# norabelrose/sparse-vae

Measured on AMD Instinct MI355X. Metric: training tokens/sec + ELBO match vs CPU ref, 512-tok seq, 1/2/4/8 MI355X, higher is better.
Workload: dtype bf16; 1 GPU; c2: TransformerVAE 6L d512 heads 8 seq 512, batch 64/GPU, dense attention, dropout 0.1, fwd+bwd+allreduce+clip+RAdam; model=TransformerVAE-6L-d512, global_batch=64, seq_len=512, parallelism=dp1

## Files before the change

include/svae.h:

```cpp
#ifndef SVAE_H
#define SVAE_H
#include <stdint.h>
#ifdef __cplusplus
extern "C" {
#endif

typedef void* svae_stream_t;

enum svae_epi {
  SVAE_EPI_BF16 = 0,
  SVAE_EPI_F32 = 1,
  SVAE_EPI_F32_ACC = 2,
  SVAE_EPI_F32_ATOMIC = 3,
  SVAE_EPI_GELU = 4,
  SVAE_EPI_GELU_BWD = 5,
  SVAE_EPI_DROPOUT_RESID = 6,
  SVAE_EPI_ROTARY_BF16 = 7,
  SVAE_EPI_CE_STATS = 8,
  SVAE_EPI_CE_PROB = 9,
  SVAE_EPI_ROWSCALE_GATHER = 10
};

typedef struct svae_gemm_desc {
  const void* A;
  const void* B;
  int64_t lda, ldb, batch_stride_a, batch_stride_b;
  int32_t M, N, K;
  int32_t batch, splits;
  int32_t a_t, b_t;
  int32_t epi;
  void* C;
  int64_t ldc, batch_stride_c;
  const float* bias;
  const float* resid;
  int64_t ldr;
  void* aux;
  int64_t ldaux;
  float alpha;
  float drop_p;
  uint64_t seed;
  const float* rot_tab;
  int32_t rot_cols, rot_d, rot_seq;
  const int32_t* labels;
  float* label_logit;
  float* a_rowsum;
  const float* k_weight;
  const float* row_a;
  const float* row_b;
  const void* gather;
  int64_t ldg;
  float* delta;
  const float* delta_o32;
  int64_t ld_o32;
  int32_t delta_hd, delta_seq;
} svae_gemm_desc;

int svae_gemm(const svae_gemm_desc* d, svae_stream_t stream);

int svae_gemm_pair(const svae_gemm_desc* d0, const svae_gemm_desc* d1, svae_stream_t stream);

#define SVAE_GROUP_MAX 256
#define SVAE_GROUP_MAX_BLOCKS 1024
int64_t svae_gemm_group_table_bytes(int32_t n);
int svae_gemm_group(const svae_gemm_desc* d, int32_t n, int32_t max_blocks, void* table, void* table_host,
                    int64_t table_bytes, svae_stream_t stream);

int svae_resid_ln_fwd(const float* x, const void* y, int32_t y_dtype, int64_t ldy, float drop_p, uint64_t seed,
                      const float* zrows, int32_t zmod, const float* w, const float* b, float* xo, void* h, float* mean,
                      float* rstd, int32_t rows, int32_t D, svae_stream_t stream);
int svae_layernorm_fwd(const void* x, int32_t x_dtype, const float* w, const float* b, void* y,
                       float* mean, float* rstd, int32_t rows, int32_t D, svae_stream_t stream);
int svae_layernorm_bwd(const void* dy, const void* x, int32_t x_dtype, const float* w, const float* mean,
                       const float* rstd, const float* dres, float* dx, void* dx_bf, float* part,
                       int32_t nblk, int32_t rows, int32_t D, int32_t zero_mod, svae_stream_t stream);
int svae_layernorm_bwd_drop(const void* dy, const void* x, int32_t x_dtype, const float* w, const float* mean,
                            const float* rstd, const float* dres, float* dx, void* dx_bf, float* part, int32_t nblk,
                            int32_t rows, int32_t D, int32_t zero_mod, float bf_drop_p, uint64_t bf_seed,
                            int32_t bf_zero_mod, float* zrow, void* zrow_bf, svae_stream_t stream);
int svae_layernorm_bwd_gelu(const void* dy, const void* x, int32_t x_dtype, const float* w, const float* mean,
                            const float* rstd, const void* gp, void* out_bf, float* part, int32_t nblk, int32_t rows,
                            int32_t D, svae_stream_t stream);
int svae_layernorm_fwd_z(float* x, const float* zrows, int32_t zmod, const float* w, const float* b, void* y,
                         float* mean, float* rstd, int32_t rows, int32_t D, svae_stream_t stream);
int svae_layernorm_nblk(int32_t rows);
#define SVAE_LN_MULTI_MAX 4
int svae_layernorm_fwd_multi(const float* x, const float* const* w, const float* const* b, void* const* y, int32_t n,
                             float* mean, float* rstd, int32_t rows, int32_t D, svae_stream_t stream);
int svae_layernorm_bwd_multi(const void* const* dy, const float* x, const float* const* w, const float* mean,
                             const float* rstd, const float* dres, float* dx, float* const* part, int32_t nblk,
                             int32_t n, int32_t rows, int32_t D, svae_stream_t stream);

int svae_colsum(const void* in, int32_t in_dtype, int32_t rows, int32_t cols, int64_t ld, float* out,
                int32_t accumulate, svae_stream_t stream);

#define SVAE_COLSUM_MAX 8
typedef struct svae_colsum_seg {
  const float* in;
  float* out;
  int64_t ld;
  int32_t rows, cols;
} svae_colsum_seg;
int svae_colsum_multi(const svae_colsum_seg* segs, int32_t n, svae_stream_t stream);

typedef struct svae_attn_desc {
  const void* q; const void* k; const void* v; void* o;
  int64_t sq, sk, sv, so, bq, bk, bv, bo;
  const uint8_t* key_pad;
  float* lse;
  int32_t B, H, Lq, Lk, hd, causal;
  float scale;
  const void* dout; int64_t sdo, bdo;
  float* delta;
  float* dq;
  int64_t bdq;
  void* dk; void* dv;
  int64_t sdk, sdv, bdk, bdv;
  const float* rot_tab;
  int32_t rot_d;
  float* o32;
  int64_t so32, bo32;
  float* dq_part;
  void* dq_bf;
  int64_t ldq_bf;
  int32_t window;
  int32_t delta_ready;
  void* o_lo;
  int64_t so_lo, bo_lo;
  float* fwd_ws;
  int64_t fwd_ws_elems;
} svae_attn_desc;

int svae_attn_fwd(const svae_attn_desc* d, svae_stream_t stream);
int64_t svae_attn_fwd_ws_elems(int32_t B, int32_t H, int32_t Lq, int32_t Lk, int32_t hd, int32_t causal, int32_t window);
int svae_attn_bwd(const svae_attn_desc* d, svae_stream_t stream);
int64_t svae_attn_dq_part_elems(int32_t B, int32_t H, int32_t Lq, int32_t Lk, int32_t hd);
int64_t svae_attn_dq_part_elems_w(int32_t B, int32_t H, int32_t Lq, int32_t Lk, int32_t hd, int32_t window);
int svae_dq_finalize(const float* dq, void* out, int64_t ldo, int32_t rows, int32_t D, const float* rot_tab,
                     int32_t seq, svae_stream_t stream);

int svae_embedding_fwd(const int32_t* ids, const void* table_bf, float* out, void* out_bf, int32_t rows,
                       int32_t D, svae_stream_t stream);
int svae_embedding_fwd_dual(const int32_t* ids, const void* table, float* out, float* out2, int32_t rows, int32_t D,
                            svae_stream_t stream);
int svae_embedding_bwd(const int32_t* ids, const float* dout, float* dtable, int32_t rows, int32_t D,
                       svae_stream_t stream);

int svae_reparam_kl_fwd(const float* stats, const float* eps, uint64_t seed, const int64_t* ntok,
                        float* z, void* z_bf, float* eps_out, float* raw_kl, float* kl_out, int32_t B,
                        int32_t Z, svae_stream_t stream);
int svae_reparam_kl_bwd(const float* stats, const float* eps, const float* dz, const int64_t* ntok,
                        const float* gkl, float* dstats, int32_t B, int32_t Z, svae_stream_t stream);

int svae_ce_finalize(const float* part, int32_t ntile, const float* label_logit, const int32_t* labels,
                     int32_t rows, int32_t seq, int32_t nchunks, int32_t chunk_len, float* lse, float* row_loss,
                     float* chunk_w, float* nll_out, float* red_ws, svae_stream_t stream);
int svae_ce_weighted_nll(const float* row_loss, const int32_t* labels, const float* tok_w, int32_t rows,
                         int32_t seq, int32_t nchunks, int32_t chunk_len, float* out, float* red_ws,
                         svae_stream_t stream);
int32_t svae_ce_red_ws_elems(int32_t nchunks);
int svae_ce_grad(void* logits, int64_t ld, const float* lse, const float* chunk_w, const int32_t* labels,
                 const float* gscale, float* dbias, int32_t rows, int32_t V, int32_t seq, int32_t nchunks,
                 int32_t chunk_len, svae_stream_t stream);

int svae_ce_label_logit(const void* hh, int64_t ldh, const void* W, int64_t ldw, const float* bias,
                        const int32_t* labels, int32_t rows, int32_t D, float* out, svae_stream_t stream);
int svae_ce_prob_finalize(const float* part, int32_t ntile, const float* row_off, const int32_t* labels,
                          int32_t rows, int32_t seq, int32_t nchunks, int32_t chunk_len, float* lse, float* row_loss,
                          float* chunk_w, float* nll_out, float* red_ws, svae_stream_t stream);
int svae_ce_prob_finalize_fix(const float* part, int32_t ntile, float* row_off, const int32_t* labels, int32_t rows,
                              int32_t seq, int32_t nchunks, int32_t chunk_len, float* lse, float* row_loss,
                              float* chunk_w, float* nll_out, float* red_ws, const void* hh, int64_t ldh, const void* W,
                              int64_t ldw, const float* bias, void* P, int64_t ldp, int32_t V, int32_t D,
                              int32_t* sat_ws, svae_stream_t stream);
int svae_ce_prob_bwd_prep(const void* hh, int64_t ldh, const float* lse, const float* row_off, const float* chunk_w,
                          const int32_t* labels, const float* gscale, int32_t rows, int32_t seq, int32_t nchunks,
                          int32_t chunk_len, int32_t D, void* hh_out, float* r_out, float* q_out, float* dbias,
                          svae_stream_t stream);
int svae_embedding_bwd_ce(const int32_t* ids, const float* dout, float* dtable, int32_t rows, int32_t D, int32_t seq,
                          const void* hh, const float* q, svae_stream_t stream);

int svae_dropout_bwd_cast(const float* g, void* out, float p, uint64_t seed, int64_t n, int32_t cols,
                          int64_t ld_in, svae_stream_t stream);
int svae_gelu_bwd(const float* dx, const void* gp, void* out, int64_t n, svae_stream_t stream);
int svae_prep_tokens(const int64_t* ids, const void* pad, int32_t pad_mode, int32_t B, int32_t L, int32_t* ids32,
                     int32_t* labels, void* padm, const int64_t* ntok, int64_t* ntok_out, svae_stream_t stream);
int svae_step_scalars(const float* nll, const float* kl, const float* gloss, float kl_weight, float* loss, float* gs,
                      svae_stream_t stream);
int svae_cast_bf16(const float* in, void* out, int64_t n, svae_stream_t stream);
int svae_transpose_blocks(const void* src, void* dst, const int64_t* table, int32_t nblocks, int32_t total_tiles,
                          svae_stream_t stream);
int svae_extract_rows(float* x, int64_t ld, int32_t rows, int32_t mod, int32_t D, float* out,
                      svae_stream_t stream);
int svae_zproj_bwd(const float* g, const void* z, const void* W, float* dW, float* db, float* dz, int32_t B,
                   int32_t d, int32_t Z, svae_stream_t stream);
#define SVAE_ZPROJ_MAX 32
typedef struct svae_zproj_seg {
  const float* g;
  const void* W;
  float* dW;
  float* db;
} svae_zproj_seg;
int svae_zproj_bwd_multi(const svae_zproj_seg* segs, int32_t n, const void* z, float* dz, int32_t B, int32_t d,
                         int32_t Z, svae_stream_t stream);
typedef struct svae_zproj_fwd_seg {
  const void* W;
  const float* bias;
  float* out;
} svae_zproj_fwd_seg;
int svae_zproj_fwd_multi(const svae_zproj_fwd_seg* segs, int32_t n, const void* z, int32_t B, int32_t d, int32_t Z,
                         svae_stream_t stream);

int svae_sumsq(const float* g, int64_t n, float* part, int32_t nblk, svae_stream_t stream);
int svae_radam(float* p, void* pbf, const float* g, float* m, float* v, int64_t n, const float* part,
               int32_t nblk, const float* scal, float* norm_out, svae_stream_t stream);
int svae_clip_grad(float* g, int64_t n, const float* part, int32_t nblk, float max_norm, float* norm_out,
                   svae_stream_t stream);

int svae_gemm_f32(const float* A, const float* W, float* C, int32_t M, int32_t N, int32_t K, int64_t lda, int64_t ldw,
                  int64_t ldc, const float* bias, const float* resid, int64_t ldr, int32_t epi, const float* rot_tab,
                  int32_t rot_cols, int32_t rot_d, int32_t rot_seq, svae_stream_t stream);
int svae_attn_fwd_f32(const float* q, const float* k, const float* v, float* o, int64_t sq, int64_t sk, int64_t sv,
                      int64_t so, int64_t bq, int64_t bk, int64_t bv, int64_t bo, const uint8_t* key_pad, int32_t B,
                      int32_t H, int32_t Lq, int32_t Lk, int32_t hd, int32_t causal, int32_t window, float scale,
                      svae_stream_t stream);
int svae_layernorm_fwd_f32(const float* x, const float* w, const float* b, float* y, int32_t rows, int32_t D,
                           svae_stream_t stream);

int svae_mutual_info(const float* stats, const float* eps, uint64_t seed, const float* kl, int32_t B, int32_t Z,
                     int32_t S, float* ws, float* out, svae_stream_t stream);

int svae_ce_seq_logprob(const float* part, int32_t ntile, const float* label_logit, const int32_t* labels,
                        int32_t rows, int32_t seq, float* out, svae_stream_t stream);

int svae_dec_linear(const float* X, int64_t ldx, const float* W, int64_t ldw, const float* bias, float* Y, int64_t ldy,
                    const float* resid, int64_t ldr, int32_t M, int32_t N, int32_t K, int32_t epi, const float* rot_tab,
                    int32_t rot_cols, int32_t rot_d, const int32_t* cur, float* part_ws, int64_t part_elems,
                    svae_stream_t stream);
int svae_dec_attn(const float* qkv, int64_t ldq, float* kcache, float* vcache, int32_t B, int32_t H, int32_t hd,
                  int32_t T, const int32_t* cur, int32_t window, float scale, float* O, int64_t ldo,
                  svae_stream_t stream);
int svae_dec_embed(const int64_t* out_ids, int32_t T, const int32_t* cur, const float* table, float* x, int32_t B,
                   int32_t D, svae_stream_t stream);
int svae_dec_penalty(float* logits, int64_t ldl, int32_t rows, const int32_t* row_map, const int64_t* out_ids,
                     int32_t T, const int32_t* cur, const uint8_t* live, float penalty, svae_stream_t stream);
int svae_dec_sample(const float* logits, int64_t ldl, int32_t V, int32_t rows, const int32_t* row_map,
                    int64_t* out_ids, int32_t T, const int32_t* cur, uint8_t* live, int32_t end_token,
                    float temperature, int32_t top_k, float top_p, uint64_t seed, int32_t* live_count,
                    svae_stream_t stream);
int svae_dec_advance(int32_t* cur, svae_stream_t stream);

int svae_slot_linear(const float* X, int64_t ldx, const float* W, int64_t ldw, const float* bias, float* Y, int64_t ldy,
                     const float* resid, int64_t ldr, int32_t S, int32_t N, int32_t K, const float* rot_tab,
                     int32_t rot_cols, int32_t rot_d, const int32_t* pos, float* part_ws, int64_t part_elems,
                     svae_stream_t stream);
int svae_slot_attn(const float* qkv, int64_t ldq, float* kcache, float* vcache, int32_t S, int32_t H, int32_t hd,
                   int32_t T, const int32_t* pos, int32_t window, float scale, float* O, int64_t ldo,
                   svae_stream_t stream);
int svae_slot_embed(const int64_t* ids, int32_t T, const int32_t* pos, const float* table, float* x, int32_t S,
                    int32_t D, svae_stream_t stream);
int svae_slot_splice(float* x, const float* zp, int64_t ldz, const int32_t* pos, int32_t S, int32_t D,
// ... 77 lines not shown
```

sparse-vae_amd/csrc/elementwise.hip:

```cpp
#include "common.h"
#include "../../include/svae.h"

using namespace svae;

namespace {

__global__ __launch_bounds__(256) void emb_fwd_kernel(const int* __restrict__ ids, const float* __restrict__ table,
                                                      float* __restrict__ out, bf16* __restrict__ out_bf, int rows,
                                                      int D, float* __restrict__ out2) {
  const int lane = threadIdx.x & 63;
  const int row = blockIdx.x * 4 + (threadIdx.x >> 6);
  if (row >= rows) return;
  const long long src = (long long)ids[row] * D;
  for (int c = lane * 4; c < D; c += 256) {
    const f32x4 v = *(const f32x4*)(table + src + c);
    *(f32x4*)(out + (long long)row * D + c) = v;
    if (out2) *(f32x4*)(out2 + (long long)row * D + c) = v;
    if (out_bf)
      *(bf16x4*)(out_bf + (long long)row * D + c) = (bf16x4){f2bf(v[0]), f2bf(v[1]), f2bf(v[2]), f2bf(v[3])};
  }
}

__global__ __launch_bounds__(256) void emb_bwd_kernel(const int* __restrict__ ids, const float* __restrict__ dout,
                                                      float* __restrict__ dtable, int rows, int D) {
  const int lane = threadIdx.x & 63;
  const int row = blockIdx.x * 4 + (threadIdx.x >> 6);
  if (row >= rows) return;
  const long long dst = (long long)ids[row] * D;
  for (int c = lane; c < D; c += 64) atomicAdd(dtable + dst + c, dout[(long long)row * D + c]);
}

__global__ __launch_bounds__(256) void emb_bwd_ce_kernel(const int* __restrict__ ids, const float* __restrict__ dout,
                                                         float* __restrict__ dtable, int rows, int D, int seq,
                                                         const bf16* __restrict__ hh, const float* __restrict__ q) {
  const int lane = threadIdx.x & 63;
  const int row = blockIdx.x * 4 + (threadIdx.x >> 6);
  if (row >= rows) return;
  const long long dst = (long long)ids[row] * D;
  const float qp = (row % seq != 0) ? q[row - 1] : 0.f;
  const bf16* hp = hh + (long long)(row - 1) * D;
  for (int c = lane; c < D; c += 64) {
    float g = dout[(long long)row * D + c];
    if (qp != 0.f) g -= qp * (float)hp[c];
    atomicAdd(dtable + dst + c, g);
  }
}

constexpr int REPARAM_WAVES = 16;

__global__ __launch_bounds__(1024) void reparam_fwd_kernel(const float* __restrict__ stats, const float* __restrict__ eps_in,
                                                           unsigned long long seed, const long long* __restrict__ ntok,
                                                           float* __restrict__ z, bf16* __restrict__ z_bf,
                                                           float* __restrict__ eps_out, float* __restrict__ raw_kl,
                                                           float* __restrict__ kl_out, int B, int Z) {
  __shared__ float red[2][REPARAM_WAVES];
  const int lane = threadIdx.x & 63, wave = threadIdx.x >> 6;
  float acc_norm = 0.f, acc_raw = 0.f;
  constexpr int NB = 4;
  for (int b0 = wave; b0 < B; b0 += NB * REPARAM_WAVES) {
    float klsum[NB];
#pragma unroll
    for (int k = 0; k < NB; ++k) klsum[k] = 0.f;
    for (int j = lane; j < Z; j += 64) {
      float mu[NB], lv[NB], e[NB];
#pragma unroll
      for (int k = 0; k < NB; ++k) {
        const int b = b0 + k * REPARAM_WAVES;
        if (b < B) {
          mu[k] = stats[(long long)b * 2 * Z + j];
          lv[k] = stats[(long long)b * 2 * Z + Z + j];
          if (eps_in) {
            e[k] = eps_in[(long long)b * Z + j];
          } else {
            const unsigned long long idx = ((unsigned long long)b * Z + j) * 2ull;
            const float u1 = rand_uniform(seed, idx), u2 = rand_uniform(seed, idx + 1);
            e[k] = sqrtf(-2.f * __logf(u1)) * __cosf(6.283185307179586f * u2);
          }
        }
      }
#pragma unroll
      for (int k = 0; k < NB; ++k) {
        const int b = b0 + k * REPARAM_WAVES;
        if (b < B) {
          const float var = __expf(lv[k]);
          const float zz = mu[k] + e[k] * sqrtf(var);
          if (eps_out) eps_out[(long long)b * Z + j] = e[k];
          z[(long long)b * Z + j] = zz;
          if (z_bf) z_bf[(long long)b * Z + j] = f2bf(zz);
          klsum[k] += 0.5f * (mu[k] * mu[k] + var - lv[k] - 1.0f);
        }
      }
    }
#pragma unroll
    for (int k = 0; k < NB; ++k) {
      const int b = b0 + k * REPARAM_WAVES;
      if (b < B) {
        const float ks = wave_sum(klsum[k]);
        if (lane == 0) raw_kl[b] = ks;
        acc_raw += ks;
        acc_norm += ks / (float)ntok[b];
      }
    }
  }
  if (lane == 0) { red[0][wave] = acc_norm; red[1][wave] = acc_raw; }
  __syncthreads();
  if (threadIdx.x == 0) {
    float n = 0.f, r = 0.f;
#pragma unroll
    for (int w = 0; w < REPARAM_WAVES; ++w) { n += red[0][w]; r += red[1][w]; }
    kl_out[0] = n / B;
    kl_out[1] = r / B;
  }
}

__global__ __launch_bounds__(256) void reparam_bwd_kernel(const float* __restrict__ stats, const float* __restrict__ eps,
                                                          const float* __restrict__ dz, const long long* __restrict__ ntok,
                                                          const float* __restrict__ gkl, float* __restrict__ dstats,
                                                          int B, int Z) {
  const int i = blockIdx.x * 256 + threadIdx.x;
  if (i >= B * Z) return;
  const int b = i / Z, j = i % Z;
  const float mu = stats[(long long)b * 2 * Z + j];
  const float lv = stats[(long long)b * 2 * Z + Z + j];
  const float var = __expf(lv), sd = sqrtf(var);
  const float w = gkl[0] / ((float)B * (float)ntok[b]);
  const float g = dz ? dz[i] : 0.f;
  dstats[(long long)b * 2 * Z + j] = g + w * mu;
  dstats[(long long)b * 2 * Z + Z + j] = g * eps[i] * sd * 0.5f + w * 0.5f * (var - 1.0f);
}

__global__ __launch_bounds__(256) void ce_rows_kernel(const float* __restrict__ part, int ntile,
                                                      const float* __restrict__ label_logit, const int* __restrict__ labels,
                                                      int rows, float* __restrict__ lse, float* __restrict__ row_loss) {
  const int lane = threadIdx.x & 63;
  const int row = blockIdx.x * 4 + (threadIdx.x >> 6);
  if (row >= rows) return;
  const float2* pr = (const float2*)part + (long long)row * ntile;
  float mx = -INFINITY;
  for (int t = lane; t < ntile; t += 64) mx = fmaxf(mx, pr[t].x);
  mx = wave_max(mx);
  float se = 0.f;
  for (int t = lane; t < ntile; t += 64) {
    const float2 v = pr[t];
    se += (v.x == -INFINITY) ? 0.f : v.y * __expf(v.x - mx);
  }
  se = wave_sum(se);
  if (lane == 0) {
    const float l = mx + __logf(se);
    lse[row] = l;
    row_loss[row] = labels[row] != 0 ? l - label_logit[row] : 0.f;
  }
}

__global__ __launch_bounds__(256) void ce_label_logit_kernel(const bf16* __restrict__ hh, long long ldh,
                                                             const bf16* __restrict__ W, long long ldw,
                                                             const float* __restrict__ bias,
                                                             const int* __restrict__ labels, int rows, int D,
                                                             float* __restrict__ out) {
  const int lane = threadIdx.x & 63;
  const int row = blockIdx.x * 4 + (threadIdx.x >> 6);
  if (row >= rows) return;
  const int lab = labels[row];
  if (lab == 0) {
    if (lane == 0) out[row] = 0.f;
    return;
  }
  float acc = 0.f;
  for (int c = lane * 8; c < D; c += 512) {
    const bf16x8 a = *(const bf16x8*)(hh + (long long)row * ldh + c);
    const bf16x8 b = *(const bf16x8*)(W + (long long)lab * ldw + c);
#pragma unroll
    for (int e = 0; e < 8; ++e) acc = fmaf((float)a[e], (float)b[e], acc);
  }
  acc = wave_sum(acc);
  if (lane == 0) out[row] = acc + (bias ? bias[lab] : 0.f);
}

__global__ __launch_bounds__(256) void ce_prob_rows_kernel(const float* __restrict__ part, int ntile,
                                                           const float* __restrict__ off, const int* __restrict__ labels,
                                                           int rows, float* __restrict__ lse, float* __restrict__ row_loss,
                                                           int* __restrict__ sat) {
  __shared__ float red[8][33];
  const int r = threadIdx.x & 31, sl = threadIdx.x >> 5;
  const int row = blockIdx.x * 32 + r;
  float acc = 0.f;
  if (row < rows) {
    int t = sl;
    for (; t + 56 < ntile; t += 64) {
      float v[8];
#pragma unroll
      for (int u = 0; u < 8; ++u) v[u] = part[(long long)(t + 8 * u) * rows + row];
      acc += ((v[0] + v[1]) + (v[2] + v[3])) + ((v[4] + v[5]) + (v[6] + v[7]));
    }
    for (; t < ntile; t += 8) acc += part[(long long)t * rows + row];
  }
  red[sl][r] = acc;
  __syncthreads();
  if (sl != 0 || row >= rows) return;
  float se = red[0][r];
#pragma unroll
  for (int k = 1; k < 8; ++k) se += red[k][r];
  const bool live = labels[row] != 0;
  const float l = live ? __logf(se) : 0.f;
  lse[row] = live ? off[row] + l : 0.f;
  row_loss[row] = l;
  if (sat && live && !(se < 0x1p100f)) sat[1 + atomicAdd(sat, 1)] = row;
}

__global__ __launch_bounds__(256) void ce_prob_fixup_kernel(const int* __restrict__ sat, const bf16* __restrict__ hh,
                                                            long long ldh, const bf16* __restrict__ W, long long ldw,
                                                            const float* __restrict__ bias, bf16* __restrict__ P,
                                                            long long ldp, int V, int D, float* __restrict__ off,
                                                            float* __restrict__ lse, float* __restrict__ row_loss) {
  __shared__ float h[1024];
  __shared__ float red[4];
  const int n = sat[0];
  const int lane = threadIdx.x & 63, w = threadIdx.x >> 6;
  for (int i = blockIdx.x; i < n; i += gridDim.x) {
    const int row = sat[1 + i];
    __syncthreads();
    for (int c = threadIdx.x; c < D; c += 256) h[c] = (float)hh[(long long)row * ldh + c];
    __syncthreads();
    float mx = -INFINITY;
    for (int col = threadIdx.x; col < V; col += 256) {
      const bf16* wr = W + (long long)col * ldw;
      float acc = 0.f;
      for (int c = 0; c < D; c += 8) {
        const bf16x8 b = *(const bf16x8*)(wr + c);
#pragma unroll
        for (int e = 0; e < 8; ++e) acc = fmaf(h[c + e], (float)b[e], acc);
      }
      mx = fmaxf(mx, acc + (bias ? bias[col] : 0.f));
    }
    mx = wave_max(mx);
    if (lane == 0) red[w] = mx;
    __syncthreads();
    mx = fmaxf(fmaxf(red[0], red[1]), fmaxf(red[2], red[3]));
    __syncthreads();
    float se = 0.f;
    for (int col = threadIdx.x; col < V; col += 256) {
      const bf16* wr = W + (long long)col * ldw;
      float acc = 0.f;
      for (int c = 0; c < D; c += 8) {
        const bf16x8 b = *(const bf16x8*)(wr + c);
#pragma unroll
        for (int e = 0; e < 8; ++e) acc = fmaf(h[c + e], (float)b[e], acc);
      }
      const float p = __expf(acc + (bias ? bias[col] : 0.f) - mx);
      P[(long long)row * ldp + col] = f2bf(p);
      se += p;
    }
    se = wave_sum(se);
    if (lane == 0) red[w] = se;
    __syncthreads();
    if (threadIdx.x == 0) {
      const float l = mx + __logf(red[0] + red[1] + red[2] + red[3]);
      row_loss[row] = l - off[row];
      lse[row] = l;
      off[row] = mx;
    }
  }
}

__global__ __launch_bounds__(256) void ce_prob_bwd_prep_kernel(const bf16* __restrict__ hh, long long ldh,
                                                               const float* __restrict__ lse,
                                                               const float* __restrict__ off,
                                                               const float* __restrict__ chunk_w,
                                                               const int* __restrict__ labels,
                                                               const float* __restrict__ gscale, int rows, int seq,
                                                               int nchunks, int chunk_len, int D,
                                                               bf16* __restrict__ hh_out, float* __restrict__ r_out,
                                                               float* __restrict__ q_out, float* __restrict__ dbias) {
  const int lane = threadIdx.x & 63;
  const int row = blockIdx.x * 4 + (threadIdx.x >> 6);
  if (row >= rows) return;
  const int lab = labels[row];
  float q = 0.f, r = 0.f;
  if (lab != 0) {
    const int ch = min((row % seq) / chunk_len, nchunks - 1);
    q = gscale[0] * chunk_w[ch];
    r = q * __expf(off[row] - lse[row]);
  }
  for (int c = lane * 8; c < D; c += 512) {
    const bf16x8 a = *(const bf16x8*)(hh + (long long)row * ldh + c);
    bf16x8 o;
#pragma unroll
    for (int e = 0; e < 8; ++e) o[e] = f2bf(r * (float)a[e]);
    *(bf16x8*)(hh_out + (long long)row * D + c) = o;
  }
  if (lane == 0) {
    r_out[row] = r;
    q_out[row] = q;
    if (lab != 0 && dbias) atomicAdd(dbias + lab, -q);
  }
}

__global__ __launch_bounds__(256) void ce_seq_logprob_kernel(const float* __restrict__ part, int ntile,
                                                             const float* __restrict__ label_logit,
                                                             const int* __restrict__ labels, int seq,
                                                             float* __restrict__ out) {
  __shared__ float ws[4];
  const int lane = threadIdx.x & 63, w = threadIdx.x >> 6;
  const long long r0 = (long long)blockIdx.x * seq;
  float acc = 0.f;
  for (int i = w; i < seq; i += 4) {
    const long long row = r0 + i;
    if (labels[row] == 0) continue;
    const float2* pr = (const float2*)part + row * ntile;
    float mx = -INFINITY;
    for (int t = lane; t < ntile; t += 64) mx = fmaxf(mx, pr[t].x);
    mx = wave_max(mx);
    float se = 0.f;
    for (int t = lane; t < ntile; t += 64) {
      const float2 v = pr[t];
      se += (v.x == -INFINITY) ? 0.f : v.y * __expf(v.x - mx);
    }
    se = wave_sum(se);
    acc += label_logit[row] - (mx + __logf(se));
  }
  if (lane == 0) ws[w] = acc;
  __syncthreads();
  if (threadIdx.x == 0) out[blockIdx.x] = ws[0] + ws[1] + ws[2] + ws[3];
}

__global__ __launch_bounds__(256) void mi_marginal_kernel(const float* __restrict__ stats, const float* __restrict__ eps,
                                                          unsigned long long seed, int B, int Z,
                                                          float* __restrict__ ws) {
  extern __shared__ float xs[];
  __shared__ float red[8];
  const int si = blockIdx.x, i = si % B, tid = threadIdx.x;
  const int lane = tid & 63, w = tid >> 6;
  float sq = 0.f;
  for (int z = tid; z < Z; z += 256) {
    const float mu = stats[(long long)i * 2 * Z + z];
    const float sd = sqrtf(__expf(stats[(long long)i * 2 * Z + Z + z]));
    float e;
    if (eps) {
      e = eps[(long long)si * Z + z];
    } else {
      const unsigned long long idx = ((unsigned long long)si * Z + z) * 2ull;
      const float u1 = rand_uniform(seed, idx), u2 = rand_uniform(seed, idx + 1);
      e = sqrtf(-2.f * __logf(u1)) * __cosf(6.283185307179586f * u2);
    }
    const float x = mu + e * sd;
    xs[z] = x;
    sq += x * x;
  }
  __syncthreads();
  const float lsq2pi = 0.91893853320467274f;
  float m = -INFINITY, e = 0.f;
  for (int j = tid; j < B; j += 256) {
    const float* st = stats + (long long)j * 2 * Z;
    float acc = 0.f;
    for (int z = 0; z < Z; ++z) {
      const float lv = st[Z + z];
      const float d = xs[z] - st[z];
      acc += -(d * d) * (0.5f * __expf(-lv)) - 0.5f * lv - lsq2pi;
    }
    const float nm = fmaxf(m, acc);
    e = e * __expf(m - nm) + __expf(acc - nm);
    m = nm;
  }
  float mx = wave_max(m);
  if (lane == 0) red[w] = mx;
  __syncthreads();
  mx = fmaxf(fmaxf(red[0], red[1]), fmaxf(red[2], red[3]));
  __syncthreads();
  float se = wave_sum(m == -INFINITY ? 0.f : e * __expf(m - mx));
  sq = wave_sum(sq);
  if (lane == 0) { red[w] = se; red[4 + w] = sq; }
  __syncthreads();
  if (tid == 0) {
    ws[si] = mx + __logf(red[0] + red[1] + red[2] + red[3]) - __logf((float)B);
    ws[gridDim.x + si] = red[4] + red[5] + red[6] + red[7];
  }
}

__global__ __launch_bounds__(256) void mi_final_kernel(const float* __restrict__ ws, int n, int Z,
                                                       const float* __restrict__ kl, float* __restrict__ out) {
  __shared__ float red[8];
  const int tid = threadIdx.x, lane = tid & 63, w = tid >> 6;
  float m = 0.f, q = 0.f;
  for (int k = tid; k < n; k += 256) { m += ws[k]; q += ws[n + k]; }
  m = wave_sum(m);
  q = wave_sum(q);
  if (lane == 0) { red[w] = m; red[4 + w] = q; }
  __syncthreads();
  if (tid == 0) {
    const float mm = (red[0] + red[1] + red[2] + red[3]) / n;
    const float qq = (red[4] + red[5] + red[6] + red[7]) / n;
    const float sample_prob = -0.5f * (qq + Z * 1.8378770664093453f);
    out[0] = kl[0] - (sample_prob - mm);
  }
}

constexpr int CE_RED_BLOCKS = 64;
constexpr int CE_MAX_CHUNKS = 1024;

__global__ __launch_bounds__(256) void ce_reduce_part_kernel(const float* __restrict__ row_loss,
                                                             const int* __restrict__ labels,
                                                             const float* __restrict__ tok_w, int rows, int seq,
                                                             int nchunks, int chunk_len, float* __restrict__ part) {
  __shared__ float red[8];
  const int ch = blockIdx.y;
  const int p0 = ch * chunk_len;
  const int clen = ch == nchunks - 1 ? seq - p0 : chunk_len;
  const int n = (rows / seq) * clen;
  float s = 0.f, c = 0.f;
  for (int i = blockIdx.x * 256 + threadIdx.x; i < n; i += CE_RED_BLOCKS * 256) {
    const int r = (i / clen) * seq + p0 + i % clen;
    const int lab = labels[r];
    if (lab != 0) {
      const float w = tok_w ? tok_w[lab] : 1.f;
      s += w * row_loss[r];
      c += w;
    }
  }
  s = wave_sum(s);
  c = wave_sum(c);
  if ((threadIdx.x & 63) == 0) { red[threadIdx.x >> 6] = s; red[4 + (threadIdx.x >> 6)] = c; }
  __syncthreads();
  if (threadIdx.x == 0) {
    float* o = part + ((long long)ch * CE_RED_BLOCKS + blockIdx.x) * 2;
    o[0] = (red[0] + red[1]) + (red[2] + red[3]);
    o[1] = (red[4] + red[5]) + (red[6] + red[7]);
  }
}

__global__ __launch_bounds__(256) void ce_reduce_final_kernel(const float* __restrict__ part, int nchunks,
                                                              float* __restrict__ chunk_w, float* __restrict__ nll_out) {
  __shared__ float mean[CE_MAX_CHUNKS];
  for (int k = threadIdx.x; k < nchunks; k += 256) {
    float ts = 0.f, tc = 0.f;
    for (int b = 0; b < CE_RED_BLOCKS; ++b) {
      ts += part[((long long)k * CE_RED_BLOCKS + b) * 2];
      tc += part[((long long)k * CE_RED_BLOCKS + b) * 2 + 1];
    }
    mean[k] = ts / tc;
    if (chunk_w) chunk_w[k] = 1.0f / (tc * (float)nchunks);
  }
  __syncthreads();
  if (threadIdx.x == 0) {
    float nll = 0.f;
    for (int j = 0; j < nchunks; ++j) nll += mean[j];
    nll_out[0] = nll / nchunks;
  }
}

#define CE_U 2
#define CE_LOAD(p) __builtin_nontemporal_load(p)
#define CE_STORE(v, p) __builtin_nontemporal_store(v, p)
__global__ __launch_bounds__(256) void ce_grad_kernel(bf16* __restrict__ logits, long long ld, const float* __restrict__ lse,
                                                      const float* __restrict__ chunk_w, const int* __restrict__ labels,
                                                      const float* __restrict__ gscale, float* __restrict__ dbias, int rows,
                                                      int V, int seq, int nchunks, int chunk_len, int rows_per_block) {
  const int c0 = (blockIdx.x * 256 + threadIdx.x) * 8;
  const int r0 = blockIdx.y * rows_per_block;
  const int r1 = min(rows, r0 + rows_per_block);
  const float g = gscale[0];
  float db[8] = {0.f, 0.f, 0.f, 0.f, 0.f, 0.f, 0.f, 0.f};
  if (c0 < V) {
    for (int row = r0; row < r1; row += CE_U) {
      bf16x8 v[CE_U];
#pragma unroll
      for (int u = 0; u < CE_U; ++u)
        if (row + u < r1) v[u] = CE_LOAD((const bf16x8*)(logits + (long long)(row + u) * ld + c0));
#pragma unroll
      for (int u = 0; u < CE_U; ++u) {
        const int rr = row + u;
        if (rr >= r1) break;
        bf16x8* ptr = (bf16x8*)(logits + (long long)rr * ld + c0);
        const int lab = labels[rr];
        bf16x8 o;
        if (lab == 0) {
          o = (bf16x8){0, 0, 0, 0, 0, 0, 0, 0};
        } else {
          const int ch = min((rr % seq) / chunk_len, nchunks - 1);
          const float w = g * chunk_w[ch];
          const float l = lse[rr];
#pragma unroll
          for (int e = 0; e < 8; ++e) {
            float pr = __expf((float)v[u][e] - l);
            if (c0 + e == lab) pr -= 1.0f;
            const float d = w * pr;
            db[e] += d;
            o[e] = f2bf(d);
          }
        }
        CE_STORE(o, ptr);
      }
    }
    if (dbias) {
#pragma unroll
      for (int e = 0; e < 8; ++e) atomicAdd(dbias + c0 + e, db[e]);
    }
  }
}

__global__ __launch_bounds__(256) void dropout_bwd_cast_kernel(const float* __restrict__ g, bf16* __restrict__ out, float p,
                                                               unsigned long long seed, long long n, int cols, long long ld_in) {
  const float scale = p > 0.f ? 1.0f / (1.0f - p) : 1.0f;
  for (long long i = ((long long)blockIdx.x * 256 + threadIdx.x) * 4; i < n; i += (long long)gridDim.x * 1024) {
    const long long r = i / cols;
    const int c = (int)(i % cols);
    const f32x4 v = *(const f32x4*)(g + r * ld_in + c);
    bf16x4 o;
    float u[4] = {1.f, 1.f, 1.f, 1.f};
    if (p > 0.f) rand_uniform4(seed, (unsigned long long)i >> 2, u);
#pragma unroll
    for (int e = 0; e < 4; ++e) {
      float x = v[e];
      if (p > 0.f) x = (u[e] >= p) ? x * scale : 0.f;
      o[e] = f2bf(x);
    }
    *(bf16x4*)(out + i) = o;
  }
}

__global__ __launch_bounds__(256) void prep_tokens_kernel(const int64_t* __restrict__ ids, const unsigned char* __restrict__ pad,
                                                          int pad_mode, int rows, int L, int32_t* __restrict__ ids32,
                                                          int32_t* __restrict__ labels, unsigned char* __restrict__ padm,
                                                          const int64_t* __restrict__ ntok, int64_t* __restrict__ ntok_out,
                                                          int B) {
  const int t = blockIdx.x * 256 + threadIdx.x;
  if (t < B && ntok) ntok_out[t] = ntok[t];
  if (t >= rows) return;
  const int64_t v = ids[t];
  ids32[t] = (int32_t)v;
  labels[t] = (t % L == L - 1) ? 0 : (int32_t)ids[t + 1];
// ... 224 lines not shown
  if (g < 1) g = 1;
  if (g > cap) g = cap;
  return (int)g;
}

}

SVAE_EXPORT int svae_embedding_fwd(const int32_t* ids, const void* table, float* out, void* out_bf, int32_t rows,
                                   int32_t D, svae_stream_t stream) {
  if (!ids || !table || !out || rows <= 0 || D % 4) return SVAE_EINVAL;
  hipLaunchKernelGGL(emb_fwd_kernel, dim3((rows + 3) / 4), dim3(256), 0, (hipStream_t)stream, ids, (const float*)table,
                     out, (bf16*)out_bf, rows, D, (float*)nullptr);
  SVAE_LAUNCH_CHECK();
  return SVAE_OK;
}

SVAE_EXPORT int svae_embedding_fwd_dual(const int32_t* ids, const void* table, float* out, float* out2, int32_t rows,
                                        int32_t D, svae_stream_t stream) {
  if (!ids || !table || !out || !out2 || rows <= 0 || D % 4) return SVAE_EINVAL;
  hipLaunchKernelGGL(emb_fwd_kernel, dim3((rows + 3) / 4), dim3(256), 0, (hipStream_t)stream, ids, (const float*)table,
                     out, (bf16*)nullptr, rows, D, out2);
  SVAE_LAUNCH_CHECK();
  return SVAE_OK;
}

SVAE_EXPORT int svae_embedding_bwd(const int32_t* ids, const float* dout, float* dtable, int32_t rows, int32_t D,
                                   svae_stream_t stream) {
  if (!ids || !dout || !dtable || rows <= 0 || D <= 0) return SVAE_EINVAL;
  hipLaunchKernelGGL(emb_bwd_kernel, dim3((rows + 3) / 4), dim3(256), 0, (hipStream_t)stream, ids, dout, dtable, rows, D);
  SVAE_LAUNCH_CHECK();
  return SVAE_OK;
}

SVAE_EXPORT int svae_embedding_bwd_ce(const int32_t* ids, const float* dout, float* dtable, int32_t rows, int32_t D,
                                      int32_t seq, const void* hh, const float* q, svae_stream_t stream) {
  if (!ids || !dout || !dtable || !hh || !q || rows <= 0 || D <= 0 || seq <= 0 || rows % seq) return SVAE_EINVAL;
  hipLaunchKernelGGL(emb_bwd_ce_kernel, dim3((rows + 3) / 4), dim3(256), 0, (hipStream_t)stream, ids, dout, dtable, rows,
                     D, seq, (const bf16*)hh, q);
  SVAE_LAUNCH_CHECK();
  return SVAE_OK;
}

SVAE_EXPORT int svae_ce_label_logit(const void* hh, int64_t ldh, const void* W, int64_t ldw, const float* bias,
                                    const int32_t* labels, int32_t rows, int32_t D, float* out, svae_stream_t stream) {
  if (!hh || !W || !labels || !out || rows <= 0 || D <= 0 || D % 8 || ldh % 8 || ldw % 8) return SVAE_EINVAL;
  if (((uintptr_t)hh | (uintptr_t)W) & 15) return SVAE_EINVAL;
  hipLaunchKernelGGL(ce_label_logit_kernel, dim3((rows + 3) / 4), dim3(256), 0, (hipStream_t)stream, (const bf16*)hh,
                     (long long)ldh, (const bf16*)W, (long long)ldw, bias, labels, rows, D, out);
  SVAE_LAUNCH_CHECK();
  return SVAE_OK;
}

SVAE_EXPORT int svae_ce_prob_finalize(const float* part, int32_t ntile, const float* row_off, const int32_t* labels,
                                      int32_t rows, int32_t seq, int32_t nchunks, int32_t chunk_len, float* lse,
                                      float* row_loss, float* chunk_w, float* nll_out, float* red_ws,
                                      svae_stream_t stream) {
  return svae_ce_prob_finalize_fix(part, ntile, (float*)row_off, labels, rows, seq, nchunks, chunk_len, lse, row_loss,
                                   chunk_w, nll_out, red_ws, nullptr, 0, nullptr, 0, nullptr, nullptr, 0, 0, 0, nullptr,
                                   stream);
}

SVAE_EXPORT int svae_ce_prob_finalize_fix(const float* part, int32_t ntile, float* row_off, const int32_t* labels,
                                          int32_t rows, int32_t seq, int32_t nchunks, int32_t chunk_len, float* lse,
                                          float* row_loss, float* chunk_w, float* nll_out, float* red_ws,
                                          const void* hh, int64_t ldh, const void* W, int64_t ldw, const float* bias,
                                          void* P, int64_t ldp, int32_t V, int32_t D, int32_t* sat_ws,
                                          svae_stream_t stream) {
  if (!part || !row_off || !labels || !lse || !row_loss || !chunk_w || !nll_out || !red_ws) return SVAE_EINVAL;
  if (rows <= 0 || ntile <= 0 || seq <= 0 || rows % seq || nchunks <= 0 || nchunks > CE_MAX_CHUNKS ||
      chunk_len <= 0 || (long long)(nchunks - 1) * chunk_len >= seq)
    return SVAE_EINVAL;
  const bool fix = sat_ws != nullptr;
  if (fix && (!hh || !W || !P || V <= 0 || D <= 0 || D > 1024 || D % 8 || ldh % 8 || ldw % 8 ||
              (((uintptr_t)hh | (uintptr_t)W) & 15)))
    return SVAE_EINVAL;
  hipStream_t s = (hipStream_t)stream;
  if (fix && hipMemsetAsync(sat_ws, 0, sizeof(int32_t), s) != hipSuccess) return SVAE_ELAUNCH;
  hipLaunchKernelGGL(ce_prob_rows_kernel, dim3((rows + 31) / 32), dim3(256), 0, s, part, ntile, row_off, labels, rows,
                     lse, row_loss, (int*)sat_ws);
  if (fix)
    hipLaunchKernelGGL(ce_prob_fixup_kernel, dim3(64), dim3(256), 0, s, (const int*)sat_ws, (const bf16*)hh,
                       (long long)ldh, (const bf16*)W, (long long)ldw, bias, (bf16*)P, (long long)ldp, V, D, row_off,
                       lse, row_loss);
  hipLaunchKernelGGL(ce_reduce_part_kernel, dim3(CE_RED_BLOCKS, nchunks), dim3(256), 0, s, row_loss, labels,
                     (const float*)nullptr, rows, seq, nchunks, chunk_len, red_ws);
  hipLaunchKernelGGL(ce_reduce_final_kernel, dim3(1), dim3(256), 0, s, red_ws, nchunks, chunk_w, nll_out);
  SVAE_LAUNCH_CHECK();
  return SVAE_OK;
}

SVAE_EXPORT int svae_ce_prob_bwd_prep(const void* hh, int64_t ldh, const float* lse, const float* row_off,
                                      const float* chunk_w, const int32_t* labels, const float* gscale, int32_t rows,
                                      int32_t seq, int32_t nchunks, int32_t chunk_len, int32_t D, void* hh_out,
                                      float* r_out, float* q_out, float* dbias, svae_stream_t stream) {
  if (!hh || !lse || !row_off || !chunk_w || !labels || !gscale || !hh_out || !r_out || !q_out) return SVAE_EINVAL;
  if (rows <= 0 || seq <= 0 || nchunks <= 0 || chunk_len <= 0 || D <= 0 || D % 8 || ldh % 8) return SVAE_EINVAL;
  if (((uintptr_t)hh | (uintptr_t)hh_out) & 15) return SVAE_EINVAL;
  hipLaunchKernelGGL(ce_prob_bwd_prep_kernel, dim3((rows + 3) / 4), dim3(256), 0, (hipStream_t)stream, (const bf16*)hh,
                     (long long)ldh, lse, row_off, chunk_w, labels, gscale, rows, seq, nchunks, chunk_len, D,
                     (bf16*)hh_out, r_out, q_out, dbias);
  SVAE_LAUNCH_CHECK();
  return SVAE_OK;
}

SVAE_EXPORT int svae_reparam_kl_fwd(const float* stats, const float* eps, uint64_t seed, const int64_t* ntok, float* z,
                                    void* z_bf, float* eps_out, float* raw_kl, float* kl_out, int32_t B, int32_t Z,
                                    svae_stream_t stream) {
  if (!stats || !ntok || !z || !raw_kl || !kl_out || B <= 0 || Z <= 0) return SVAE_EINVAL;
  hipLaunchKernelGGL(reparam_fwd_kernel, dim3(1), dim3(64 * REPARAM_WAVES), 0, (hipStream_t)stream, stats, eps, seed,
                     (const long long*)ntok, z, (bf16*)z_bf, eps_out, raw_kl, kl_out, B, Z);
  SVAE_LAUNCH_CHECK();
  return SVAE_OK;
}

SVAE_EXPORT int svae_reparam_kl_bwd(const float* stats, const float* eps, const float* dz, const int64_t* ntok,
                                    const float* gkl, float* dstats, int32_t B, int32_t Z, svae_stream_t stream) {
  if (!stats || !eps || !ntok || !gkl || !dstats || B <= 0 || Z <= 0) return SVAE_EINVAL;
  hipLaunchKernelGGL(reparam_bwd_kernel, dim3((B * Z + 255) / 256), dim3(256), 0, (hipStream_t)stream, stats, eps, dz,
                     (const long long*)ntok, gkl, dstats, B, Z);
  SVAE_LAUNCH_CHECK();
  return SVAE_OK;
}

SVAE_EXPORT int svae_ce_finalize(const float* part, int32_t ntile, const float* label_logit, const int32_t* labels,
                                 int32_t rows, int32_t seq, int32_t nchunks, int32_t chunk_len, float* lse,
                                 float* row_loss, float* chunk_w, float* nll_out, float* red_ws, svae_stream_t stream) {
  if (!part || !label_logit || !labels || !lse || !row_loss || !chunk_w || !nll_out || !red_ws) return SVAE_EINVAL;
  if (rows <= 0 || ntile <= 0 || seq <= 0 || rows % seq || nchunks <= 0 || nchunks > CE_MAX_CHUNKS ||
      chunk_len <= 0 || (long long)(nchunks - 1) * chunk_len >= seq)
    return SVAE_EINVAL;
  hipStream_t s = (hipStream_t)stream;
  hipLaunchKernelGGL(ce_rows_kernel, dim3((rows + 3) / 4), dim3(256), 0, s, part, ntile, label_logit, labels, rows, lse,
                     row_loss);
  hipLaunchKernelGGL(ce_reduce_part_kernel, dim3(CE_RED_BLOCKS, nchunks), dim3(256), 0, s, row_loss, labels,
                     (const float*)nullptr, rows, seq, nchunks, chunk_len, red_ws);
  hipLaunchKernelGGL(ce_reduce_final_kernel, dim3(1), dim3(256), 0, s, red_ws, nchunks, chunk_w, nll_out);
  SVAE_LAUNCH_CHECK();
  return SVAE_OK;
}

SVAE_EXPORT int svae_ce_weighted_nll(const float* row_loss, const int32_t* labels, const float* tok_w, int32_t rows,
                                     int32_t seq, int32_t nchunks, int32_t chunk_len, float* out, float* red_ws,
                                     svae_stream_t stream) {
  if (!row_loss || !labels || !tok_w || !out || !red_ws) return SVAE_EINVAL;
  if (rows <= 0 || seq <= 0 || rows % seq || nchunks <= 0 || nchunks > CE_MAX_CHUNKS || chunk_len <= 0 ||
      (long long)(nchunks - 1) * chunk_len >= seq)
    return SVAE_EINVAL;
  hipStream_t s = (hipStream_t)stream;
  hipLaunchKernelGGL(ce_reduce_part_kernel, dim3(CE_RED_BLOCKS, nchunks), dim3(256), 0, s, row_loss, labels, tok_w, rows,
                     seq, nchunks, chunk_len, red_ws);
  hipLaunchKernelGGL(ce_reduce_final_kernel, dim3(1), dim3(256), 0, s, red_ws, nchunks, (float*)nullptr, out);
  SVAE_LAUNCH_CHECK();
  return SVAE_OK;
}

SVAE_EXPORT int32_t svae_ce_red_ws_elems(int32_t nchunks) { return nchunks * CE_RED_BLOCKS * 2; }

SVAE_EXPORT int svae_mutual_info(const float* stats, const float* eps, uint64_t seed, const float* kl, int32_t B,
                                 int32_t Z, int32_t S, float* ws, float* out, svae_stream_t stream) {
  if (!stats || !kl || !ws || !out || B <= 0 || Z <= 0 || S <= 0 || Z > 4096) return SVAE_EINVAL;
  hipStream_t s = (hipStream_t)stream;
  hipLaunchKernelGGL(mi_marginal_kernel, dim3(S * B), dim3(256), (size_t)Z * sizeof(float), s, stats, eps,
                     (unsigned long long)seed, B, Z, ws);
  hipLaunchKernelGGL(mi_final_kernel, dim3(1), dim3(256), 0, s, ws, S * B, Z, kl, out);
  SVAE_LAUNCH_CHECK();
  return SVAE_OK;
}

SVAE_EXPORT int svae_ce_seq_logprob(const float* part, int32_t ntile, const float* label_logit, const int32_t* labels,
                                    int32_t rows, int32_t seq, float* out, svae_stream_t stream) {
  if (!part || !label_logit || !labels || !out || rows <= 0 || ntile <= 0 || seq <= 0 || rows % seq) return SVAE_EINVAL;
  hipLaunchKernelGGL(ce_seq_logprob_kernel, dim3(rows / seq), dim3(256), 0, (hipStream_t)stream, part, ntile,
                     label_logit, labels, seq, out);
  SVAE_LAUNCH_CHECK();
  return SVAE_OK;
}

SVAE_EXPORT int svae_ce_grad(void* logits, int64_t ld, const float* lse, const float* chunk_w, const int32_t* labels,
                             const float* gscale, float* dbias, int32_t rows, int32_t V, int32_t seq, int32_t nchunks,
                             int32_t chunk_len, svae_stream_t stream) {
  if (!logits || !lse || !chunk_w || !labels || !gscale || rows <= 0 || V % 8 || ld % 8) return SVAE_EINVAL;
  const int strips = (V + 2047) / 2048;
  int rpb = 256;
  while (rpb > 16 && (long long)strips * ((rows + rpb - 1) / rpb) < 1024) rpb /= 2;
  dim3 grid(strips, (rows + rpb - 1) / rpb);
  hipLaunchKernelGGL(ce_grad_kernel, grid, dim3(256), 0, (hipStream_t)stream, (bf16*)logits, ld, lse, chunk_w, labels,
                     gscale, dbias, rows, V, seq, nchunks, chunk_len, rpb);
  SVAE_LAUNCH_CHECK();
  return SVAE_OK;
}

SVAE_EXPORT int svae_dropout_bwd_cast(const float* g, void* out, float p, uint64_t seed, int64_t n, int32_t cols,
                                      int64_t ld_in, svae_stream_t stream) {
  if (!g || !out || n <= 0 || cols <= 0 || cols % 4 || n % cols || ld_in % 4) return SVAE_EINVAL;
  hipLaunchKernelGGL(dropout_bwd_cast_kernel, dim3(grid_for(n, 1024)), dim3(256), 0, (hipStream_t)stream, g, (bf16*)out,
                     p, seed, n, cols, ld_in);
  SVAE_LAUNCH_CHECK();
  return SVAE_OK;
}

SVAE_EXPORT int svae_gelu_bwd(const float* dx, const void* gp, void* out, int64_t n, svae_stream_t stream) {
  if (!dx || !gp || !out || n <= 0) return SVAE_EINVAL;
  hipLaunchKernelGGL(gelu_bwd_kernel, dim3(grid_for(n, 256)), dim3(256), 0, (hipStream_t)stream, dx, (const bf16*)gp,
                     (bf16*)out, n);
  SVAE_LAUNCH_CHECK();
  return SVAE_OK;
}

SVAE_EXPORT int svae_prep_tokens(const int64_t* ids, const void* pad, int32_t pad_mode, int32_t B, int32_t L,
                                 int32_t* ids32, int32_t* labels, void* padm, const int64_t* ntok, int64_t* ntok_out,
                                 svae_stream_t stream) {
  if (!ids || !ids32 || !labels || B <= 0 || L <= 0 || pad_mode < 0 || pad_mode > 2) return SVAE_EINVAL;
  if ((pad_mode && !padm) || (pad_mode == 2 && !pad) || (!ntok != !ntok_out)) return SVAE_EINVAL;
  const long long rows = (long long)B * L;
  if (rows > 0x7FFFFFFFLL - 256) return SVAE_EINVAL;
  const long long work = rows > B ? rows : B;
  hipLaunchKernelGGL(prep_tokens_kernel, dim3((unsigned)((work + 255) / 256)), dim3(256), 0, (hipStream_t)stream, ids,
                     (const unsigned char*)pad, pad_mode, (int)rows, L, ids32, labels, (unsigned char*)padm, ntok,
                     ntok_out, B);
  SVAE_LAUNCH_CHECK();
  return SVAE_OK;
}

SVAE_EXPORT int svae_step_scalars(const float* nll, const float* kl, const float* gloss, float kl_weight, float* loss,
                                  float* gs, svae_stream_t stream) {
  if ((!loss && !gs) || (loss && (!nll || !kl)) || (gs && !gloss)) return SVAE_EINVAL;
  hipLaunchKernelGGL(step_scalars_kernel, dim3(1), dim3(64), 0, (hipStream_t)stream, nll, kl, gloss, kl_weight, loss, gs);
  SVAE_LAUNCH_CHECK();
  return SVAE_OK;
}

SVAE_EXPORT int svae_cast_bf16(const float* in, void* out, int64_t n, svae_stream_t stream) {
// ... 263 lines not shown
```

sparse-vae_amd/csrc/layernorm.hip:

```cpp
#include <algorithm>

#include "common.h"
#include "../../include/svae.h"

using namespace svae;

namespace {


template <typename T>
__device__ __forceinline__ f32x4 load4(const T* p);
template <>
__device__ __forceinline__ f32x4 load4<float>(const float* p) { return *(const f32x4*)p; }
template <>
__device__ __forceinline__ f32x4 load4<bf16>(const bf16* p) {
  bf16x4 v = *(const bf16x4*)p;
  return (f32x4){(float)v[0], (float)v[1], (float)v[2], (float)v[3]};
}
__device__ __forceinline__ void store4_bf(bf16* p, f32x4 v) {
  *(bf16x4*)p = (bf16x4){f2bf(v[0]), f2bf(v[1]), f2bf(v[2]), f2bf(v[3])};
}

template <int MAXV>
__device__ __forceinline__ int ln_col(int lane, int k) {
// ... 407 lines not shown
      if (c < D) {
#pragma unroll
        for (int e = 0; e < 4; ++e) xh[j][e] = (cur.xv[j][e] - mean) * rstd;
#pragma unroll
        for (int i = 0; i < NM; ++i) {
          if (i >= m.n) break;
          const f32x4 ww = *(const f32x4*)(m.w[i] + c);
#pragma unroll
          for (int e = 0; e < 4; ++e) {
            const float dv = (float)cur.dv[i][j][e];
            g[j][e] += dv * ww[e];
            adw[i][j][e] += dv * xh[j][e];
            adb[i][j][e] += dv;
          }
        }
#pragma unroll
        for (int e = 0; e < 4; ++e) { s1 += g[j][e]; s2 += g[j][e] * xh[j][e]; }
      }
    }
    const float m1 = wave_sum(s1) / D, m2 = wave_sum(s2) / D;
#pragma unroll
    for (int j = 0; j < MAXV; ++j) {
      const int c = (lane + 64 * j) * 4;
      if (c < D) {
        f32x4 o;
#pragma unroll
        for (int e = 0; e < 4; ++e) o[e] = rstd * (g[j][e] - m1 - xh[j][e] * m2) + cur.rr[j][e];
        *(f32x4*)(dx + base + c) = o;
      }
    }
    cur = nxt;
  }
#pragma unroll
  for (int i = 0; i < NM; ++i) {
    if (i >= m.n) break;
    if (i > 0) __syncthreads();
#pragma unroll
    for (int j = 0; j < MAXV; ++j) {
      const int c = (lane + 64 * j) * 4;
      if (c < D) {
        *(f32x4*)&red[wave][0][c] = adw[i][j];
        *(f32x4*)&red[wave][1][c] = adb[i][j];
      }
    }
    __syncthreads();
    for (int c = threadIdx.x; c < 2 * D; c += 256) {
      const int which = c / D, col = c % D;
      const float s = red[0][which][col] + red[1][which][col] + red[2][which][col] + red[3][which][col];
      m.part[i][((long long)blockIdx.x * 2 + which) * D + col] = s;
    }
  }
}

template <typename T>
__global__ __launch_bounds__(256) void colsum_kernel(const T* __restrict__ in, int rows, int cols, long long ld,
                                                     float* __restrict__ out, int rows_per_split) {
  __shared__ f32x4 red[16][17];
  const int ct = threadIdx.x & 15, rt = threadIdx.x >> 4;
  const int c = (blockIdx.x * 16 + ct) * 4;
  const int r0 = blockIdx.y * rows_per_split;
  const int r1 = min(rows, r0 + rows_per_split);
  f32x4 acc = {0.f, 0.f, 0.f, 0.f};
  if (c < cols) {
    int r = r0 + rt;
    for (; r + 112 < r1; r += 128) {
      f32x4 v[8];
#pragma unroll
      for (int i = 0; i < 8; ++i) v[i] = load4<T>(in + (long long)(r + 16 * i) * ld + c);
      acc += ((v[0] + v[1]) + (v[2] + v[3])) + ((v[4] + v[5]) + (v[6] + v[7]));
    }
    for (; r < r1; r += 16) acc += load4<T>(in + (long long)r * ld + c);
  }
  red[rt][ct] = acc;
  __syncthreads();
  if (threadIdx.x < 16 && c < cols) {
    f32x4 s = red[0][ct];
#pragma unroll
    for (int i = 1; i < 16; ++i) s += red[i][ct];
#pragma unroll
    for (int e = 0; e < 4; ++e) atomicAdd(out + c + e, s[e]);
  }
}

struct ColsumSegs {
  const float* in[SVAE_COLSUM_MAX];
  float* out[SVAE_COLSUM_MAX];
  long long ld[SVAE_COLSUM_MAX];
  int rows[SVAE_COLSUM_MAX], cols[SVAE_COLSUM_MAX], rps[SVAE_COLSUM_MAX], colblocks[SVAE_COLSUM_MAX];
  int first[SVAE_COLSUM_MAX + 1];
  int n;
};
__global__ __launch_bounds__(256) void colsum_multi_kernel(ColsumSegs sg) {
  __shared__ f32x4 red[16][17];
  int sgi = 0;
  while (sgi + 1 < sg.n && (int)blockIdx.x >= sg.first[sgi + 1]) ++sgi;
  const int local = blockIdx.x - sg.first[sgi];
  const int cb = local % sg.colblocks[sgi], split = local / sg.colblocks[sgi];
  const float* in = sg.in[sgi];
  const int rows = sg.rows[sgi], cols = sg.cols[sgi];
  const long long ld = sg.ld[sgi];
  const int ct = threadIdx.x & 15, rt = threadIdx.x >> 4;
  const int c = (cb * 16 + ct) * 4;
  const int r0 = split * sg.rps[sgi];
  const int r1 = min(rows, r0 + sg.rps[sgi]);
  f32x4 acc = {0.f, 0.f, 0.f, 0.f};
  if (c < cols) {
    int r = r0 + rt;
    for (; r + 112 < r1; r += 128) {
      f32x4 v[8];
#pragma unroll
      for (int i = 0; i < 8; ++i) v[i] = *(const f32x4*)(in + (long long)(r + 16 * i) * ld + c);
      acc += ((v[0] + v[1]) + (v[2] + v[3])) + ((v[4] + v[5]) + (v[6] + v[7]));
    }
    for (; r < r1; r += 16) acc += *(const f32x4*)(in + (long long)r * ld + c);
  }
  red[rt][ct] = acc;
  __syncthreads();
  if (threadIdx.x < 16 && c < cols) {
    f32x4 s = red[0][ct];
#pragma unroll
    for (int i = 1; i < 16; ++i) s += red[i][ct];
#pragma unroll
    for (int e = 0; e < 4; ++e) atomicAdd(sg.out[sgi] + c + e, s[e]);
  }
}

static void colsum_grid(int rows, int cols, int& colblocks, int& splits, int& rps) {
  colblocks = (cols + 63) / 64;
  splits = (256 + colblocks - 1) / colblocks;
  const int max_splits = (rows + 127) / 128;
  if (splits > max_splits) splits = max_splits;
  if (splits < 1) splits = 1;
  rps = (rows + splits - 1) / splits;
  splits = (rows + rps - 1) / rps;
}

}

SVAE_EXPORT int svae_colsum_multi(const svae_colsum_seg* segs, int32_t n, svae_stream_t stream) {
  if (!segs || n <= 0 || n > SVAE_COLSUM_MAX) return SVAE_EINVAL;
  ColsumSegs sg;
  sg.n = n;
  int total = 0;
  for (int i = 0; i < n; ++i) {
    const svae_colsum_seg& q = segs[i];
    if (!q.in || !q.out || q.rows <= 0 || q.cols <= 0 || q.cols % 4 || q.ld % 4) return SVAE_EINVAL;
    if (((uintptr_t)q.in | (uintptr_t)q.out) & 15) return SVAE_EINVAL;
    int cb, sp, rps;
    colsum_grid(q.rows, q.cols, cb, sp, rps);
    sg.in[i] = q.in; sg.out[i] = q.out; sg.ld[i] = q.ld;
    sg.rows[i] = q.rows; sg.cols[i] = q.cols; sg.rps[i] = rps; sg.colblocks[i] = cb;
    sg.first[i] = total;
    total += cb * sp;
  }
  sg.first[n] = total;
  hipLaunchKernelGGL(colsum_multi_kernel, dim3((unsigned)total), dim3(256), 0, (hipStream_t)stream, sg);
  SVAE_LAUNCH_CHECK();
  return SVAE_OK;
}

struct LnFwdPlan {
  unsigned grid;
  int mv;
};
static LnFwdPlan ln_fwd_plan(int rows, int D) {
  const int mv = (D % 8 == 0 && D <= 512) ? 2 : D <= 768 ? 3 : D % 8 == 0 ? 4 : 5;
  return {(unsigned)std::min((rows + 3) / 4, D <= 768 ? 2048 : 1024), mv};
}

SVAE_EXPORT int svae_layernorm_fwd(const void* x, int32_t x_dtype, const float* w, const float* b, void* y,
                                   float* mean, float* rstd, int32_t rows, int32_t D, svae_stream_t stream) {
  if (!x || !w || !b || !y || !mean || !rstd || rows <= 0 || D <= 0 || D % 4 || D > 1024) return SVAE_EINVAL;
  const LnFwdPlan plan = ln_fwd_plan(rows, D);
  const dim3 grid(plan.grid);
  hipStream_t s = (hipStream_t)stream;
#define SVAE_LN_FWD(MV)                                                                                            \
  do {                                                                                                             \
    if (x_dtype == 0)                                                                                              \
      hipLaunchKernelGGL((ln_fwd_kernel<float, MV>), grid, dim3(256), 0, s, (const float*)x, w, b, (bf16*)y, mean, \
                         rstd, rows, D);                                                                           \
    else                                                                                                           \
      hipLaunchKernelGGL((ln_fwd_kernel<bf16, MV>), grid, dim3(256), 0, s, (const bf16*)x, w, b, (bf16*)y, mean,   \
                         rstd, rows, D);                                                                           \
  } while (0)
  if (plan.mv == 2) SVAE_LN_FWD(2);
  else if (plan.mv == 3) SVAE_LN_FWD(3);
  else if (plan.mv == 4) SVAE_LN_FWD(4);
  else SVAE_LN_FWD(5);
#undef SVAE_LN_FWD
  SVAE_LAUNCH_CHECK();
  return SVAE_OK;
}

SVAE_EXPORT int svae_layernorm_fwd_z(float* x, const float* zrows, int32_t zmod, const float* w, const float* b, void* y,
                                     float* mean, float* rstd, int32_t rows, int32_t D, svae_stream_t stream) {
  if (!x || !zrows || zmod <= 0 || !w || !b || !y || !mean || !rstd || rows <= 0 || D <= 0 || D % 8 || D > 1024)
    return SVAE_EINVAL;
  if (((uintptr_t)x | (uintptr_t)zrows) & 15) return SVAE_EINVAL;
  const LnFwdPlan plan = ln_fwd_plan(rows, D);
  const dim3 grid(plan.grid);
  hipStream_t s = (hipStream_t)stream;
  if (plan.mv == 2)
    hipLaunchKernelGGL((ln_fwd_kernel<float, 2, true>), grid, dim3(256), 0, s, (const float*)x, w, b, (bf16*)y, mean,
                       rstd, rows, D, zrows, zmod, x);
  else if (plan.mv == 3)
    hipLaunchKernelGGL((ln_fwd_kernel<float, 3, true>), grid, dim3(256), 0, s, (const float*)x, w, b, (bf16*)y, mean,
                       rstd, rows, D, zrows, zmod, x);
  else
    hipLaunchKernelGGL((ln_fwd_kernel<float, 4, true>), grid, dim3(256), 0, s, (const float*)x, w, b, (bf16*)y, mean,
                       rstd, rows, D, zrows, zmod, x);
  SVAE_LAUNCH_CHECK();
  return SVAE_OK;
}

SVAE_EXPORT int svae_resid_ln_fwd(const float* x, const void* y, int32_t y_dtype, int64_t ldy, float drop_p,
                                  uint64_t seed, const float* zrows, int32_t zmod, const float* w, const float* b,
                                  float* xo, void* h, float* mean, float* rstd, int32_t rows, int32_t D,
                                  svae_stream_t stream) {
  if (!h || rows <= 0 || D <= 0 || D % 8 || D > 1024 || (!x && !y && !zrows) || (y_dtype != 0 && y_dtype != 1))
    return SVAE_EINVAL;
  if ((w == nullptr) != (b == nullptr) || (w && (!mean || !rstd)) || (zrows && zmod <= 0)) return SVAE_EINVAL;
  if (drop_p < 0.f || drop_p >= 1.f || (y && ldy % 8) || (((uintptr_t)y | (uintptr_t)h) & 15)) return SVAE_EINVAL;
  if (((uintptr_t)x | (uintptr_t)xo | (uintptr_t)zrows | (uintptr_t)w | (uintptr_t)b) & 15) return SVAE_EINVAL;
  dim3 grid((rows + 3) / 4);
  hipStream_t s = (hipStream_t)stream;
#define SVAE_RLN(NR, CPL, TY)                                                                                     \
  hipLaunchKernelGGL((resid_ln_fwd_kernel<NR, CPL, TY>), grid, dim3(256), 0, s, x, (const TY*)y, (long long)ldy,     \
                     drop_p, (unsigned long long)seed, zrows, zmod, w, b, xo, (bf16*)h, mean, rstd, rows, D)
  if (D <= 512) {
    if (y_dtype == 0) SVAE_RLN(1, 8, float); else SVAE_RLN(1, 8, bf16);
  } else if (D <= 768) {
    if (y_dtype == 0) SVAE_RLN(3, 4, float); else SVAE_RLN(3, 4, bf16);
  } else {
    if (y_dtype == 0) SVAE_RLN(2, 8, float); else SVAE_RLN(2, 8, bf16);
  }
#undef SVAE_RLN
  SVAE_LAUNCH_CHECK();
  return SVAE_OK;
}

SVAE_EXPORT int svae_layernorm_fwd_multi(const float* x, const float* const* w, const float* const* b, void* const* y,
// ... 131 lines not shown
```

sparse-vae_amd/sparse_vae/_native.py:

```python
import ctypes
import os

import torch

_HERE = os.path.dirname(os.path.abspath(__file__))
LIB_PATH = os.environ.get('SVAE_LIB') or os.path.join(_HERE, 'libsvae.so')

c_void_p, c_int32, c_int64, c_float, c_uint64 = (ctypes.c_void_p, ctypes.c_int32, ctypes.c_int64,
                                                  ctypes.c_float, ctypes.c_uint64)
c_fptr = ctypes.c_void_p

EPI_BF16, EPI_F32, EPI_F32_ACC, EPI_F32_ATOMIC, EPI_GELU, EPI_GELU_BWD, EPI_DROPOUT_RESID, \
    EPI_ROTARY_BF16, EPI_CE_STATS, EPI_CE_PROB, EPI_ROWSCALE_GATHER = range(11)

LATENT_L2, LATENT_COSINE, LATENT_KL = range(3)
LATENT_METRICS = {'l2': LATENT_L2, 'cosine': LATENT_COSINE, 'kl': LATENT_KL}
LATENT_MAX_BLOCKS = 1024
TSNE_ROWS_PER_BLOCK, TSNE_TILE_COLS = 512, 256
PAIR_RBF, PAIR_IMQ = range(2)
PAIR_KINDS = {'rbf': PAIR_RBF, 'imq': PAIR_IMQ}
PAIRSUM_TILE_COLS, PAIRSUM_MAX_P, MMD_REDUCE_BLOCKS = 32, 8, 256
KMEANS_MAX_K, KMEANS_TILE_CENTROIDS, KMEANS_SORT_BLOCKS, KMEANS_SEED_BLOCK_ROWS = 1024, 32, 256, 256


class GemmDesc(ctypes.Structure):
    _fields_ = [
        ('A', c_void_p), ('B', c_void_p),
        ('lda', c_int64), ('ldb', c_int64), ('batch_stride_a', c_int64), ('batch_stride_b', c_int64),
        ('M', c_int32), ('N', c_int32), ('K', c_int32),
        ('batch', c_int32), ('splits', c_int32),
        ('a_t', c_int32), ('b_t', c_int32),
        ('epi', c_int32),
        ('C', c_void_p),
        ('ldc', c_int64), ('batch_stride_c', c_int64),
        ('bias', c_void_p), ('resid', c_void_p), ('ldr', c_int64),
        ('aux', c_void_p), ('ldaux', c_int64),
        ('alpha', c_float), ('drop_p', c_float), ('seed', c_uint64),
        ('rot_tab', c_void_p), ('rot_cols', c_int32), ('rot_d', c_int32), ('rot_seq', c_int32),
        ('labels', c_void_p), ('label_logit', c_void_p),
        ('a_rowsum', c_void_p),
        ('k_weight', c_void_p), ('row_a', c_void_p), ('row_b', c_void_p), ('gather', c_void_p), ('ldg', c_int64),
        ('delta', c_void_p), ('delta_o32', c_void_p), ('ld_o32', c_int64), ('delta_hd', c_int32), ('delta_seq', c_int32),
    ]


class AttnDesc(ctypes.Structure):
    _fields_ = [
        ('q', c_void_p), ('k', c_void_p), ('v', c_void_p), ('o', c_void_p),
        ('sq', c_int64), ('sk', c_int64), ('sv', c_int64), ('so', c_int64),
        ('bq', c_int64), ('bk', c_int64), ('bv', c_int64), ('bo', c_int64),
        ('key_pad', c_void_p), ('lse', c_void_p),
        ('B', c_int32), ('H', c_int32), ('Lq', c_int32), ('Lk', c_int32), ('hd', c_int32), ('causal', c_int32),
        ('scale', c_float),
        ('dout', c_void_p), ('sdo', c_int64), ('bdo', c_int64),
        ('delta', c_void_p), ('dq', c_void_p), ('bdq', c_int64),
        ('dk', c_void_p), ('dv', c_void_p),
        ('sdk', c_int64), ('sdv', c_int64), ('bdk', c_int64), ('bdv', c_int64),
        ('rot_tab', c_void_p), ('rot_d', c_int32),
        ('o32', c_void_p), ('so32', c_int64), ('bo32', c_int64),
        ('dq_part', c_void_p), ('dq_bf', c_void_p), ('ldq_bf', c_int64),
        ('window', c_int32),
        ('delta_ready', c_int32),
        ('o_lo', c_void_p), ('so_lo', c_int64), ('bo_lo', c_int64),
        ('fwd_ws', c_void_p), ('fwd_ws_elems', c_int64),
    ]


GROUP_MAX = 256
COLSUM_MAX = 8
LN_MULTI_MAX = 4


ZPROJ_MAX = 32


class ZprojSeg(ctypes.Structure):
    _fields_ = [('g', c_void_p), ('W', c_void_p), ('dW', c_void_p), ('db', c_void_p)]


class ZprojFwdSeg(ctypes.Structure):
    _fields_ = [('W', c_void_p), ('bias', c_void_p), ('out', c_void_p)]


class ColsumSeg(ctypes.Structure):
    _fields_ = [('inp', c_void_p), ('out', c_void_p), ('ld', c_int64), ('rows', c_int32), ('cols', c_int32)]


_SIGS = {
    'svae_gemm': [ctypes.POINTER(GemmDesc), c_void_p],
    'svae_gemm_pair': [ctypes.POINTER(GemmDesc), ctypes.POINTER(GemmDesc), c_void_p],
    'svae_gemm_group_table_bytes': [c_int32],
    'svae_gemm_group': [ctypes.POINTER(GemmDesc), c_int32, c_int32, c_void_p, c_void_p, c_int64, c_void_p],
    'svae_resid_ln_fwd': [c_void_p, c_void_p, c_int32, c_int64, c_float, c_uint64, c_void_p, c_int32, c_void_p,
                          c_void_p, c_void_p, c_void_p, c_void_p, c_void_p, c_int32, c_int32, c_void_p],
    'svae_layernorm_fwd': [c_void_p, c_int32, c_void_p, c_void_p, c_void_p, c_void_p, c_void_p, c_int32, c_int32,
                           c_void_p],
    'svae_layernorm_bwd': [c_void_p, c_void_p, c_int32, c_void_p, c_void_p, c_void_p, c_void_p, c_void_p, c_void_p,
                           c_void_p, c_int32, c_int32, c_int32, c_int32, c_void_p],
    'svae_layernorm_bwd_drop': [c_void_p, c_void_p, c_int32, c_void_p, c_void_p, c_void_p, c_void_p, c_void_p,
                                c_void_p, c_void_p, c_int32, c_int32, c_int32, c_int32, c_float, c_uint64, c_int32,
                                c_void_p, c_void_p, c_void_p],
    'svae_layernorm_bwd_gelu': [c_void_p, c_void_p, c_int32, c_void_p, c_void_p, c_void_p, c_void_p, c_void_p,
                                c_void_p, c_int32, c_int32, c_int32, c_void_p],
    'svae_layernorm_nblk': [c_int32],
    'svae_colsum': [c_void_p, c_int32, c_int32, c_int32, c_int64, c_void_p, c_int32, c_void_p],
    'svae_colsum_multi': [c_void_p, c_int32, c_void_p],
    'svae_attn_fwd': [ctypes.POINTER(AttnDesc), c_void_p],
    'svae_attn_bwd': [ctypes.POINTER(AttnDesc), c_void_p],
    'svae_attn_dq_part_elems': [c_int32, c_int32, c_int32, c_int32, c_int32],
    'svae_attn_dq_part_elems_w': [c_int32, c_int32, c_int32, c_int32, c_int32, c_int32],
    'svae_attn_fwd_ws_elems': [c_int32, c_int32, c_int32, c_int32, c_int32, c_int32, c_int32],
    'svae_transpose_blocks': [c_void_p, c_void_p, c_void_p, c_int32, c_int32, c_void_p],
    'svae_dq_finalize': [c_void_p, c_void_p, c_int64, c_int32, c_int32, c_void_p, c_int32, c_void_p],
    'svae_embedding_fwd': [c_void_p, c_void_p, c_void_p, c_void_p, c_int32, c_int32, c_void_p],
    'svae_embedding_fwd_dual': [c_void_p, c_void_p, c_void_p, c_void_p, c_int32, c_int32, c_void_p],
    'svae_embedding_bwd': [c_void_p, c_void_p, c_void_p, c_int32, c_int32, c_void_p],
    'svae_reparam_kl_fwd': [c_void_p, c_void_p, c_uint64, c_void_p, c_void_p, c_void_p, c_void_p, c_void_p,
                            c_void_p, c_int32, c_int32, c_void_p],
    'svae_reparam_kl_bwd': [c_void_p, c_void_p, c_void_p, c_void_p, c_void_p, c_void_p, c_int32, c_int32, c_void_p],
    'svae_ce_finalize': [c_void_p, c_int32, c_void_p, c_void_p, c_int32, c_int32, c_int32, c_int32, c_void_p,
                         c_void_p, c_void_p, c_void_p, c_void_p, c_void_p],
    'svae_ce_weighted_nll': [c_void_p, c_void_p, c_void_p, c_int32, c_int32, c_int32, c_int32, c_void_p, c_void_p,
                             c_void_p],
    'svae_ce_red_ws_elems': [c_int32],
    'svae_clip_grad': [c_void_p, c_int64, c_void_p, c_int32, c_float, c_void_p, c_void_p],
    'svae_ce_label_logit': [c_void_p, c_int64, c_void_p, c_int64, c_void_p, c_void_p, c_int32, c_int32, c_void_p,
                            c_void_p],
    'svae_ce_prob_finalize': [c_void_p, c_int32, c_void_p, c_void_p, c_int32, c_int32, c_int32, c_int32, c_void_p,
                              c_void_p, c_void_p, c_void_p, c_void_p, c_void_p],
    'svae_ce_prob_finalize_fix': [c_void_p, c_int32, c_void_p, c_void_p, c_int32, c_int32, c_int32, c_int32, c_void_p,
                                  c_void_p, c_void_p, c_void_p, c_void_p, c_void_p, c_int64, c_void_p, c_int64, c_void_p,
                                  c_void_p, c_int64, c_int32, c_int32, c_void_p, c_void_p],
    'svae_ce_prob_bwd_prep': [c_void_p, c_int64, c_void_p, c_void_p, c_void_p, c_void_p, c_void_p, c_int32, c_int32,
                              c_int32, c_int32, c_int32, c_void_p, c_void_p, c_void_p, c_void_p, c_void_p],
    'svae_embedding_bwd_ce': [c_void_p, c_void_p, c_void_p, c_int32, c_int32, c_int32, c_void_p, c_void_p, c_void_p],
    'svae_ce_grad': [c_void_p, c_int64, c_void_p, c_void_p, c_void_p, c_void_p, c_void_p, c_int32, c_int32, c_int32,
                     c_int32, c_int32, c_void_p],
    'svae_dropout_bwd_cast': [c_void_p, c_void_p, c_float, c_uint64, c_int64, c_int32, c_int64, c_void_p],
    'svae_gelu_bwd': [c_void_p, c_void_p, c_void_p, c_int64, c_void_p],
    'svae_prep_tokens': [c_void_p, c_void_p, c_int32, c_int32, c_int32, c_void_p, c_void_p, c_void_p, c_void_p,
                         c_void_p, c_void_p],
    'svae_step_scalars': [c_void_p, c_void_p, c_void_p, c_float, c_void_p, c_void_p, c_void_p],
    'svae_zproj_bwd_multi': [c_void_p, c_int32, c_void_p, c_void_p, c_int32, c_int32, c_int32, c_void_p],
    'svae_zproj_fwd_multi': [c_void_p, c_int32, c_void_p, c_int32, c_int32, c_int32, c_void_p],
    'svae_layernorm_fwd_multi': [c_void_p, c_void_p, c_void_p, c_void_p, c_int32, c_void_p, c_void_p, c_int32, c_int32,
                                 c_void_p],
    'svae_layernorm_bwd_multi': [c_void_p, c_void_p, c_void_p, c_void_p, c_void_p, c_void_p, c_void_p, c_void_p,
                                 c_int32, c_int32, c_int32, c_int32, c_void_p],
    'svae_layernorm_fwd_z': [c_void_p, c_void_p, c_int32, c_void_p, c_void_p, c_void_p, c_void_p, c_void_p, c_int32,
                             c_int32, c_void_p],
    'svae_cast_bf16': [c_void_p, c_void_p, c_int64, c_void_p],
    'svae_extract_rows': [c_void_p, c_int64, c_int32, c_int32, c_int32, c_void_p, c_void_p],
    'svae_zproj_bwd': [c_void_p, c_void_p, c_void_p, c_void_p, c_void_p, c_void_p, c_int32, c_int32, c_int32, c_void_p],
    'svae_sumsq': [c_void_p, c_int64, c_void_p, c_int32, c_void_p],
    'svae_radam': [c_void_p, c_void_p, c_void_p, c_void_p, c_void_p, c_int64, c_void_p, c_int32, c_void_p,
                   c_void_p, c_void_p],
    'svae_gemm_f32': [c_void_p, c_void_p, c_void_p, c_int32, c_int32, c_int32, c_int64, c_int64, c_int64, c_void_p,
                      c_void_p, c_int64, c_int32, c_void_p, c_int32, c_int32, c_int32, c_void_p],
    'svae_attn_fwd_f32': [c_void_p, c_void_p, c_void_p, c_void_p, c_int64, c_int64, c_int64, c_int64, c_int64, c_int64,
                          c_int64, c_int64, c_void_p, c_int32, c_int32, c_int32, c_int32, c_int32, c_int32, c_int32,
                          c_float, c_void_p],
    'svae_layernorm_fwd_f32': [c_void_p, c_void_p, c_void_p, c_void_p, c_int32, c_int32, c_void_p],
    'svae_ce_seq_logprob': [c_void_p, c_int32, c_void_p, c_void_p, c_int32, c_int32, c_void_p, c_void_p],
    'svae_dec_linear': [c_void_p, c_int64, c_void_p, c_int64, c_void_p, c_void_p, c_int64, c_void_p, c_int64, c_int32,
                        c_int32, c_int32, c_int32, c_void_p, c_int32, c_int32, c_void_p, c_void_p, c_int64, c_void_p],
    'svae_dec_attn': [c_void_p, c_int64, c_void_p, c_void_p, c_int32, c_int32, c_int32, c_int32, c_void_p, c_int32,
                      c_float, c_void_p, c_int64, c_void_p],
    'svae_dec_embed': [c_void_p, c_int32, c_void_p, c_void_p, c_void_p, c_int32, c_int32, c_void_p],
    'svae_dec_penalty': [c_void_p, c_int64, c_int32, c_void_p, c_void_p, c_int32, c_void_p, c_void_p, c_float,
                         c_void_p],
    'svae_dec_sample': [c_void_p, c_int64, c_int32, c_int32, c_void_p, c_void_p, c_int32, c_void_p, c_void_p, c_int32,
                        c_float, c_int32, c_float, c_uint64, c_void_p, c_void_p],
    'svae_dec_advance': [c_void_p, c_void_p],
    'svae_slot_linear': [c_void_p, c_int64, c_void_p, c_int64, c_void_p, c_void_p, c_int64, c_void_p, c_int64, c_int32,
                         c_int32, c_int32, c_void_p, c_int32, c_int32, c_void_p, c_void_p, c_int64, c_void_p],
    'svae_slot_attn': [c_void_p, c_int64, c_void_p, c_void_p, c_int32, c_int32, c_int32, c_int32, c_void_p, c_int32,
                       c_float, c_void_p, c_int64, c_void_p],
    'svae_slot_embed': [c_void_p, c_int32, c_void_p, c_void_p, c_void_p, c_int32, c_int32, c_void_p],
    'svae_slot_splice': [c_void_p, c_void_p, c_int64, c_void_p, c_int32, c_int32, c_void_p],
    'svae_slot_penalty': [c_void_p, c_int64, c_int32, c_void_p, c_int32, c_void_p, c_float, c_void_p],
    'svae_slot_sample': [c_void_p, c_int64, c_int32, c_int32, c_void_p, c_int32, c_void_p, c_void_p, c_void_p, c_int32,
                         c_int32, c_float, c_int32, c_float, c_uint64, c_void_p],
    'svae_slot_refill': [c_void_p, c_void_p, c_void_p, c_int32, c_int32, c_int32, c_void_p, c_void_p, c_int32, c_int32,
                         c_void_p, c_void_p, c_void_p],
    'svae_mutual_info': [c_void_p, c_void_p, c_uint64, c_void_p, c_int32, c_int32, c_int32, c_void_p, c_void_p,
                         c_void_p],
    'svae_latent_prepare': [c_void_p, c_void_p, c_void_p, c_void_p, c_void_p, c_int32, c_int32, c_void_p],
    'svae_latent_scores': [c_int32, c_void_p, c_void_p, c_void_p, c_void_p, c_int32, c_void_p, c_void_p, c_void_p,
                           c_void_p, c_int32, c_int32, c_void_p, c_void_p],
    'svae_latent_topk_ws_bytes': [c_int32, c_int32],
    'svae_latent_topk': [c_int32, c_void_p, c_void_p, c_void_p, c_void_p, c_int32, c_void_p, c_void_p, c_void_p,
                         c_void_p, c_int32, c_int32, c_int32, c_void_p, c_int64, c_void_p, c_void_p, c_void_p],
    'svae_tsne_affinities': [c_void_p, c_int32, c_int32, c_float, c_void_p, c_void_p, c_void_p],
    'svae_tsne_repulse_slice_cols': [c_int32],
    'svae_tsne_repulse_ws_bytes': [c_int32],
    'svae_tsne_repulse': [c_void_p, c_int32, c_void_p, c_int64, c_void_p, c_void_p, c_void_p, c_void_p],
    'svae_tsne_attract': [c_void_p, c_void_p, c_void_p, c_void_p, c_void_p, c_int32, c_int32, c_void_p, c_void_p],
    'svae_tsne_update': [c_void_p, c_void_p, c_void_p, c_void_p, c_void_p, c_void_p, c_int32, c_float, c_float,
                         c_float, c_void_p],
    'svae_pairsum_geometry': [c_int32, c_int32, c_int32, c_int32, c_void_p],
    'svae_pairsum_ws_bytes': [c_int32, c_int32, c_int32, c_int32],
    'svae_pairsum': [c_void_p, c_int32, c_void_p, c_int32, c_int32, c_int32, c_int32, c_void_p, c_int32, c_void_p,
                     c_void_p, c_int64, c_void_p, c_void_p],
    'svae_mmd_rowterm_ws_bytes': [c_int32],
    'svae_mmd_rowterm': [c_void_p, c_void_p, c_void_p, c_int32, c_int32, c_void_p, c_int64, c_void_p, c_void_p],
    'svae_latent_colstats_ws_bytes': [c_int32, c_int32],
    'svae_latent_colstats': [c_void_p, c_void_p, c_int32, c_int32, c_void_p, c_int64, c_void_p, c_void_p, c_void_p,
                             c_void_p],
    'svae_latent_draw': [c_void_p, c_void_p, c_void_p, c_uint64, c_int32, c_int32, c_void_p, c_void_p],
    'svae_kmeans_geometry': [c_int32, c_int32, c_int32, c_void_p],
    'svae_kmeans_assign_ws_bytes': [c_int32, c_int32, c_int32],
    'svae_kmeans_assign': [c_void_p, c_int32, c_void_p, c_int32, c_int32, c_void_p, c_void_p, c_void_p, c_void_p,
                           c_void_p, c_int64, c_void_p],
    'svae_kmeans_update_ws_bytes': [c_int32, c_int32, c_int32],
    'svae_kmeans_update': [c_void_p, c_int32, c_void_p, c_int32, c_int32, c_void_p, c_void_p, c_void_p, c_int64,
                           c_void_p],
    'svae_kmeans_seed_ws_bytes': [c_int32, c_int32, c_int32],
# ... 42 lines not shown
```

sparse-vae_amd/sparse_vae/engine.py:

```python
import math
import os
from collections import OrderedDict

import torch

from . import kernels as K
from ._native import COLSUM_MAX, GROUP_MAX, LN_MULTI_MAX, ZPROJ_MAX
from ._native import EPI_BF16, EPI_F32, EPI_F32_ACC, EPI_GELU, EPI_GELU_BWD, EPI_DROPOUT_RESID, \
    EPI_ROTARY_BF16, EPI_CE_STATS, EPI_F32_ATOMIC, EPI_CE_PROB, EPI_ROWSCALE_GATHER

bf16, f32 = torch.bfloat16, torch.float32
ALIGN = 64
CE_CHUNK_NUMEL = 2 ** 30


def _attn_entries(pre, d, learned):
    out = []
    if learned:
        out.append((pre + 'learned_queries', (1, learned, d)))
        names = ['k_linear', 'v_linear']
    else:
        names = ['q_linear', 'k_linear', 'v_linear']
    out += [(pre + n + '.weight', (d, d)) for n in names]
    out += [(pre + n + '.bias', (d,)) for n in names]
    out += [(pre + 'output_linear.weight', (d, d)), (pre + 'output_linear.bias', (d,))]
    return out


def _ctx_ln_entries(pre, d):
    return [(pre + 'context_layer_norm.weight', (d,)), (pre + 'context_layer_norm.bias', (d,))]


def _layer_entries(pre, d, learned=None, cross=False, ctx_ln=True):
    out = _attn_entries(pre + 'attention.', d, learned)
    out += [(pre + 'attn_layer_norm.weight', (d,)), (pre + 'attn_layer_norm.bias', (d,))]
    if cross:
        out += _attn_entries(pre + 'cross_attention.', d, None)
        out += [(pre + 'cross_attn_layer_norm.weight', (d,)), (pre + 'cross_attn_layer_norm.bias', (d,))]
        if ctx_ln:
            out += _ctx_ln_entries(pre, d)
    out += [(pre + 'ffn.0.weight', (4 * d, d)), (pre + 'ffn.0.bias', (4 * d,)), (pre + 'ffn.2.weight', (d, 4 * d)),
            (pre + 'ffn_layer_norm.weight', (d,)), (pre + 'ffn_layer_norm.bias', (d,))]
    return out


def _pos_linear_entries(pre, d):
    return [(pre + 'pos_linear.weight', (d, d)), (pre + 'pos_linear.bias', (d,))]


def ctx_ln_batched(hp):
    return hp.enc_layers - 2 >= 2 and os.environ.get('SVAE_CTX_LN_BATCH', '1') != '0'


def layout_entries(hp):
    d, V, Z, N = hp.d_model, hp.vocab_size, hp.latent_depth, hp.num_latents
    live = [('output_layer.0.weight', (d, d)), ('output_layer.0.bias', (d,)),
            ('output_layer.2.weight', (d,)), ('output_layer.2.bias', (d,)), ('output_layer.3.bias', (V,))]
    dead = []
    for i in reversed(range(hp.num_layers)):
        live += _layer_entries(f'decoder_layers.{i}.', d)
        live += [(f'z_projections.{i}.weight', (d, Z)), (f'z_projections.{i}.bias', (d,))]
        dead += _pos_linear_entries(f'decoder_layers.{i}.attention.', d)
    live += [('q_of_z_given_x.linear.weight', (2 * Z, d)), ('q_of_z_given_x.linear.bias', (2 * Z,))]
    live += _layer_entries('encoder.bottleneck.', d, learned=1)
    dead += _pos_linear_entries('encoder.bottleneck.attention.', d)
    nmid = hp.enc_layers - 2
    batched = ctx_ln_batched(hp)
    for j in reversed(range(nmid)):
        live += _layer_entries(f'encoder.middle_layers.{j}.', d, cross=True, ctx_ln=not batched)
        dead += _pos_linear_entries(f'encoder.middle_layers.{j}.attention.', d)
        dead += _pos_linear_entries(f'encoder.middle_layers.{j}.cross_attention.', d)
    if batched:
        for j in reversed(range(nmid)):
            live += _ctx_ln_entries(f'encoder.middle_layers.{j}.', d)
    live += _layer_entries('encoder.first_layer.', d, learned=N)
    dead += _pos_linear_entries('encoder.first_layer.attention.', d)
    live += [('input_layer.0.weight', (V, d))]
    return live, dead


class FlatParams:

    def __init__(self, hp, device):
        live, dead = layout_entries(hp)
        self.ctx_batched = ctx_ln_batched(hp)
        self.offsets = OrderedDict()
        off = 0
        for name, shape in live + dead:
            n = math.prod(shape)
            self.offsets[name] = (off, shape)
# ... 38 lines not shown
                assert off + rows * cols <= o or o + r * c <= off, f'overlapping transposed blocks at {name}'
            self.t_blocks[key] = (off, rows, cols)
            self._t_table = None
            self.refresh_transposed([key])
        return self.shadow_t[off:off + rows * cols].view(cols, rows)

    def refresh_transposed(self, keys=None):
        if not self.t_blocks:
            return
        if keys is None and self._t_table is not None:
            table, nb, tiles = self._t_table
        else:
            rows_tab, tiles = [], 0
            for k in (keys if keys is not None else self.t_blocks):
                o, r, c = self.t_blocks[k]
                rows_tab.append([o, r, c, tiles])
                tiles += -(-r // 64) * -(-c // 64)
            table = torch.tensor(rows_tab, dtype=torch.int64).to(self.device)
            nb = len(rows_tab)
            if keys is None:
                self._t_table = (table, nb, tiles)
        K.transpose_blocks(self.shadow, self.shadow_t, table, nb, tiles)

    def sync_shadow(self, force=False):
        if force or self.master._version != self.shadow_version:
            K.cast_bf16(self.master, self.shadow)
            self.refresh_transposed()
            self.shadow_version = self.master._version


class Workspace:

    def __init__(self, device):
        self.device = device
        self.bufs = {}

    def get(self, name, shape, dtype=bf16, zero=False):
        t = self.bufs.get(name)
        if t is None or t.shape != torch.Size(shape) or t.dtype != dtype:
            t = torch.empty(shape, dtype=dtype, device=self.device)
            self.bufs[name] = t
        if zero:
            t.zero_()
        return t


def rotary_table(positions, d, max_pos=10000):
    half = d // 2
    freqs = torch.arange(half, dtype=f32)
    pos = torch.arange(0, positions, dtype=f32)
    theta = max_pos ** (-freqs / half)
    ang = pos[:, None] * theta
    return torch.stack([ang.cos(), ang.sin()], dim=-1).contiguous()


def _mix_seed(a, b):
    x = (a * 0x9E3779B97F4A7C15 + b * 0xBF58476D1CE4E5B9 + 0x94D049BB133111EB) & 0xFFFFFFFFFFFFFFFF
    x ^= x >> 31
    return x


class VAEEngine:
    def __init__(self, hp, flat: FlatParams):
        self.hp = hp
        self.P = flat
        self.ws = Workspace(flat.device)
        self.d = hp.d_model
        self.H = hp.num_heads
        self.He = hp.d_model // 64
        assert self.d % self.H == 0 and self.d % 64 == 0
        self.hd = self.d // self.H
        self._rot = {}
        self.window = getattr(hp, 'attn_window', 0)
        self.saved = None
        self.probe = None
        self.head_mode = os.environ.get('SVAE_HEAD', 'prob')
        assert self.head_mode in ('prob', 'logits'), self.head_mode
        self.dw_group = os.environ.get('SVAE_DW_GROUP', '1') != '0'
        self._dw_jobs = []
        self._dwq = None
        self._dw_names = False
        self._dwg_states, self._dwg_sched = [], {}
        self._zp_pending, self._zp_ctx = [], None
        self._cs_pending = []
        self.ncu = (torch.cuda.get_device_properties(flat.device).multi_processor_count
                    if flat.device.type == 'cuda' else 256)

    def rot(self, L, window=0):
        need = max(L, self.hp.num_latents)
        base = 2 * window * 32 if window else 10000
        t = self._rot.get(base)
        if t is None or t.shape[0] < need:
            t = rotary_table(max(need, 512), self.d, base).to(self.P.device)
            self._rot[base] = t
        return t

    def _ln_fwd(self, name, x, rows, tag, zsplice=None):
        D = self.d
        y = self.ws.get(tag + '.y', (rows, D))
        mean = self.ws.get(tag + '.mean', (rows,), f32)
        rstd = self.ws.get(tag + '.rstd', (rows,), f32)
        if zsplice is not None:
            K.layernorm_fwd_z(x, zsplice[0], zsplice[1], self.P.f(name + '.weight'), self.P.f(name + '.bias'), y, mean,
                              rstd, rows, D)
        else:
            K.layernorm_fwd(x, self.P.f(name + '.weight'), self.P.f(name + '.bias'), y, mean, rstd, rows, D)
        return y, (x, mean, rstd)

    def _ln_bwd(self, name, dy, st, rows, dres, dx, dx_bf=None, bf_drop=None, zsplice=None, gelu=None):
        x, mean, rstd = st
        D = self.d
        wg = self.P.grad[self.P.offsets[name + '.weight'][0]:][:2 * D]
        if len(self._cs_pending) == COLSUM_MAX:
            self.flush_colsum()
        k, n1 = len(self._cs_pending), 1024 * 2 * D
        part = self.ws.get('ln.parts', (COLSUM_MAX * n1,), f32)[k * n1:(k + 1) * n1]
        if gelu is not None:
            K.layernorm_bwd_gelu(dy, x, self.P.f(name + '.weight'), mean, rstd, gelu, dx_bf, wg, rows, D, part,
                                 defer=self._cs_pending)
            return
        K.layernorm_bwd(dy, x, self.P.f(name + '.weight'), mean, rstd, dres, dx, dx_bf, wg, rows, D, part,
                        bf_drop=bf_drop, zsplice=zsplice, defer=self._cs_pending)

    def flush_zproj(self):
        if self._zp_pending:
            z_bf, dz, B, d, Z = self._zp_ctx
            K.zproj_bwd_multi(self._zp_pending, z_bf, dz, B, d, Z)
            self._zp_pending = []

    def flush_colsum(self):
        if self._cs_pending:
            K.colsum_multi(self._cs_pending)
            self._cs_pending = []

    def _job(self, dY, X, wname, rows, n_out, n_in, ldy=None, ldx=None, bias=None):
        bg = None
        if bias is not None:
            off = self.P.offsets[bias][0]
            bg = self.P.grad[off:off + n_out]
        return K.DwJob(dY, X, self.P.g(wname), rows, n_out, n_in, ldy, ldx, bg)

    def _dw(self, job):
        if self._dwq is not None and job.rows >= K.GROUP_MIN_ROWS:
            self._dwq.append(job)
        else:
            K.linear_dw(*job)

    def _head_dw_splits(self, V, d):
        env = int(os.environ.get('SVAE_HEAD_DW_SPLITS', '0') or 0)
        if env > 0:
            return env
        tiles = -(-V // 256) * -(-d // 256)
        ncu = self.ncu
        eff = lambda s: tiles * s / (ncu * -(-(tiles * s) // ncu))
        return 2 if tiles >= ncu and eff(2) > eff(1) + 0.1 else 1

    def _dw_pair(self, j0, j1):
        if self._dwq is not None:
            self._dw(j0)
            self._dw(j1)
        else:
            K.linear_dw_pair(j0, j1)

    def _bname(self, name, st):
        return f'{name}.{st["tag"]}' if self._dw_names else name

    def flush_dw(self):
        q, self._dw_jobs = self._dw_jobs, []
        k = 0
        for c in range(0, len(q), GROUP_MAX):
            jobs = q[c:c + GROUP_MAX]
            key = tuple((j.n_out, j.n_in, j.rows) for j in jobs)
            if key not in self._dwg_sched:
                self._dwg_sched[key] = K.group_schedule(key, self.ncu)
            for idx, splits, slab in self._dwg_sched[key]:
                if len(self._dwg_states) <= k:
                    self._dwg_states.append(K.DwGroupState(self.P.device))
                K.linear_dw_group([jobs[i] for i in idx], splits, self._dwg_states[k], slab=slab)
                k += 1

    def _db(self, dY, bname, rows, cols, ld=None):
        off = self.P.offsets[bname][0]
        K.colsum(dY, rows, cols, ld or cols, self.P.grad[off:off + cols])

    def layer_fwd(self, pre, x, B, Sx, L, pad, *, learned=0, cross=False, causal=False, ctx=None, heads, hd,
                  drop_p=0.0, seed=0, tag, out=None, window=0, out_bf=None, zsplice=None, ctx_ln=None):
        d, ws, P = self.d, self.ws, self.P
        rows_x = B * Sx
        rot = self.rot(max(Sx, L), window)
        st = {'pre': pre, 'B': B, 'Sx': Sx, 'L': L, 'learned': learned, 'cross': cross, 'causal': causal,
              'heads': heads, 'hd': hd, 'drop_p': drop_p, 'seed': seed, 'x': x, 'tag': tag, 'window': window}
        a = pre + 'attention.'
        h, st['ln_a'] = self._ln_fwd(pre + 'attn_layer_norm', x, rows_x, tag + '.ln_a', zsplice=zsplice)
        st['h'] = h
        pad_k = pad if Sx == L else None
        if learned:
            Lq = learned
            kv = ws.get(tag + '.kv', (rows_x, 2 * d))
            K.gemm(h, P.w(a + 'k_linear.weight'), kv, rows_x, 2 * d, d, epi=EPI_ROTARY_BF16,
                   bias=P.f(a + 'k_linear.bias'), rot=rot, rot_cols=d, rot_d=d, rot_seq=Sx)
            q = P.w(a + 'learned_queries').view(Lq, d)
            qargs = dict(sq=d, bq=0)
            kt, vt, sk = kv, kv[:, d:], 2 * d
            st['kv'] = kv
        else:
            Lq = Sx
            qkv = ws.get(tag + '.qkv', (rows_x, 3 * d))
            K.gemm(h, P.w(a + 'q_linear.weight'), qkv, rows_x, 3 * d, d, epi=EPI_ROTARY_BF16,
                   bias=P.f(a + 'q_linear.bias'), rot=rot, rot_cols=2 * d, rot_d=d, rot_seq=Sx)
            q = qkv
            qargs = dict(sq=3 * d, bq=Sx * 3 * d)
            kt, vt, sk = qkv[:, d:], qkv[:, 2 * d:], 3 * d
            st['qkv'] = qkv
        rows_q = B * Lq
        O = ws.get(tag + '.O', (rows_q, d))
        Ox = self._o_extra(tag + '.O', rows_q, d, Lq)
        lse = ws.get(tag + '.lse', (B, heads, Lq), f32)
        K.attention(q, kt, vt, O, lse, B=B, H=heads, Lq=Lq, Lk=Sx, hd=hd, so=d, bo=Lq * d, sk=sk, sv=sk,
                    bk=Sx * sk, bv=Sx * sk, key_pad=pad_k, causal=causal, window=window, **Ox, **qargs)
        st.update(O=O, Ox=Ox, lse=lse, Lq=Lq, pad_k=pad_k)
        resid = Lq == Sx
        x1 = ws.get(tag + '.x1', (rows_q, d), f32)
        K.gemm(O, P.w(a + 'output_linear.weight'), x1, rows_q, d, d, epi=EPI_F32,
               bias=P.f(a + 'output_linear.bias'), resid=x if resid else None, ldr=d)
        st['resid'] = resid
        st['x1'] = x1
        xc = x1
        if cross:
            c = pre + 'cross_attention.'
            rows_c = B * L
            if ctx_ln is not None:
                cx, st['ln_ctx'] = ctx_ln
                st['ctx_deferred'] = True
            else:
                cx, st['ln_ctx'] = self._ln_fwd(pre + 'context_layer_norm', ctx, rows_c, tag + '.ln_ctx')
            hq, st['ln_cross'] = self._ln_fwd(pre + 'cross_attn_layer_norm', x1, rows_q, tag + '.ln_cross')
            qc = ws.get(tag + '.qc', (rows_q, d))
            K.gemm(hq, P.w(c + 'q_linear.weight'), qc, rows_q, d, d, epi=EPI_ROTARY_BF16, bias=P.f(c + 'q_linear.bias'),
                   rot=rot, rot_cols=d, rot_d=d, rot_seq=Lq)
            kvc = ws.get(tag + '.kvc', (rows_c, 2 * d))
            K.gemm(cx, P.w(c + 'k_linear.weight'), kvc, rows_c, 2 * d, d, epi=EPI_ROTARY_BF16,
                   bias=P.f(c + 'k_linear.bias'), rot=rot, rot_cols=d, rot_d=d, rot_seq=L)
            Oc = ws.get(tag + '.Oc', (rows_q, d))
            Ocx = self._o_extra(tag + '.Oc', rows_q, d, Lq)
            lsec = ws.get(tag + '.lsec', (B, heads, Lq), f32)
            K.attention(qc, kvc, kvc[:, d:], Oc, lsec, B=B, H=heads, Lq=Lq, Lk=L, hd=hd, sq=d, bq=Lq * d, sk=2 * d,
                        sv=2 * d, bk=L * 2 * d, bv=L * 2 * d, so=d, bo=Lq * d, key_pad=pad, causal=False, **Ocx)
            st['Ocx'] = Ocx
            x2 = ws.get(tag + '.x2', (rows_q, d), f32)
            K.gemm(Oc, P.w(c + 'output_linear.weight'), x2, rows_q, d, d, epi=EPI_F32,
                   bias=P.f(c + 'output_linear.bias'), resid=x1, ldr=d)
            st.update(cx=cx, hq=hq, qc=qc, kvc=kvc, Oc=Oc, lsec=lsec, x2=x2, pad_ctx=pad)
            xc = x2
        h2, st['ln_f'] = self._ln_fwd(pre + 'ffn_layer_norm', xc, rows_q, tag + '.ln_f')
        gprime = ws.get(tag + '.gprime', (rows_q, 4 * d))
        f = ws.get(tag + '.f', (rows_q, 4 * d))
        K.gemm(h2, P.w(pre + 'ffn.0.weight'), f, rows_q, 4 * d, d, epi=EPI_GELU, bias=P.f(pre + 'ffn.0.bias'),
               aux=gprime, ldaux=4 * d)
        out = ws.get(tag + '.out', (rows_q, d), f32) if out is None else out
        K.gemm(f, P.w(pre + 'ffn.2.weight'), out, rows_q, d, 4 * d, epi=EPI_DROPOUT_RESID, resid=xc, ldr=d,
               drop_p=drop_p, seed=seed, aux=out_bf, ldaux=d if out_bf is not None else 0)
        st.update(h2=h2, gprime=gprime, f=f, xc=xc, rows_q=rows_q)
        return out, st

    def _o_extra(self, tag, rows_q, d, Lq):
        return dict(o_lo=self.ws.get(tag + 'lo', (rows_q, d)), so_lo=d, bo_lo=Lq * d)

    def _dq_part(self, B, H, Lq, Lk, hd, window=0):
        n = K.attn_dq_part_elems(B, H, Lq, Lk, hd, window)
        t = self.ws.bufs.get('b.dqpart')
        return t if t is not None and t.numel() >= n else self.ws.get('b.dqpart', (n,), f32)

    def layer_bwd(self, st, dout, dx_out, *, dx_accumulate=False, dctx=None, g2_ready=False, next_drop=None,
                  zsplice=None, next_st=None):
        d, ws, P = self.d, self.ws, self.P
        pre, B, Sx, L, Lq = st['pre'], st['B'], st['Sx'], st['L'], st['Lq']
        heads, hd = st['heads'], st['hd']
        rows_x, rows_q = B * Sx, st['rows_q']
        rot = self.rot(max(Sx, L), st['window'])
        a = pre + 'attention.'
        bn = lambda name: self._bname(name, st)
        self._dwq = self._dw_jobs if self._dw_names else None
        g2 = ws.get(bn('b.g2'), (rows_q, d))
        if not g2_ready:
            K.dropout_bwd_cast(dout, g2, st['drop_p'], st['seed'], rows_q, d)
        dpre = ws.get(bn('b.dpre'), (rows_q, 4 * d))
        K.gemm(g2, P.wT(pre + 'ffn.2.weight', d, 4 * d), dpre, rows_q, 4 * d, d, epi=EPI_GELU_BWD, aux=st['gprime'],
               ldaux=4 * d)
        self._dw_pair(self._job(g2, st['f'], pre + 'ffn.2.weight', rows_q, d, 4 * d),
                      self._job(dpre, st['h2'], pre + 'ffn.0.weight', rows_q, 4 * d, d, bias=pre + 'ffn.0.bias'))
        dh2 = ws.get('b.dh2', (rows_q, d))
        K.gemm(dpre, P.wT(pre + 'ffn.0.weight', 4 * d, d), dh2, rows_q, d, 4 * d, epi=EPI_BF16)
        dxc = ws.get('b.dxc', (rows_q, d), f32)
        gxc = ws.get(bn('b.gxc'), (rows_q, d))
        self._ln_bwd(pre + 'ffn_layer_norm', dh2, st['ln_f'], rows_q, dout, dxc, gxc)
        dx1, gx1 = dxc, gxc
        if st['cross']:
            c = pre + 'cross_attention.'
            rows_c = B * L
            dOc = ws.get('b.dO', (rows_q, d))
            delta = ws.get('b.delta', (B, heads, Lq), f32)
            K.gemm(gxc, P.wT(c + 'output_linear.weight', d, d), dOc, rows_q, d, d, epi=EPI_BF16)
            dqc = ws.get(bn('b.dqc'), (rows_q, d))
            dkvc = ws.get(bn('b.dkvc'), (rows_c, 2 * d))
            K.attention(st['qc'], st['kvc'], st['kvc'][:, d:], st['Oc'], st['lsec'], B=B, H=heads, Lq=Lq, Lk=L,
                        hd=hd, sq=d, bq=Lq * d, sk=2 * d, sv=2 * d, bk=L * 2 * d, bv=L * 2 * d, so=d, bo=Lq * d,
                        key_pad=st['pad_ctx'], causal=False, backward=True, dout=dOc, sdo=d, bdo=Lq * d, delta=delta,
                        dq_bf=dqc, ldq_bf=d, dk=dkvc, dv=dkvc[:, d:], sdk=2 * d, sdv=2 * d, bdk=L * 2 * d,
                        bdv=L * 2 * d, rot=rot, rot_d=d, **st['Ocx'], dq_part=self._dq_part(B, heads, Lq, L, hd))
            self._dw_pair(self._job(gxc, st['Oc'], c + 'output_linear.weight', rows_q, d, d,
                                    bias=c + 'output_linear.bias'),
                          self._job(dqc, st['hq'], c + 'q_linear.weight', rows_q, d, d, bias=c + 'q_linear.bias'))
            dhq = ws.get('b.dhq', (rows_q, d))
            K.gemm(dqc, P.wT(c + 'q_linear.weight', d, d), dhq, rows_q, d, d, epi=EPI_BF16)
            self._dw(self._job(dkvc, st['cx'], c + 'k_linear.weight', rows_c, 2 * d, d, bias=c + 'k_linear.bias'))
            dcx = ws.get('b.dcx.' + st['tag'] if st.get('ctx_deferred') else 'b.dcx', (rows_c, d))
            K.gemm(dkvc, P.wT(c + 'k_linear.weight', 2 * d, d), dcx, rows_c, d, 2 * d, epi=EPI_BF16)
            dx1 = ws.get('b.dx1', (rows_q, d), f32)
            gx1 = ws.get(bn('b.gx1'), (rows_q, d))
            self._ln_bwd(pre + 'cross_attn_layer_norm', dhq, st['ln_cross'], rows_q, dxc, dx1, gx1)
            if st.get('ctx_deferred'):
                st['dcx'] = dcx
            else:
                self._ln_bwd(pre + 'context_layer_norm', dcx, st['ln_ctx'], rows_c, dctx, dctx)
        wo_dw = self._job(gx1, st['O'], a + 'output_linear.weight', rows_q, d, d, bias=a + 'output_linear.bias')
        dO = ws.get('b.dO', (rows_q, d))
        delta = ws.get('b.delta', (B, heads, Lq), f32)
        K.gemm(gx1, P.wT(a + 'output_linear.weight', d, d), dO, rows_q, d, d, epi=EPI_BF16)
        if st['learned']:
            kv = st['kv']
            dq32 = ws.get('b.dq32', (B * Lq, d), f32)
            dkv = ws.get(bn('b.dkv'), (rows_x, 2 * d))
            K.attention(P.w(a + 'learned_queries').view(Lq, d), kv, kv[:, d:], st['O'], st['lse'], B=B, H=heads,
                        Lq=Lq, Lk=Sx, hd=hd, sq=d, bq=0, sk=2 * d, sv=2 * d, bk=Sx * 2 * d, bv=Sx * 2 * d, so=d,
                        bo=Lq * d, key_pad=st['pad_k'], causal=False, backward=True, dout=dO, sdo=d, bdo=Lq * d,
                        delta=delta, dq=dq32, bdq=Lq * d, dk=dkv, dv=dkv[:, d:], sdk=2 * d, sdv=2 * d,
                        bdk=Sx * 2 * d, bdv=Sx * 2 * d, rot=rot, rot_d=d, **st['Ox'],
                        dq_part=self._dq_part(B, heads, Lq, Sx, hd))
            K.colsum(dq32, B, Lq * d, Lq * d, P.g(a + 'learned_queries').view(-1))
            self._dw_pair(wo_dw, self._job(dkv, st['h'], a + 'k_linear.weight', rows_x, 2 * d, d,
                                           bias=a + 'k_linear.bias'))
            dh = ws.get('b.dh', (rows_x, d))
            K.gemm(dkv, P.wT(a + 'k_linear.weight', 2 * d, d), dh, rows_x, d, 2 * d, epi=EPI_BF16)
        else:
            qkv = st['qkv']
            dqkv = ws.get(bn('b.dqkv'), (rows_x, 3 * d))
            K.attention(qkv, qkv[:, d:], qkv[:, 2 * d:], st['O'], st['lse'], B=B, H=heads, Lq=Lq, Lk=Sx, hd=hd,
                        sq=3 * d, bq=Sx * 3 * d, sk=3 * d, sv=3 * d, bk=Sx * 3 * d, bv=Sx * 3 * d, so=d, bo=Lq * d,
                        key_pad=st['pad_k'], causal=st['causal'], window=st['window'], backward=True, dout=dO,
                        sdo=d, bdo=Lq * d, delta=delta, dq_bf=dqkv, ldq_bf=3 * d, dk=dqkv[:, d:], dv=dqkv[:, 2 * d:],
                        sdk=3 * d, sdv=3 * d, bdk=Sx * 3 * d, bdv=Sx * 3 * d, rot=rot, rot_d=d, **st['Ox'],
                        dq_part=self._dq_part(B, heads, Lq, Sx, hd, st['window']))
            self._dw_pair(wo_dw, self._job(dqkv, st['h'], a + 'q_linear.weight', rows_x, 3 * d, d,
                                           bias=a + 'q_linear.bias'))
            dh = ws.get('b.dh', (rows_x, d))
            K.gemm(dqkv, P.wT(a + 'q_linear.weight', 3 * d, d), dh, rows_x, d, 3 * d, epi=EPI_BF16)
        if st['resid']:
            self._ln_bwd(pre + 'attn_layer_norm', dh, st['ln_a'], rows_x, dx1, dx_out,
                         dx_bf=(ws.get(self._bname('b.g2', next_st or st), (rows_x, d)) if next_drop is not None
                                else None), bf_drop=next_drop,
                         zsplice=zsplice)
            if dx_accumulate:
                raise NotImplementedError('residual + accumulate is handled by the caller')
        else:
            self._ln_bwd(pre + 'attn_layer_norm', dh, st['ln_a'], rows_x, dx_out if dx_accumulate else None, dx_out)
        self._dwq = None

    def forward(self, ids, ntok, *, pad=True, eps=None, seed=0, kl_weight=1.0, dropout=0.1, need_logits=False):
        hp, d, ws, P = self.hp, self.d, self.ws, self.P
        if not ids.is_cuda:
            raise RuntimeError('VAEEngine needs device tensors (no CPU fallback)')
        P.sync_shadow()
        B, L = ids.shape
        T, V, Z, N = B * L, hp.vocab_size, hp.latent_depth, hp.num_latents
        ids32 = ws.get('ids', (B, L), torch.int32)
        padm = None
        if pad is not None and pad is not False:
            padm = ws.get('pad', (B, L), torch.uint8)
        labels = ws.get('labels', (B, L), torch.int32)
        ntok64 = ws.get('ntok', (B,), torch.int64)
        if (ids.dtype == torch.int64 and ids.is_contiguous() and isinstance(ntok, torch.Tensor) and ntok.is_cuda
                and ntok.dtype == torch.int64 and ntok.is_contiguous() and ntok.numel() == B
                and (padm is None or pad is True or (pad.dtype == torch.bool and pad.is_contiguous()))):
            K.prep_tokens(ids, pad if padm is not None else None, B, L, ids32, labels, padm, ntok, ntok64)
        else:
            ids32, padm = self._inputs(ids, pad)
            labels[:, :-1].copy_(ids32[:, 1:])
            labels[:, -1] = 0
            ntok64.copy_(ntok)
        sv = {'B': B, 'L': L, 'dropout': dropout, 'seed': seed}

        x_emb = ws.get('x_emb', (T, d), f32)
        K.embedding_fwd(ids32, P.f('input_layer.0.weight'), x_emb, T, d, out2=ws.get('x_dec0', (T, d), f32))

        enc_bf, stats, sv['enc_layers'] = self._encode(x_emb, B, L, padm, dropout, seed)

        zf = ws.get('z', (B, Z), f32)
        zb = ws.get('z_bf', (B, Z))
        eps_buf = ws.get('eps', (B, Z), f32)
        raw_kl = ws.get('raw_kl', (B,), f32)
        kl = ws.get('kl', (2,), f32)
        if eps is not None:
            eps_buf.copy_(eps.reshape(B, Z))
        K.reparam_fwd(stats, eps_buf if eps is not None else None, _mix_seed(seed, 7), ntok64, zf, zb, eps_buf,
                      raw_kl, kl, B, Z)
        sv.update(enc_bf=enc_bf, stats=stats, z_bf=zb, eps=eps_buf)

        xf, sv['dec_layers'] = self._decode(x_emb, zb, padm, B, L, dropout, seed, x_ready=True)

        hh, gp0, h0, ln_h = self._head_hidden(xf, T)
        nchunks, chunk_len = K.ce_chunking(B, L, V, CE_CHUNK_NUMEL)
        lse = ws.get('ce.lse', (T,), f32)
        row_loss = ws.get('ce.row_loss', (T,), f32)
        chunk_w = ws.get('ce.chunk_w', (max(8, nchunks),), f32)
        nll = ws.get('nll', (1,), f32)
        ntile = -(-V // 128)
        head = 'logits' if need_logits else self.head_mode
        W, bias = P.w('input_layer.0.weight'), P.f('output_layer.3.bias')
        logits = ws.get('logits', (T, V))
        probe = self.probe
        if probe is not None:
            e0 = torch.cuda.Event(enable_timing=True)
            e0.record()
        if head == 'prob':
            coff = ws.get('ce.off', (T,), f32)
            K.ce_label_logit(hh, W, bias, labels, T, d, coff)
            part = ws.get('ce.psum', (ntile, T), f32)
            K.gemm(hh, W, logits, T, V, d, epi=EPI_CE_PROB, bias=bias, aux=part, labels=labels, row_a=coff)
        else:
            coff = None
            part = ws.get('ce.part', (T, ntile, 2), f32)
            lab_logit = ws.get('ce.label_logit', (T,), f32)
            K.gemm(hh, W, logits, T, V, d, epi=EPI_CE_STATS, bias=bias, aux=part, labels=labels, label_logit=lab_logit)
        if probe is not None:
            e1 = torch.cuda.Event(enable_timing=True)
            e1.record()
            probe.append((e0, e1))
        if head == 'prob':
            sat = ws.get('ce.sat', (T + 1,), torch.int32)
            K.ce_prob_finalize(part, ntile, coff, labels, T, L, nchunks, chunk_len, lse, row_loss, chunk_w, nll,
                               fix=(hh, W, bias, logits, sat))
        else:
            K.ce_finalize(part, ntile, lab_logit, labels, T, L, nchunks, chunk_len, lse, row_loss, chunk_w, nll)
        sv.update(xf=xf, gp0=gp0, h0=h0, hh=hh, ln_h=ln_h, logits=logits, lse=lse, chunk_w=chunk_w,
                  nchunks=nchunks, chunk_len=chunk_len, labels=labels, ids32=ids32, ntok=ntok64, x_emb=x_emb,
                  row_loss=row_loss, head=head, coff=coff)
        loss = ws.get('loss', (1,), f32)
        K.step_scalars(kl_weight, nll=nll, kl=kl, loss=loss)
        self.saved = sv
        return {'loss': loss[0], 'nll': nll[0], 'kl': kl[0], 'train_kl': kl[1], 'raw_kl': raw_kl,
                'mu': stats[:, :Z], 'logvar': stats[:, Z:], 'stats': stats, 'kl_buf': kl, 'z': zf, 'eps': eps_buf,
                'logits': logits if need_logits else None,
                'ce_saturated': sat[0] if head == 'prob' else None}

    def weighted_nll(self, tok_w):
        sv = self.saved
        out = torch.empty(1, dtype=f32, device=self.P.device)
        B, L = sv['B'], sv['L']
        K.ce_weighted_nll(sv['row_loss'], sv['labels'], tok_w, B * L, L, sv['nchunks'], sv['chunk_len'], out)
        return out[0]

    def _encode(self, x_emb, B, L, padm, dropout, seed):
        hp, d, ws, P = self.hp, self.d, self.ws, self.P
        N, Z = hp.num_latents, hp.latent_depth
        lay = []
        z, st = self.layer_fwd('encoder.first_layer.', x_emb, B, L, L, padm, learned=N, heads=self.He, hd=64,
                               drop_p=dropout, seed=_mix_seed(seed, 1000), tag='e0')
        lay.append(st)
        nmid = hp.enc_layers - 2
        cxs = self._ctx_ln_fwd(x_emb, B * L, nmid) if P.ctx_batched else [None] * nmid
        for j in range(nmid):
            z, st = self.layer_fwd(f'encoder.middle_layers.{j}.', z, B, N, L, padm, cross=True, ctx=x_emb,
                                   heads=self.He, hd=64, drop_p=dropout, seed=_mix_seed(seed, 1001 + j), tag=f'e{j + 1}',
                                   ctx_ln=cxs[j])
            lay.append(st)
        enc, st = self.layer_fwd('encoder.bottleneck.', z, B, N, L, padm, learned=1, heads=self.He, hd=64,
                                 drop_p=dropout, seed=_mix_seed(seed, 1999), tag='eb')
        lay.append(st)
        enc_bf = ws.get('enc_bf', (B, d))
        K.cast_bf16(enc, enc_bf)
        stats = ws.get('stats', (B, 2 * Z), f32)
        K.gemm(enc_bf, P.w('q_of_z_given_x.linear.weight'), stats, B, 2 * Z, d, epi=EPI_F32,
               bias=P.f('q_of_z_given_x.linear.bias'))
        return enc_bf, stats, lay

    def _ctx_ln_fwd(self, x, rows, nmid):
        D, ws, P = self.d, self.ws, self.P
        mean = ws.get('ctx.ln.mean', (rows,), f32)
        rstd = ws.get('ctx.ln.rstd', (rows,), f32)
        out = []
        for j0 in range(0, nmid, LN_MULTI_MAX):
            js = range(j0, min(nmid, j0 + LN_MULTI_MAX))
            names = [f'encoder.middle_layers.{j}.context_layer_norm' for j in js]
            ys = [ws.get(f'e{j + 1}.ln_ctx.y', (rows, D)) for j in js]
            K.layernorm_fwd_multi(x, [P.f(n + '.weight') for n in names], [P.f(n + '.bias') for n in names], ys, mean,
                                  rstd, rows, D)
            out += [(y, (x, mean, rstd)) for y in ys]
        return out

    def _ctx_ln_bwd(self, sts, dctx):
        D, P = self.d, self.P
        for j0 in range(0, len(sts), LN_MULTI_MAX):
            grp = sts[j0:j0 + LN_MULTI_MAX]
            x, mean, rstd = grp[0]['ln_ctx']
            rows = x.shape[0]
            names = [g['pre'] + 'context_layer_norm' for g in grp]
            wgs = [P.grad[P.offsets[n + '.weight'][0]:][:2 * D] for n in names]
            n1 = 1024 * 2 * D
            if len(self._cs_pending) + len(grp) > COLSUM_MAX:
                self.flush_colsum()
            k = len(self._cs_pending)
            part = self.ws.get('ln.parts', (COLSUM_MAX * n1,), f32)[k * n1:(k + len(grp)) * n1]
            K.layernorm_bwd_multi([g['dcx'] for g in grp], x, [P.f(n + '.weight') for n in names], mean, rstd, dctx,
                                  dctx, wgs, rows, D, part, defer=self._cs_pending)

    def _inputs(self, ids, pad):
        B, L = ids.shape
        ids32 = self.ws.get('ids', (B, L), torch.int32)
        ids32.copy_(ids)
        padm = None
        if pad is not None and pad is not False:
            padm = self.ws.get('pad', (B, L), torch.uint8)
            padm.copy_(ids.eq(0) if pad is True else pad)
        return ids32, padm

    def mutual_info(self, out, eps=None, num_samples=10):
        stats = out['stats']
        B, Z = stats.shape[0], stats.shape[1] // 2
        if eps is not None:
            eps = eps.to(stats.device, f32).reshape(num_samples, B, Z).contiguous()
        ws = self.ws.get('mi_ws', (2 * num_samples * B,), f32)
        res = torch.empty((), dtype=f32, device=stats.device)
        seed = int(torch.randint(0, 2 ** 62, (1,)).item())
        K.mutual_info(stats, out['kl_buf'], B, Z, seed, res, ws, eps=eps, S=num_samples)
        return res

    def posterior(self, ids, pad=True):
        if not ids.is_cuda:
            raise RuntimeError('VAEEngine needs device tensors (no CPU fallback)')
        self.P.sync_shadow()
        B, L = ids.shape
        ids32, padm = self._inputs(ids, pad)
        x_emb = self.ws.get('x_emb', (B * L, self.d), f32)
        K.embedding_fwd(ids32, self.P.f('input_layer.0.weight'), x_emb, B * L, self.d)
        _, stats, _ = self._encode(x_emb, B, L, padm, 0.0, 0)
        return stats

    def seq_log_prob(self, x_emb, labels, z, pad=None, max_tokens=32768):
        hp, d, ws, P = self.hp, self.d, self.ws, self.P
        if not x_emb.is_cuda:
            raise RuntimeError('VAEEngine needs device tensors (no CPU fallback)')
        P.sync_shadow()
        G, Bt, L = x_emb.shape[0], x_emb.shape[1], x_emb.shape[2]
        V, Z = hp.vocab_size, hp.latent_depth
        out = torch.empty(G, Bt, dtype=f32, device=P.device)
        ntile = -(-V // 128)
        if Bt * L <= max_tokens:
            gstep, bstep = max(1, max_tokens // (Bt * L)), Bt
        else:
            gstep, bstep = 1, max(1, max_tokens // L)
        for g0 in range(0, G, gstep):
            g1 = min(G, g0 + gstep)
            for b0 in range(0, Bt, bstep):
                b1 = min(Bt, b0 + bstep)
                ng, nb = g1 - g0, b1 - b0
                B = ng * nb
                T = B * L
                padm = None
                if pad is not None:
                    padm = ws.get('pad', (B, L), torch.uint8)
                    padm.view(ng, nb, L).copy_(pad[g0:g1, b0:b1])
                lab = ws.get('labels', (B, L), torch.int32)
                lab.view(ng, nb, L)[:, :, :-1].copy_(labels[g0:g1, b0:b1])
                lab[:, -1] = 0
                xe = ws.get('x_emb', (T, d), f32)
                xe.view(ng, nb, L, d).copy_(x_emb[g0:g1, b0:b1])
                zf = ws.get('z_f32', (B, Z), f32)
                zf.view(ng, nb, Z).copy_(z[g0:g1, b0:b1])
                zb = ws.get('z_bf', (B, Z))
                K.cast_bf16(zf, zb)
                xf, _ = self._decode(xe, zb, padm, B, L, 0.0, 0)
                hh = self._head_hidden(xf, T)[0]
                part = ws.get('ce.part', (T, ntile, 2), f32)
                lab_logit = ws.get('ce.label_logit', (T,), f32)
                K.gemm(hh, P.w('input_layer.0.weight'), None, T, V, d, epi=EPI_CE_STATS,
                       bias=P.f('output_layer.3.bias'), aux=part, labels=lab, label_logit=lab_logit)
                res = ws.get('seq_lp', (B,), f32)
                K.ce_seq_logprob(part, ntile, lab_logit, lab, T, L, res)
                out[g0:g1, b0:b1].copy_(res.view(ng, nb))
        return out

    def _head_hidden(self, xf, T):
        d, ws, P = self.d, self.ws, self.P
        gp0 = ws.get('h0_gprime', (T, d))
        h0 = ws.get('h0', (T, d))
# ... 19 lines not shown
            segs = [(P.w(f'z_projections.{i}.weight'), P.f(f'z_projections.{i}.bias'), zall[i])
                    for i in range(hp.num_layers)]
            for c0 in range(0, len(segs), ZPROJ_MAX):
                K.zproj_fwd_multi(segs[c0:c0 + ZPROJ_MAX], zb, B, d, Z)
        for i in range(hp.num_layers):
            last = i + 1 == hp.num_layers
            if not zf_batch:
                K.gemm(zb, P.w(f'z_projections.{i}.weight'), xs, B, d, Z, ldc=L * d, epi=EPI_F32,
                       bias=P.f(f'z_projections.{i}.bias'))
            xs, st = self.layer_fwd(f'decoder_layers.{i}.', xs, B, L, L, padm, causal=True, heads=self.H,
                                    hd=self.hd, drop_p=dropout, seed=_mix_seed(seed, i), tag=f'd{i}',
                                    out=ws.get(f'x_dec{i + 1}', (T, d), f32), window=self.window,
                                    out_bf=xf if last else None, zsplice=(zall[i], L) if zf_batch else None)
            dec.append(st)
        return xf, dec

    def reconstruct_f32(self, x_emb, z, pad=None):
        hp, d, P = self.hp, self.d, self.P
        dev = P.device
        B, L = x_emb.shape[0], x_emb.shape[1]
        T, V, Z, H, hd = B * L, hp.vocab_size, hp.latent_depth, self.H, self.hd
        rot = self.rot(L, self.window)
        padm = None
        if pad is not None:
            padm = torch.empty(B, L, dtype=torch.uint8, device=dev)
            padm.copy_(pad)
        x = x_emb.reshape(T, d).clone()
        h = torch.empty(T, d, device=dev)
        qkv = torch.empty(T, 3 * d, device=dev)
        o = torch.empty(T, d, device=dev)
        x1 = torch.empty(T, d, device=dev)
        f = torch.empty(T, 4 * d, device=dev)
        for i in range(hp.num_layers):
            pre = f'decoder_layers.{i}.'
            a = pre + 'attention.'
            K.gemm_f32(z, P.f(f'z_projections.{i}.weight'), x, B, d, Z, ldc=L * d, bias=P.f(f'z_projections.{i}.bias'))
            K.layernorm_fwd_f32(x, P.f(pre + 'attn_layer_norm.weight'), P.f(pre + 'attn_layer_norm.bias'), h, T, d)
            K.gemm_f32(h, P.f(a + 'q_linear.weight'), qkv, T, 3 * d, d, epi=EPI_ROTARY_BF16, bias=P.f(a + 'q_linear.bias'),
                       rot=rot, rot_cols=2 * d, rot_d=d, rot_seq=L)
            K.attention_f32(qkv, qkv[:, d:], qkv[:, 2 * d:], o, B=B, H=H, Lq=L, Lk=L, hd=hd, sq=3 * d, sk=3 * d,
                            sv=3 * d, so=d, bq=L * 3 * d, bk=L * 3 * d, bv=L * 3 * d, bo=L * d, key_pad=padm, causal=True,
                            window=self.window)
            K.gemm_f32(o, P.f(a + 'output_linear.weight'), x1, T, d, d, bias=P.f(a + 'output_linear.bias'), resid=x, ldr=d)
            K.layernorm_fwd_f32(x1, P.f(pre + 'ffn_layer_norm.weight'), P.f(pre + 'ffn_layer_norm.bias'), h, T, d)
            K.gemm_f32(h, P.f(pre + 'ffn.0.weight'), f, T, 4 * d, d, epi=EPI_GELU, bias=P.f(pre + 'ffn.0.bias'))
            K.gemm_f32(f, P.f(pre + 'ffn.2.weight'), x, T, d, 4 * d, resid=x1, ldr=d)
        h0 = torch.empty(T, d, device=dev)
        K.gemm_f32(x, P.f('output_layer.0.weight'), h0, T, d, d, epi=EPI_GELU, bias=P.f('output_layer.0.bias'))
        K.layernorm_fwd_f32(h0, P.f('output_layer.2.weight'), P.f('output_layer.2.bias'), h, T, d)
        logits = torch.empty(B, L, V, device=dev)
        K.gemm_f32(h, P.f('input_layer.0.weight'), logits, T, V, d, bias=P.f('output_layer.3.bias'))
        return logits

    def reconstruct(self, x_emb, z, pad=None):
        hp, d, ws, P = self.hp, self.d, self.ws, self.P
        P.sync_shadow()
        B, L = x_emb.shape[0], x_emb.shape[1]
        T, V, Z = B * L, hp.vocab_size, hp.latent_depth
        padm = None
        if pad is not None:
            padm = ws.get('pad', (B, L), torch.uint8)
            padm.copy_(pad)
        zb = ws.get('z_bf', (B, Z))
        K.cast_bf16(z, zb)
        xf, _ = self._decode(x_emb.reshape(T, d), zb, padm, B, L, 0.0, 0)
        hh = self._head_hidden(xf, T)[0]
        logits = torch.empty(B, L, V, dtype=bf16, device=P.device)
        K.gemm(hh, P.w('input_layer.0.weight'), logits, T, V, d, epi=EPI_BF16, bias=P.f('output_layer.3.bias'))
        return logits

    def backward(self, gloss, kl_weight, ready=None):
        sv, hp, d, ws, P = self.saved, self.hp, self.d, self.ws, self.P
        user_ready = ready

        def ready(end):
            if user_ready is not None:
                self.flush_colsum()
                self.flush_zproj()
                user_ready(end)
        if sv is None:
            raise RuntimeError('backward() without a saved forward')
        self._dwq, self._dw_jobs = None, []
        self._dw_names = self.dw_group and user_ready is None
        B, L = sv['B'], sv['L']
        T, V, Z, N = B * L, hp.vocab_size, hp.latent_depth, hp.num_latents
        gs = ws.get('gscale', (2,), f32)
        gl = gloss.reshape(1)
        if gl.is_cuda and gl.dtype == f32:
            K.step_scalars(kl_weight, gloss=gl, gs=gs)
        else:
            gs[0:1].copy_(gl)
            gs[1:2].copy_(gl * kl_weight)

        logits = sv['logits']
        dhh = ws.get('b.dhh', (T, d))
        nch, clen = sv['nchunks'], sv['chunk_len']
        if sv['head'] == 'prob':
            hh = sv['hh']
            hh_r = ws.get('b.hh_r', (T, d))
            r_t = ws.get('b.ce_r', (T,), f32)
            q_t = ws.get('b.ce_q', (T,), f32)
            dbias = P.g('output_layer.3.bias')
            K.ce_prob_bwd_prep(hh, sv['lse'], sv['coff'], sv['chunk_w'], sv['labels'], gs[0:1], T, L, nch, clen, d, hh_r,
                               r_t, q_t, dbias)
            s = self._head_dw_splits(V, d)
            if s == 1:
                K.gemm(logits, hh_r, P.g('input_layer.0.weight'), V, d, T, a_t=True, b_t=True, lda=V, ldb=d, ldc=d,
                       epi=EPI_F32_ACC, a_rowsum=dbias, k_weight=r_t)
            else:
                slab = ws.get('b.head_dw_slab', (s * V * d,), f32)
                K.gemm(logits, hh_r, P.g('input_layer.0.weight'), V, d, T, a_t=True, b_t=True, lda=V, ldb=d, ldc=d,
                       epi=EPI_F32_ATOMIC, splits=s, aux=slab, a_rowsum=dbias, k_weight=r_t)
            W = P.w('input_layer.0.weight')
            K.gemm(logits, P.wT('input_layer.0.weight', V, d), dhh, T, d, V, epi=EPI_ROWSCALE_GATHER,
                   labels=sv['labels'], row_a=r_t, row_b=q_t, gather=W, ldg=d)
            sv['ce_q'] = q_t
        else:
            K.ce_grad(logits, V, sv['lse'], sv['chunk_w'], sv['labels'], gs[0:1], T, V, L, nch, clen)
            self._dw(self._job(logits, sv['hh'], 'input_layer.0.weight', T, V, d, bias='output_layer.3.bias'))
            K.gemm(logits, P.wT('input_layer.0.weight', V, d), dhh, T, d, V, epi=EPI_BF16)
        dpre0 = ws.get('b.dpre0', (T, d))
        self._ln_bwd('output_layer.2', dhh, sv['ln_h'], T, None, None, dx_bf=dpre0, gelu=sv['gp0'])
        self._dw(self._job(dpre0, sv['xf'], 'output_layer.0.weight', T, d, d, bias='output_layer.0.bias'))
        dx = ws.get('b.dx_dec', (T, d), f32)
        top = sv['dec_layers'][-1]
        g2_pre = top['rows_q'] == T
        K.gemm(dpre0, P.wT('output_layer.0.weight', d, d), dx, T, d, d, epi=EPI_F32,
               aux=ws.get(self._bname('b.g2', top), (T, d)) if g2_pre else None, ldaux=d if g2_pre else 0,
               drop_p=top['drop_p'] if g2_pre else 0.0, seed=top['seed'] if g2_pre else 0)
        ready(P.end('output_layer.3.bias'))

        dz = ws.get('b.dz', (B, Z), f32, zero=True)
        dzh = ws.get('b.dzh', (B, d), f32)
        dzh_bf = ws.get('b.dzh_bf', (B, d))
        dx_prev = ws.get('b.dx_prev', (T, d), f32)
        g2_ready = g2_pre
        for i in reversed(range(hp.num_layers)):
            st = sv['dec_layers'][i]
            nd = None
            if i > 0 and st['resid'] and sv['dec_layers'][i - 1]['rows_q'] == T:
                nst = sv['dec_layers'][i - 1]
                nd = (nst['drop_p'], nst['seed'], L)
            dzh_i = ws.get('b.dzh_all', (hp.num_layers, B, d), f32)[i]
            zs = (L, dzh_i, None) if st['resid'] and st['rows_q'] == T else None
            self.layer_bwd(st, dx, dx_prev, g2_ready=g2_ready, next_drop=nd, zsplice=zs,
                           next_st=sv['dec_layers'][i - 1] if nd is not None else None)
            g2_ready = nd is not None
            wz, bz = f'z_projections.{i}.weight', f'z_projections.{i}.bias'
            if zs is not None:
                if len(self._zp_pending) == ZPROJ_MAX:
                    self.flush_zproj()
                self._zp_ctx = (sv['z_bf'], dz, B, d, Z)
                self._zp_pending.append((dzh_i, P.w(wz), P.g(wz), P.g(bz)))
            else:
                self.flush_zproj()
                K.extract_rows(dx_prev, d, T, L, d, dzh)
                K.cast_bf16(dzh, dzh_bf)
                self._dw(self._job(dzh_bf, sv['z_bf'], wz, B, d, Z, bias=bz))
                K.gemm(dzh_bf, P.w(wz), dz, B, Z, d, b_t=True, epi=EPI_F32_ATOMIC, splits=max(1, min(8, d // 64)))
            ready(P.end(f'z_projections.{i}.bias'))
            dx, dx_prev = dx_prev, dx
        self.flush_zproj()
        dx_emb = dx

        dstats = ws.get('b.dstats', (B, 2 * Z), f32)
        K.reparam_bwd(sv['stats'], sv['eps'], dz, sv['ntok'], gs[1:2], dstats, B, Z)
        dstats_bf = ws.get('b.dstats_bf', (B, 2 * Z))
        K.cast_bf16(dstats, dstats_bf)
        self._dw(self._job(dstats_bf, sv['enc_bf'], 'q_of_z_given_x.linear.weight', B, 2 * Z, d))
        self._db(dstats, 'q_of_z_given_x.linear.bias', B, 2 * Z)
        denc = ws.get('b.denc', (B, d), f32)
        K.gemm(dstats_bf, P.w('q_of_z_given_x.linear.weight'), denc, B, d, 2 * Z, b_t=True, epi=EPI_F32)
        ready(P.end('q_of_z_given_x.linear.bias'))

        enc = sv['enc_layers']
        dcur = denc
        for k in reversed(range(1, len(enc))):
            st = enc[k]
            nxt = ws.get(f'b.denc{k}', (B * N, d), f32)
            self.layer_bwd(st, dcur, nxt, dctx=dx_emb)
            ready(P.end(st['pre'] + 'ffn_layer_norm.bias'))
            dcur = nxt
        deferred = [st for st in enc if st.get('ctx_deferred')]
        if deferred:
            self._ctx_ln_bwd(deferred[::-1], dx_emb)
            ready(P.end(deferred[0]['pre'] + 'context_layer_norm.bias'))
        st0 = enc[0]
        if st0['resid']:
            tmp = ws.get('b.dfirst', (T, d), f32)
            self.layer_bwd(st0, dcur, tmp)
            self.flush_dw()
            K.embedding_bwd(sv['ids32'], tmp, P.g('input_layer.0.weight'), T, d)
        else:
            self.layer_bwd(st0, dcur, dx_emb, dx_accumulate=True)
            self.flush_dw()

        ready(P.end('encoder.first_layer.ffn_layer_norm.bias'))
        self._embedding_bwd(sv, dx_emb, T, d)
        ready(P.n_live)
        self.flush_colsum()

    def _embedding_bwd(self, sv, dx, T, d):
        if sv['head'] == 'prob':
            K.embedding_bwd_ce(sv['ids32'], dx, self.P.g('input_layer.0.weight'), T, d, sv['L'], sv['hh'], sv['ce_q'])
        else:
            K.embedding_bwd(sv['ids32'], dx, self.P.g('input_layer.0.weight'), T, d)
```

sparse-vae_amd/sparse_vae/kernels.py:

```python
import ctypes
import os
from typing import NamedTuple

import torch

from . import _native as N
from ._native import lib, check, ptr, stream

bf16, f32 = torch.bfloat16, torch.float32

_gemm_desc = N.GemmDesc()


def _dev(*ts):
    for t in ts:
        if t is not None and not t.is_cuda:
            raise RuntimeError('libsvae kernels need device tensors (no CPU fallback)')


def gemm(A, B, C, M, N_, K, *, a_t=False, b_t=False, lda=None, ldb=None, ldc=None, epi=N.EPI_BF16, bias=None,
         resid=None, ldr=0, aux=None, ldaux=0, alpha=1.0, splits=1, drop_p=0.0, seed=0, rot=None, rot_cols=0,
         rot_d=0, rot_seq=0, labels=None, label_logit=None, batch=1, sA=0, sB=0, sC=0, a_rowsum=None, k_weight=None,
         row_a=None, row_b=None, gather=None, ldg=0, delta=None, delta_o32=None, ld_o32=0, delta_hd=0, delta_seq=0):
    d = _fill_desc(_gemm_desc, A, B, C, M, N_, K, a_t=a_t, b_t=b_t, lda=lda, ldb=ldb, ldc=ldc, epi=epi, bias=bias,
# ... 237 lines not shown
                                D, stream()), 'svae_resid_ln_fwd')


def layernorm_fwd(x, w, b, y, mean, rstd, rows, D):
    _dev(x, w, b, y, mean, rstd)
    check(lib.svae_layernorm_fwd(x.data_ptr(), 0 if x.dtype == f32 else 1, w.data_ptr(), b.data_ptr(), y.data_ptr(),
                                 mean.data_ptr(), rstd.data_ptr(), rows, D, stream()), 'svae_layernorm_fwd')


def layernorm_bwd(dy, x, w, mean, rstd, dres, dx, dx_bf, wgrad2, rows, D, part_ws, bf_drop=None, zsplice=None,
                  defer=None):
    nblk = lib.svae_layernorm_nblk(rows)
    part = part_ws[: nblk * 2 * D]
    if bf_drop is None and zsplice is None:
        check(lib.svae_layernorm_bwd(dy.data_ptr(), x.data_ptr(), 0 if x.dtype == f32 else 1, w.data_ptr(),
                                     mean.data_ptr(), rstd.data_ptr(), ptr(dres), dx.data_ptr(), ptr(dx_bf),
                                     part.data_ptr(), nblk, rows, D, 0, stream()), 'svae_layernorm_bwd')
    else:
        p, seed, zmod = bf_drop if bf_drop is not None else (0.0, 0, 0)
        zm, zrow, zrow_bf = zsplice if zsplice is not None else (0, None, None)
        check(lib.svae_layernorm_bwd_drop(dy.data_ptr(), x.data_ptr(), 0 if x.dtype == f32 else 1, w.data_ptr(),
                                          mean.data_ptr(), rstd.data_ptr(), ptr(dres), dx.data_ptr(), ptr(dx_bf),
                                          part.data_ptr(), nblk, rows, D, int(zm), float(p),
                                          int(seed) & 0xFFFFFFFFFFFFFFFF, int(zmod), ptr(zrow), ptr(zrow_bf),
                                          stream()), 'svae_layernorm_bwd_drop')
    if defer is not None:
        defer.append((part, nblk, 2 * D, 2 * D, wgrad2))
    else:
        colsum(part, nblk, 2 * D, 2 * D, wgrad2, accumulate=True)


def layernorm_bwd_gelu(dy, x, w, mean, rstd, gp, out_bf, wgrad2, rows, D, part_ws, defer=None):
    nblk = lib.svae_layernorm_nblk(rows)
    part = part_ws[: nblk * 2 * D]
    check(lib.svae_layernorm_bwd_gelu(dy.data_ptr(), x.data_ptr(), 0 if x.dtype == f32 else 1, w.data_ptr(),
                                      mean.data_ptr(), rstd.data_ptr(), gp.data_ptr(), out_bf.data_ptr(),
                                      part.data_ptr(), nblk, rows, D, stream()), 'svae_layernorm_bwd_gelu')
    if defer is not None:
        defer.append((part, nblk, 2 * D, 2 * D, wgrad2))
    else:
        colsum(part, nblk, 2 * D, 2 * D, wgrad2, accumulate=True)


def _ptrs(ts):
    return (ctypes.c_void_p * N.LN_MULTI_MAX)(*[t.data_ptr() for t in ts])


def layernorm_fwd_multi(x, ws, bs, ys, mean, rstd, rows, D):
    n = len(ys)
    assert 0 < n <= N.LN_MULTI_MAX and len(ws) == n and len(bs) == n and x.dtype == f32
    _dev(x, mean, rstd, *ws, *bs, *ys)
    check(lib.svae_layernorm_fwd_multi(x.data_ptr(), _ptrs(ws), _ptrs(bs), _ptrs(ys), n, mean.data_ptr(),
                                       rstd.data_ptr(), rows, D, stream()), 'svae_layernorm_fwd_multi')


def layernorm_bwd_multi(dys, x, ws, mean, rstd, dres, dx, wgrads, rows, D, part_ws, defer=None):
    n = len(dys)
    assert 0 < n <= N.LN_MULTI_MAX and len(ws) == n and len(wgrads) == n and x.dtype == f32
    _dev(x, mean, rstd, dx, *dys, *ws)
    nblk = lib.svae_layernorm_nblk(rows)
    parts = [part_ws[j * nblk * 2 * D:(j + 1) * nblk * 2 * D] for j in range(n)]
    assert parts[-1].numel() == nblk * 2 * D
    check(lib.svae_layernorm_bwd_multi(_ptrs(dys), x.data_ptr(), _ptrs(ws), mean.data_ptr(), rstd.data_ptr(),
                                       ptr(dres), dx.data_ptr(), _ptrs(parts), nblk, n, rows, D, stream()),
          'svae_layernorm_bwd_multi')
    for part, wg in zip(parts, wgrads):
        if defer is not None:
            defer.append((part, nblk, 2 * D, 2 * D, wg))
        else:
            colsum(part, nblk, 2 * D, 2 * D, wg, accumulate=True)


_colsum_segs = (N.ColsumSeg * N.COLSUM_MAX)()


def colsum_multi(segs):
    assert 0 < len(segs) <= N.COLSUM_MAX
    for i, (inp, rows, cols, ld, out) in enumerate(segs):
        _dev(inp, out)
        assert inp.dtype == f32 and out.dtype == f32
        _colsum_segs[i].inp, _colsum_segs[i].out = inp.data_ptr(), out.data_ptr()
        _colsum_segs[i].ld, _colsum_segs[i].rows, _colsum_segs[i].cols = ld, rows, cols
    check(lib.svae_colsum_multi(ctypes.addressof(_colsum_segs), len(segs), stream()), 'svae_colsum_multi')


def colsum(inp, rows, cols, ld, out, accumulate=True):
    check(lib.svae_colsum(inp.data_ptr(), 0 if inp.dtype == f32 else 1, rows, cols, ld, out.data_ptr(),
                          int(accumulate), stream()), 'svae_colsum')


_attn_desc = N.AttnDesc()


def attention(q, k, v, o, lse, *, B, H, Lq, Lk, hd, sq, sk, sv, so, bq, bk, bv, bo, key_pad=None, causal=False,
              window=0, scale=None, backward=False, dout=None, sdo=0, bdo=0, delta=None, dq=None, bdq=0, dk=None, dv=None,
              sdk=0, sdv=0, bdk=0, bdv=0, rot=None, rot_d=0, o32=None, so32=0, bo32=0, dq_part=None, dq_bf=None,
              ldq_bf=0, delta_ready=False, o_lo=None, so_lo=0, bo_lo=0):
    d = _attn_desc
    d.q, d.k, d.v, d.o = q.data_ptr(), k.data_ptr(), v.data_ptr(), o.data_ptr()
    d.sq, d.sk, d.sv, d.so, d.bq, d.bk, d.bv, d.bo = sq, sk, sv, so, bq, bk, bv, bo
    d.key_pad = ptr(key_pad)
    d.lse = lse.data_ptr()
    d.B, d.H, d.Lq, d.Lk, d.hd, d.causal = B, H, Lq, Lk, hd, int(causal)
    d.window = int(window)
    d.delta_ready = int(bool(delta_ready))
    d.scale = hd ** -0.5 if scale is None else scale
    d.o32, d.so32, d.bo32 = ptr(o32), so32, bo32
    d.o_lo, d.so_lo, d.bo_lo = ptr(o_lo), so_lo, bo_lo
    if backward:
        d.fwd_ws, d.fwd_ws_elems = None, 0
        d.dout, d.sdo, d.bdo = dout.data_ptr(), sdo, bdo
        d.delta, d.bdq = delta.data_ptr(), bdq
        d.dk, d.dv, d.sdk, d.sdv, d.bdk, d.bdv = dk.data_ptr(), dv.data_ptr(), sdk, sdv, bdk, bdv
        d.rot_tab, d.rot_d = ptr(rot), rot_d
        if dq_part is None:
            dq_part = torch.empty(attn_dq_part_elems(B, H, Lq, Lk, hd, window), device=q.device, dtype=torch.float32)
        assert dq_part.numel() >= attn_dq_part_elems(B, H, Lq, Lk, hd, window) and dq_part.dtype == torch.float32
        d.dq_part, d.dq_bf, d.ldq_bf = dq_part.data_ptr(), ptr(dq_bf), ldq_bf
        d.dq = ptr(dq)
        check(lib.svae_attn_bwd(ctypes.byref(d), stream()), 'svae_attn_bwd')
    else:
        d.dout = None
        n = lib.svae_attn_fwd_ws_elems(B, H, Lq, Lk, hd, int(causal), int(window))
        if n > 0:
            ws = _fwd_workspace(n, q.device)
            d.fwd_ws, d.fwd_ws_elems = ws.data_ptr(), ws.numel()
        else:
            d.fwd_ws, d.fwd_ws_elems = None, 0
        check(lib.svae_attn_fwd(ctypes.byref(d), stream()), 'svae_attn_fwd')


_fwd_ws = {}


def _fwd_workspace(n, device):
    t = _fwd_ws.get(device)
    if t is None or t.numel() < n:
        t = torch.empty(n, dtype=torch.float32, device=device)
        _fwd_ws[device] = t
    return t


def attn_dq_part_elems(B, H, Lq, Lk, hd, window=0):
    return lib.svae_attn_dq_part_elems_w(B, H, Lq, Lk, hd, int(window))


def dq_finalize(dq, out, ldo, rows, D, rot=None, seq=0):
    check(lib.svae_dq_finalize(dq.data_ptr(), out.data_ptr(), ldo, rows, D, ptr(rot), seq, stream()),
          'svae_dq_finalize')


def embedding_fwd(ids, table, out, rows, D, out2=None):
    if out2 is not None:
        _dev(ids, table, out, out2)
        check(lib.svae_embedding_fwd_dual(ids.data_ptr(), table.data_ptr(), out.data_ptr(), out2.data_ptr(), rows, D,
                                          stream()), 'svae_embedding_fwd_dual')
        return
    check(lib.svae_embedding_fwd(ids.data_ptr(), table.data_ptr(), out.data_ptr(), None, rows, D, stream()),
          'svae_embedding_fwd')


def embedding_bwd(ids, dout, dtable, rows, D):
    check(lib.svae_embedding_bwd(ids.data_ptr(), dout.data_ptr(), dtable.data_ptr(), rows, D, stream()),
          'svae_embedding_bwd')


def reparam_fwd(stats, eps, seed, ntok, z, z_bf, eps_out, raw_kl, kl_out, B, Z):
    check(lib.svae_reparam_kl_fwd(stats.data_ptr(), ptr(eps), seed & 0xFFFFFFFFFFFFFFFF, ntok.data_ptr(),
                                  z.data_ptr(), ptr(z_bf), ptr(eps_out), raw_kl.data_ptr(), kl_out.data_ptr(), B, Z,
                                  stream()), 'svae_reparam_kl_fwd')


def reparam_bwd(stats, eps, dz, ntok, gkl, dstats, B, Z):
    check(lib.svae_reparam_kl_bwd(stats.data_ptr(), eps.data_ptr(), ptr(dz), ntok.data_ptr(), gkl.data_ptr(),
                                  dstats.data_ptr(), B, Z, stream()), 'svae_reparam_kl_bwd')


def ce_red_ws(device, nchunks):
    n = max(1024, lib.svae_ce_red_ws_elems(nchunks))
    t = _ce_red.get(device)
    if t is None or t.numel() < n:
        t = _ce_red[device] = torch.empty(n, dtype=f32, device=device)
    return t


_ce_red = {}


def ce_finalize(part, ntile, label_logit, labels, rows, seq, nchunks, chunk_len, lse, row_loss, chunk_w, nll):
    assert chunk_w.numel() >= nchunks and chunk_w.dtype == f32
    red = ce_red_ws(part.device, nchunks)
    check(lib.svae_ce_finalize(part.data_ptr(), ntile, label_logit.data_ptr(), labels.data_ptr(), rows, seq,
                               nchunks, chunk_len, lse.data_ptr(), row_loss.data_ptr(), chunk_w.data_ptr(),
                               nll.data_ptr(), red.data_ptr(), stream()), 'svae_ce_finalize')


def ce_weighted_nll(row_loss, labels, tok_w, rows, seq, nchunks, chunk_len, out):
    _dev(row_loss, labels, tok_w, out)
    assert tok_w.dtype == f32 and tok_w.is_contiguous()
    red = ce_red_ws(row_loss.device, nchunks)
    check(lib.svae_ce_weighted_nll(row_loss.data_ptr(), labels.data_ptr(), tok_w.data_ptr(), rows, seq, nchunks,
                                   chunk_len, out.data_ptr(), red.data_ptr(), stream()), 'svae_ce_weighted_nll')


def ce_chunking(B, L, V, chunk_numel=2 ** 30):
    chunks = -(-(B * (L - 1) * V) // chunk_numel)
    chunk_len = -(-(L - 1) // chunks)
    return -(-(L - 1) // chunk_len), chunk_len


def ce_label_logit(hh, W, bias, labels, rows, D, out):
    _dev(hh, W, labels, out)
    check(lib.svae_ce_label_logit(hh.data_ptr(), hh.stride(0), W.data_ptr(), W.stride(0), ptr(bias), labels.data_ptr(),
                                  rows, D, out.data_ptr(), stream()), 'svae_ce_label_logit')


def ce_prob_finalize(part, ntile, row_off, labels, rows, seq, nchunks, chunk_len, lse, row_loss, chunk_w, nll,
                     fix=None):
    assert chunk_w.numel() >= nchunks and chunk_w.dtype == f32
    red = ce_red_ws(part.device, nchunks)
    if fix is None:
        check(lib.svae_ce_prob_finalize(part.data_ptr(), ntile, row_off.data_ptr(), labels.data_ptr(), rows, seq,
                                        nchunks, chunk_len, lse.data_ptr(), row_loss.data_ptr(), chunk_w.data_ptr(),
                                        nll.data_ptr(), red.data_ptr(), stream()), 'svae_ce_prob_finalize')
        return
    hh, W, bias, P, sat = fix
    _dev(hh, W, P, sat)
    assert sat.dtype == torch.int32 and sat.numel() >= rows + 1 and P.shape[0] >= rows
    check(lib.svae_ce_prob_finalize_fix(part.data_ptr(), ntile, row_off.data_ptr(), labels.data_ptr(), rows, seq,
                                        nchunks, chunk_len, lse.data_ptr(), row_loss.data_ptr(), chunk_w.data_ptr(),
                                        nll.data_ptr(), red.data_ptr(), hh.data_ptr(), hh.stride(0), W.data_ptr(),
                                        W.stride(0), ptr(bias), P.data_ptr(), P.stride(0), W.shape[0], hh.shape[1],
                                        sat.data_ptr(), stream()), 'svae_ce_prob_finalize_fix')


def ce_prob_bwd_prep(hh, lse, row_off, chunk_w, labels, gscale, rows, seq, nchunks, chunk_len, D, hh_out, r_out,
                     q_out, dbias=None):
    _dev(hh, lse, row_off, chunk_w, labels, gscale, hh_out, r_out, q_out)
    check(lib.svae_ce_prob_bwd_prep(hh.data_ptr(), hh.stride(0), lse.data_ptr(), row_off.data_ptr(),
                                    chunk_w.data_ptr(), labels.data_ptr(), gscale.data_ptr(), rows, seq, nchunks,
                                    chunk_len, D, hh_out.data_ptr(), r_out.data_ptr(), q_out.data_ptr(), ptr(dbias),
                                    stream()), 'svae_ce_prob_bwd_prep')


def embedding_bwd_ce(ids, dout, dtable, rows, D, seq, hh, q):
    check(lib.svae_embedding_bwd_ce(ids.data_ptr(), dout.data_ptr(), dtable.data_ptr(), rows, D, seq, hh.data_ptr(),
                                    q.data_ptr(), stream()), 'svae_embedding_bwd_ce')


def mutual_info(stats, kl, B, Z, seed, out, ws, eps=None, S=10):
    _dev(stats, kl, out, ws)
    assert ws.numel() >= 2 * S * B
    check(lib.svae_mutual_info(stats.data_ptr(), ptr(eps), seed & 0xFFFFFFFFFFFFFFFF, kl.data_ptr(), B, Z, S,
                               ws.data_ptr(), out.data_ptr(), stream()), 'svae_mutual_info')


def ce_seq_logprob(part, ntile, label_logit, labels, rows, seq, out):
    _dev(part, label_logit, labels, out)
    assert out.dtype == f32 and out.numel() == rows // seq and out.is_contiguous()
    check(lib.svae_ce_seq_logprob(part.data_ptr(), ntile, label_logit.data_ptr(), labels.data_ptr(), rows, seq,
                                  out.data_ptr(), stream()), 'svae_ce_seq_logprob')


def ce_grad(logits, ld, lse, chunk_w, labels, gscale, rows, V, seq, nchunks, chunk_len, dbias=None):
    check(lib.svae_ce_grad(logits.data_ptr(), ld, lse.data_ptr(), chunk_w.data_ptr(), labels.data_ptr(),
                           gscale.data_ptr(), ptr(dbias), rows, V, seq, nchunks, chunk_len, stream()), 'svae_ce_grad')


def prep_tokens(ids, pad, B, L, ids32, labels, padm=None, ntok=None, ntok_out=None):
    assert ids.dtype == torch.int64 and ids.is_contiguous() and ids.numel() == B * L
    mode = 0 if pad is None or pad is False else (1 if pad is True else 2)
    if mode == 2:
        assert pad.dtype == torch.bool and pad.is_contiguous() and pad.numel() == B * L
    if ntok is not None:
        assert ntok.dtype == torch.int64 and ntok.is_contiguous() and ntok.numel() == B
    _dev(ids, ids32, labels)
    check(lib.svae_prep_tokens(ids.data_ptr(), pad.data_ptr() if mode == 2 else None, mode, B, L, ids32.data_ptr(),
                               labels.data_ptr(), ptr(padm), ptr(ntok), ptr(ntok_out), stream()), 'svae_prep_tokens')


def step_scalars(kl_weight, nll=None, kl=None, loss=None, gloss=None, gs=None):
    for t in (nll, kl, loss, gloss, gs):
        assert t is None or (t.is_cuda and t.dtype == f32)
    check(lib.svae_step_scalars(ptr(nll), ptr(kl), ptr(gloss), float(kl_weight), ptr(loss), ptr(gs), stream()),
          'svae_step_scalars')


def dropout_bwd_cast(g, out, p, seed, rows, cols, ld_in=None):
    check(lib.svae_dropout_bwd_cast(g.data_ptr(), out.data_ptr(), p, seed & 0xFFFFFFFFFFFFFFFF, rows * cols, cols,
                                    ld_in or cols, stream()), 'svae_dropout_bwd_cast')


def cast_bf16(x, out, n=None):
    check(lib.svae_cast_bf16(x.data_ptr(), out.data_ptr(), n if n is not None else x.numel(), stream()),
          'svae_cast_bf16')


def transpose_blocks(src, dst, table, nblocks, total_tiles):
    check(lib.svae_transpose_blocks(src.data_ptr(), dst.data_ptr(), table.data_ptr(), nblocks, total_tiles, stream()),
          'svae_transpose_blocks')


def gelu_bwd(dx, gp, out, n):
    check(lib.svae_gelu_bwd(dx.data_ptr(), gp.data_ptr(), out.data_ptr(), n, stream()), 'svae_gelu_bwd')


def extract_rows(x, ld, rows, mod, D, out):
    check(lib.svae_extract_rows(x.data_ptr(), ld, rows, mod, D, out.data_ptr(), stream()), 'svae_extract_rows')


def zproj_bwd(g, z, W, dW, db, dz, B, d, Z):
    _dev(g, z, W, dW, db, dz)
    assert g.dtype == f32 and z.dtype == bf16 and W.dtype == bf16 and dW.dtype == f32 and dz.dtype == f32
    check(lib.svae_zproj_bwd(g.data_ptr(), z.data_ptr(), W.data_ptr(), dW.data_ptr(), db.data_ptr(), dz.data_ptr(),
                             B, d, Z, stream()), 'svae_zproj_bwd')


_zfwd_segs = (N.ZprojFwdSeg * N.ZPROJ_MAX)()


def zproj_fwd_multi(segs, z, B, d, Z):
    assert 0 < len(segs) <= N.ZPROJ_MAX
    _dev(z)
    assert z.dtype == bf16 and z.is_contiguous()
    for i, (W, bias, out) in enumerate(segs):
# ... 483 lines not shown
```

Before: 2.794 million tokens/s.

## Fuse small tail kernels into CE finalize, bwd prep, reparam and colsum list

Result: no change. 2.806 million tokens/s (median of 6 runs) (+0.4%).

```diff
diff --git a/include/svae.h b/include/svae.h
--- a/include/svae.h
+++ b/include/svae.h
@@ -101,6 +101,8 @@
   int32_t rows, cols;
 } svae_colsum_seg;
 int svae_colsum_multi(const svae_colsum_seg* segs, int32_t n, svae_stream_t stream);
+#define SVAE_COLSUM_LIST_MAX 32
+int svae_colsum_list(const svae_colsum_seg* segs, int32_t n, svae_stream_t stream);
 
 typedef struct svae_attn_desc {
   const void* q; const void* k; const void* v; void* o;
@@ -150,6 +152,9 @@
                         int32_t Z, svae_stream_t stream);
 int svae_reparam_kl_bwd(const float* stats, const float* eps, const float* dz, const int64_t* ntok,
                         const float* gkl, float* dstats, int32_t B, int32_t Z, svae_stream_t stream);
+int svae_reparam_kl_bwd_bf(const float* stats, const float* eps, const float* dz, const int64_t* ntok,
+                           const float* gkl, float* dstats, void* dstats_bf, int32_t B, int32_t Z,
+                           svae_stream_t stream);
 
 int svae_ce_finalize(const float* part, int32_t ntile, const float* label_logit, const int32_t* labels,
                      int32_t rows, int32_t seq, int32_t nchunks, int32_t chunk_len, float* lse, float* row_loss,
@@ -176,6 +181,17 @@
                           const int32_t* labels, const float* gscale, int32_t rows, int32_t seq, int32_t nchunks,
                           int32_t chunk_len, int32_t D, void* hh_out, float* r_out, float* q_out, float* dbias,
                           svae_stream_t stream);
+int svae_ce_prob_finalize_tail(const float* part, int32_t ntile, float* row_off, const int32_t* labels, int32_t rows,
+                               int32_t seq, int32_t nchunks, int32_t chunk_len, float* lse, float* row_loss,
+                               float* chunk_w, float* nll_out, float* red_ws, const void* hh, int64_t ldh,
+                               const void* W, int64_t ldw, const float* bias, void* P, int64_t ldp, int32_t V,
+                               int32_t D, int32_t* sat_ws, const float* kl, float kl_weight, float* loss_out,
+                               svae_stream_t stream);
+int svae_ce_prob_bwd_prep_gs(const void* hh, int64_t ldh, const float* lse, const float* row_off,
+                             const float* chunk_w, const int32_t* labels, const float* gloss, float kl_weight,
+                             float* gs, float* zero_out, int32_t zero_n, int32_t rows, int32_t seq, int32_t nchunks,
+                             int32_t chunk_len, int32_t D, void* hh_out, float* r_out, float* q_out, float* dbias,
+                             svae_stream_t stream);
 int svae_embedding_bwd_ce(const int32_t* ids, const float* dout, float* dtable, int32_t rows, int32_t D, int32_t seq,
                           const void* hh, const float* q, svae_stream_t stream);
 
diff --git a/sparse-vae_amd/csrc/elementwise.hip b/sparse-vae_amd/csrc/elementwise.hip
--- a/sparse-vae_amd/csrc/elementwise.hip
+++ b/sparse-vae_amd/csrc/elementwise.hip
@@ -44,6 +44,22 @@
     if (qp != 0.f) g -= qp * (float)hp[c];
     atomicAdd(dtable + dst + c, g);
   }
+}
+
+__device__ __forceinline__ bool last_block_arrive(unsigned* __restrict__ counter, unsigned nblocks) {
+  asm volatile("s_waitcnt vmcnt(0)" ::: "memory");
+  const unsigned t = __hip_atomic_fetch_add(counter, 1u, __ATOMIC_RELAXED, __HIP_MEMORY_SCOPE_AGENT);
+  if (t != nblocks - 1) return false;
+  __builtin_amdgcn_fence(__ATOMIC_ACQUIRE, "agent");
+  asm volatile("s_waitcnt vmcnt(0)" ::: "memory");
+  __hip_atomic_store(counter, 0u, __ATOMIC_RELAXED, __HIP_MEMORY_SCOPE_AGENT);
+  return true;
+}
+__device__ __forceinline__ void partial_store(float* p, float v) {
+  __hip_atomic_store(p, v, __ATOMIC_RELAXED, __HIP_MEMORY_SCOPE_AGENT);
+}
+__device__ __forceinline__ float partial_load(const float* p) {
+  return __hip_atomic_load(p, __ATOMIC_RELAXED, __HIP_MEMORY_SCOPE_AGENT);
 }
 
 constexpr int REPARAM_WAVES = 16;
@@ -116,7 +132,7 @@
 __global__ __launch_bounds__(256) void reparam_bwd_kernel(const float* __restrict__ stats, const float* __restrict__ eps,
                                                           const float* __restrict__ dz, const long long* __restrict__ ntok,
                                                           const float* __restrict__ gkl, float* __restrict__ dstats,
-                                                          int B, int Z) {
+                                                          int B, int Z, bf16* __restrict__ dstats_bf = nullptr) {
   const int i = blockIdx.x * 256 + threadIdx.x;
   if (i >= B * Z) return;
   const int b = i / Z, j = i % Z;
@@ -125,8 +141,13 @@
   const float var = __expf(lv), sd = sqrtf(var);
   const float w = gkl[0] / ((float)B * (float)ntok[b]);
   const float g = dz ? dz[i] : 0.f;
-  dstats[(long long)b * 2 * Z + j] = g + w * mu;
-  dstats[(long long)b * 2 * Z + Z + j] = g * eps[i] * sd * 0.5f + w * 0.5f * (var - 1.0f);
+  const float dmu = g + w * mu, dlv = g * eps[i] * sd * 0.5f + w * 0.5f * (var - 1.0f);
+  dstats[(long long)b * 2 * Z + j] = dmu;
+  dstats[(long long)b * 2 * Z + Z + j] = dlv;
+  if (dstats_bf) {
+    dstats_bf[(long long)b * 2 * Z + j] = f2bf(dmu);
+    dstats_bf[(long long)b * 2 * Z + Z + j] = f2bf(dlv);
+  }
 }
 
 __global__ __launch_bounds__(256) void ce_rows_kernel(const float* __restrict__ part, int ntile,
@@ -179,7 +200,7 @@
 __global__ __launch_bounds__(256) void ce_prob_rows_kernel(const float* __restrict__ part, int ntile,
                                                            const float* __restrict__ off, const int* __restrict__ labels,
                                                            int rows, float* __restrict__ lse, float* __restrict__ row_loss,
-                                                           int* __restrict__ sat) {
+                                                           int* __restrict__ sat, int* __restrict__ sat_cnt = nullptr) {
   __shared__ float red[8][33];
   const int r = threadIdx.x & 31, sl = threadIdx.x >> 5;
   const int row = blockIdx.x * 32 + r;
@@ -204,17 +225,18 @@
   const float l = live ? __logf(se) : 0.f;
   lse[row] = live ? off[row] + l : 0.f;
   row_loss[row] = l;
-  if (sat && live && !(se < 0x1p100f)) sat[1 + atomicAdd(sat, 1)] = row;
+  if (sat && live && !(se < 0x1p100f)) sat[1 + atomicAdd(sat_cnt ? sat_cnt : sat, 1)] = row;
 }
 
 __global__ __launch_bounds__(256) void ce_prob_fixup_kernel(const int* __restrict__ sat, const bf16* __restrict__ hh,
                                                             long long ldh, const bf16* __restrict__ W, long long ldw,
                                                             const float* __restrict__ bias, bf16* __restrict__ P,
                                                             long long ldp, int V, int D, float* __restrict__ off,
-                                                            float* __restrict__ lse, float* __restrict__ row_loss) {
+                                                            float* __restrict__ lse, float* __restrict__ row_loss,
+                                                            const int* __restrict__ sat_cnt = nullptr) {
   __shared__ float h[1024];
   __shared__ float red[4];
-  const int n = sat[0];
+  const int n = sat_cnt ? sat_cnt[0] : sat[0];
   const int lane = threadIdx.x & 63, w = threadIdx.x >> 6;
   for (int i = blockIdx.x; i < n; i += gridDim.x) {
     const int row = sat[1 + i];
@@ -270,7 +292,17 @@
                                                                const float* __restrict__ gscale, int rows, int seq,
                                                                int nchunks, int chunk_len, int D,
                                                                bf16* __restrict__ hh_out, float* __restrict__ r_out,
-                                                               float* __restrict__ q_out, float* __restrict__ dbias) {
+                                                               float* __restrict__ q_out, float* __restrict__ dbias,
+                                                               float kw = 0.f, float* __restrict__ gs_out = nullptr,
+                                                               float* __restrict__ zero_out = nullptr, int zero_n = 0) {
+  if (gs_out && blockIdx.x == 0) {
+    if (threadIdx.x == 0) {
+      const float g = gscale[0];
+      gs_out[0] = g;
+      gs_out[1] = __fmul_rn(g, kw);
+    }
+    for (int i = threadIdx.x; i < zero_n; i += 256) zero_out[i] = 0.f;
+  }
   const int lane = threadIdx.x & 63;
   const int row = blockIdx.x * 4 + (threadIdx.x >> 6);
   if (row >= rows) return;
@@ -397,11 +429,46 @@
 constexpr int CE_RED_BLOCKS = 64;
 constexpr int CE_MAX_CHUNKS = 1024;
 
+template <bool TAIL>
+__device__ __forceinline__ float ce_reduce_final_block(const float* part, int nchunks, float* __restrict__ chunk_w,
+                                                       float* mean) {
+  for (int k = threadIdx.x; k < nchunks; k += 256) {
+    float ts = 0.f, tc = 0.f;
+    for (int b = 0; b < CE_RED_BLOCKS; ++b) {
+      const float* p = part + ((long long)k * CE_RED_BLOCKS + b) * 2;
+      ts += TAIL ? partial_load(p) : p[0];
+      tc += TAIL ? partial_load(p + 1) : p[1];
+    }
+    mean[k] = ts / tc;
+    if (chunk_w) chunk_w[k] = 1.0f / (tc * (float)nchunks);
+  }
+  __syncthreads();
+  float nll = 0.f;
+  if (threadIdx.x == 0) {
+    for (int j = 0; j < nchunks; ++j) nll += mean[j];
+    nll /= nchunks;
+  }
+  return nll;
+}
+
+struct CeTail {
+  float* chunk_w;
+  float* nll_out;
+  const float* kl;
+  float* loss_out;
+  int* sat;
+  int* sat_cnt;
+  unsigned* done;
+  float kw;
+};
+
+template <bool TAIL>
 __global__ __launch_bounds__(256) void ce_reduce_part_kernel(const float* __restrict__ row_loss,
                                                              const int* __restrict__ labels,
                                                              const float* __restrict__ tok_w, int rows, int seq,
-                                                             int nchunks, int chunk_len, float* __restrict__ part) {
-  __shared__ float red[8];
+                                                             int nchunks, int chunk_len, float* __restrict__ part,
+                                                             CeTail tail = {}) {
+  __shared__ float red[TAIL ? CE_MAX_CHUNKS : 8];
   const int ch = blockIdx.y;
   const int p0 = ch * chunk_len;
   const int clen = ch == nchunks - 1 ? seq - p0 : chunk_len;
@@ -422,29 +489,37 @@
   __syncthreads();
   if (threadIdx.x == 0) {
     float* o = part + ((long long)ch * CE_RED_BLOCKS + blockIdx.x) * 2;
-    o[0] = (red[0] + red[1]) + (red[2] + red[3]);
-    o[1] = (red[4] + red[5]) + (red[6] + red[7]);
+    const float s0 = (red[0] + red[1]) + (red[2] + red[3]), s1 = (red[4] + red[5]) + (red[6] + red[7]);
+    if constexpr (TAIL) {
+      partial_store(o, s0);
+      partial_store(o + 1, s1);
+    } else {
+      o[0] = s0;
+      o[1] = s1;
+    }
+  }
+  if constexpr (TAIL) {
+    __shared__ int s_last;
+    if (threadIdx.x == 0) s_last = last_block_arrive(tail.done, gridDim.x * gridDim.y);
+    __syncthreads();
+    if (!s_last) return;
+    const float nll = ce_reduce_final_block<true>(part, nchunks, tail.chunk_w, red);
+    if (threadIdx.x == 0) {
+      tail.nll_out[0] = nll;
+      tail.loss_out[0] = __fadd_rn(nll, __fmul_rn(tail.kw, tail.kl[0]));
+      if (tail.sat) {
+        tail.sat[0] = tail.sat_cnt[0];
+        tail.sat_cnt[0] = 0;
+      }
+    }
   }
 }
 
 __global__ __launch_bounds__(256) void ce_reduce_final_kernel(const float* __restrict__ part, int nchunks,
                                                               float* __restrict__ chunk_w, float* __restrict__ nll_out) {
   __shared__ float mean[CE_MAX_CHUNKS];
-  for (int k = threadIdx.x; k < nchunks; k += 256) {
-    float ts = 0.f, tc = 0.f;
-    for (int b = 0; b < CE_RED_BLOCKS; ++b) {
-      ts += part[((long long)k * CE_RED_BLOCKS + b) * 2];
-      tc += part[((long long)k * CE_RED_BLOCKS + b) * 2 + 1];
-    }
-    mean[k] = ts / tc;
-    if (chunk_w) chunk_w[k] = 1.0f / (tc * (float)nchunks);
-  }
-  __syncthreads();
-  if (threadIdx.x == 0) {
-    float nll = 0.f;
-    for (int j = 0; j < nchunks; ++j) nll += mean[j];
-    nll_out[0] = nll / nchunks;
-  }
+  const float nll = ce_reduce_final_block<false>(part, nchunks, chunk_w, mean);
+  if (threadIdx.x == 0) nll_out[0] = nll;
 }
 
 #define CE_U 2
@@ -835,9 +910,40 @@
     hipLaunchKernelGGL(ce_prob_fixup_kernel, dim3(64), dim3(256), 0, s, (const int*)sat_ws, (const bf16*)hh,
                        (long long)ldh, (const bf16*)W, (long long)ldw, bias, (bf16*)P, (long long)ldp, V, D, row_off,
                        lse, row_loss);
-  hipLaunchKernelGGL(ce_reduce_part_kernel, dim3(CE_RED_BLOCKS, nchunks), dim3(256), 0, s, row_loss, labels,
+  hipLaunchKernelGGL(ce_reduce_part_kernel<false>, dim3(CE_RED_BLOCKS, nchunks), dim3(256), 0, s, row_loss, labels,
                      (const float*)nullptr, rows, seq, nchunks, chunk_len, red_ws);
   hipLaunchKernelGGL(ce_reduce_final_kernel, dim3(1), dim3(256), 0, s, red_ws, nchunks, chunk_w, nll_out);
+  SVAE_LAUNCH_CHECK();
+  return SVAE_OK;
+}
+
+SVAE_EXPORT int svae_ce_prob_finalize_tail(const float* part, int32_t ntile, float* row_off, const int32_t* labels,
+                                           int32_t rows, int32_t seq, int32_t nchunks, int32_t chunk_len, float* lse,
+                                           float* row_loss, float* chunk_w, float* nll_out, float* red_ws,
+                                           const void* hh, int64_t ldh, const void* W, int64_t ldw, const float* bias,
+                                           void* P, int64_t ldp, int32_t V, int32_t D, int32_t* sat_ws,
+                                           const float* kl, float kl_weight, float* loss_out, svae_stream_t stream) {
+  if (!part || !row_off || !labels || !lse || !row_loss || !chunk_w || !nll_out || !red_ws || !sat_ws || !kl || !loss_out)
+    return SVAE_EINVAL;
+  if (rows <= 0 || ntile <= 0 || seq <= 0 || rows % seq || nchunks <= 0 || nchunks > CE_MAX_CHUNKS ||
+      chunk_len <= 0 || (long long)(nchunks - 1) * chunk_len >= seq)
+    return SVAE_EINVAL;
+  if (!hh || !W || !P || V <= 0 || D <= 0 || D > 1024 || D % 8 || ldh % 8 || ldw % 8 ||
+      (((uintptr_t)hh | (uintptr_t)W) & 15))
+    return SVAE_EINVAL;
+  hipStream_t s = (hipStream_t)stream;
+  int* sat = (int*)sat_ws;
+  int* cnt = sat + rows + 1;
+  hipLaunchKernelGGL(ce_prob_rows_kernel, dim3((rows + 31) / 32), dim3(256), 0, s, part, ntile, row_off, labels, rows,
+                     lse, row_loss, sat, cnt);
+  hipLaunchKernelGGL(ce_prob_fixup_kernel, dim3(64), dim3(256), 0, s, (const int*)sat, (const bf16*)hh, (long long)ldh,
+                     (const bf16*)W, (long long)ldw, bias, (bf16*)P, (long long)ldp, V, D, row_off, lse, row_loss,
+                     (const int*)cnt);
+  CeTail tail;
+  tail.chunk_w = chunk_w; tail.nll_out = nll_out; tail.kl = kl; tail.loss_out = loss_out;
+  tail.sat = sat; tail.sat_cnt = cnt; tail.done = (unsigned*)(sat + rows + 2); tail.kw = kl_weight;
+  hipLaunchKernelGGL(ce_reduce_part_kernel<true>, dim3(CE_RED_BLOCKS, nchunks), dim3(256), 0, s, row_loss, labels,
+                     (const float*)nullptr, rows, seq, nchunks, chunk_len, red_ws, tail);
   SVAE_LAUNCH_CHECK();
   return SVAE_OK;
 }
@@ -856,6 +962,23 @@
   return SVAE_OK;
 }
 
+SVAE_EXPORT int svae_ce_prob_bwd_prep_gs(const void* hh, int64_t ldh, const float* lse, const float* row_off,
+                                         const float* chunk_w, const int32_t* labels, const float* gloss,
+                                         float kl_weight, float* gs, float* zero_out, int32_t zero_n, int32_t rows,
+                                         int32_t seq, int32_t nchunks, int32_t chunk_len, int32_t D, void* hh_out,
+                                         float* r_out, float* q_out, float* dbias, svae_stream_t stream) {
+  if (!hh || !lse || !row_off || !chunk_w || !labels || !gloss || !gs || gs == gloss || !hh_out || !r_out || !q_out)
+    return SVAE_EINVAL;
+  if (rows <= 0 || seq <= 0 || nchunks <= 0 || chunk_len <= 0 || D <= 0 || D % 8 || ldh % 8) return SVAE_EINVAL;
+  if (((uintptr_t)hh | (uintptr_t)hh_out) & 15) return SVAE_EINVAL;
+  if (zero_n < 0 || (zero_n > 0 && !zero_out)) return SVAE_EINVAL;
+  hipLaunchKernelGGL(ce_prob_bwd_prep_kernel, dim3((rows + 3) / 4), dim3(256), 0, (hipStream_t)stream, (const bf16*)hh,
+                     (long long)ldh, lse, row_off, chunk_w, labels, gloss, rows, seq, nchunks, chunk_len, D,
+                     (bf16*)hh_out, r_out, q_out, dbias, kl_weight, gs, zero_out, (int)zero_n);
+  SVAE_LAUNCH_CHECK();
+  return SVAE_OK;
+}
+
 SVAE_EXPORT int svae_reparam_kl_fwd(const float* stats, const float* eps, uint64_t seed, const int64_t* ntok, float* z,
                                     void* z_bf, float* eps_out, float* raw_kl, float* kl_out, int32_t B, int32_t Z,
                                     svae_stream_t stream) {
@@ -871,6 +994,16 @@
   if (!stats || !eps || !ntok || !gkl || !dstats || B <= 0 || Z <= 0) return SVAE_EINVAL;
   hipLaunchKernelGGL(reparam_bwd_kernel, dim3((B * Z + 255) / 256), dim3(256), 0, (hipStream_t)stream, stats, eps, dz,
                      (const long long*)ntok, gkl, dstats, B, Z);
+  SVAE_LAUNCH_CHECK();
+  return SVAE_OK;
+}
+
+SVAE_EXPORT int svae_reparam_kl_bwd_bf(const float* stats, const float* eps, const float* dz, const int64_t* ntok,
+                                       const float* gkl, float* dstats, void* dstats_bf, int32_t B, int32_t Z,
+                                       svae_stream_t stream) {
+  if (!stats || !eps || !ntok || !gkl || !dstats || !dstats_bf || B <= 0 || Z <= 0) return SVAE_EINVAL;
+  hipLaunchKernelGGL(reparam_bwd_kernel, dim3((B * Z + 255) / 256), dim3(256), 0, (hipStream_t)stream, stats, eps, dz,
+                     (const long long*)ntok, gkl, dstats, B, Z, (bf16*)dstats_bf);
   SVAE_LAUNCH_CHECK();
   return SVAE_OK;
 }
@@ -885,7 +1018,7 @@
   hipStream_t s = (hipStream_t)stream;
   hipLaunchKernelGGL(ce_rows_kernel, dim3((rows + 3) / 4), dim3(256), 0, s, part, ntile, label_logit, labels, rows, lse,
                      row_loss);
-  hipLaunchKernelGGL(ce_reduce_part_kernel, dim3(CE_RED_BLOCKS, nchunks), dim3(256), 0, s, row_loss, labels,
+  hipLaunchKernelGGL(ce_reduce_part_kernel<false>, dim3(CE_RED_BLOCKS, nchunks), dim3(256), 0, s, row_loss, labels,
                      (const float*)nullptr, rows, seq, nchunks, chunk_len, red_ws);
   hipLaunchKernelGGL(ce_reduce_final_kernel, dim3(1), dim3(256), 0, s, red_ws, nchunks, chunk_w, nll_out);
   SVAE_LAUNCH_CHECK();
@@ -900,7 +1033,7 @@
       (long long)(nchunks - 1) * chunk_len >= seq)
     return SVAE_EINVAL;
   hipStream_t s = (hipStream_t)stream;
-  hipLaunchKernelGGL(ce_reduce_part_kernel, dim3(CE_RED_BLOCKS, nchunks), dim3(256), 0, s, row_loss, labels, tok_w, rows,
+  hipLaunchKernelGGL(ce_reduce_part_kernel<false>, dim3(CE_RED_BLOCKS, nchunks), dim3(256), 0, s, row_loss, labels, tok_w, rows,
                      seq, nchunks, chunk_len, red_ws);
   hipLaunchKernelGGL(ce_reduce_final_kernel, dim3(1), dim3(256), 0, s, red_ws, nchunks, (float*)nullptr, out);
   SVAE_LAUNCH_CHECK();
diff --git a/sparse-vae_amd/csrc/layernorm.hip b/sparse-vae_amd/csrc/layernorm.hip
--- a/sparse-vae_amd/csrc/layernorm.hip
+++ b/sparse-vae_amd/csrc/layernorm.hip
@@ -513,15 +513,17 @@
   }
 }
 
+template <int CAP>
 struct ColsumSegs {
-  const float* in[SVAE_COLSUM_MAX];
-  float* out[SVAE_COLSUM_MAX];
-  long long ld[SVAE_COLSUM_MAX];
-  int rows[SVAE_COLSUM_MAX], cols[SVAE_COLSUM_MAX], rps[SVAE_COLSUM_MAX], colblocks[SVAE_COLSUM_MAX];
-  int first[SVAE_COLSUM_MAX + 1];
+  const float* in[CAP];
+  float* out[CAP];
+  long long ld[CAP];
+  int rows[CAP], cols[CAP], rps[CAP], colblocks[CAP];
+  int first[CAP + 1];
   int n;
 };
-__global__ __launch_bounds__(256) void colsum_multi_kernel(ColsumSegs sg) {
+template <int CAP>
+__global__ __launch_bounds__(256) void colsum_multi_kernel(ColsumSegs<CAP> sg) {
   __shared__ f32x4 red[16][17];
   int sgi = 0;
   while (sgi + 1 < sg.n && (int)blockIdx.x >= sg.first[sgi + 1]) ++sgi;
@@ -568,9 +570,10 @@
 
 }
 
-SVAE_EXPORT int svae_colsum_multi(const svae_colsum_seg* segs, int32_t n, svae_stream_t stream) {
-  if (!segs || n <= 0 || n > SVAE_COLSUM_MAX) return SVAE_EINVAL;
-  ColsumSegs sg;
+template <int CAP>
+static int launch_colsum_segs(const svae_colsum_seg* segs, int32_t n, svae_stream_t stream) {
+  if (!segs || n <= 0 || n > CAP) return SVAE_EINVAL;
+  ColsumSegs<CAP> sg;
   sg.n = n;
   int total = 0;
   for (int i = 0; i < n; ++i) {
@@ -585,9 +588,17 @@
     total += cb * sp;
   }
   sg.first[n] = total;
-  hipLaunchKernelGGL(colsum_multi_kernel, dim3((unsigned)total), dim3(256), 0, (hipStream_t)stream, sg);
+  hipLaunchKernelGGL(colsum_multi_kernel<CAP>, dim3((unsigned)total), dim3(256), 0, (hipStream_t)stream, sg);
   SVAE_LAUNCH_CHECK();
   return SVAE_OK;
+}
+
+SVAE_EXPORT int svae_colsum_multi(const svae_colsum_seg* segs, int32_t n, svae_stream_t stream) {
+  return launch_colsum_segs<SVAE_COLSUM_MAX>(segs, n, stream);
+}
+
+SVAE_EXPORT int svae_colsum_list(const svae_colsum_seg* segs, int32_t n, svae_stream_t stream) {
+  return launch_colsum_segs<SVAE_COLSUM_LIST_MAX>(segs, n, stream);
 }
 
 struct LnFwdPlan {
diff --git a/sparse-vae_amd/sparse_vae/_native.py b/sparse-vae_amd/sparse_vae/_native.py
--- a/sparse-vae_amd/sparse_vae/_native.py
+++ b/sparse-vae_amd/sparse_vae/_native.py
@@ -68,6 +68,7 @@
 
 GROUP_MAX = 256
 COLSUM_MAX = 8
+COLSUM_LIST_MAX = 32
 LN_MULTI_MAX = 4
 
 
@@ -133,6 +134,16 @@
                                   c_void_p, c_int64, c_int32, c_int32, c_void_p, c_void_p],
     'svae_ce_prob_bwd_prep': [c_void_p, c_int64, c_void_p, c_void_p, c_void_p, c_void_p, c_void_p, c_int32, c_int32,
                               c_int32, c_int32, c_int32, c_void_p, c_void_p, c_void_p, c_void_p, c_void_p],
+    'svae_ce_prob_finalize_tail': [c_void_p, c_int32, c_void_p, c_void_p, c_int32, c_int32, c_int32, c_int32, c_void_p,
+                                   c_void_p, c_void_p, c_void_p, c_void_p, c_void_p, c_int64, c_void_p, c_int64,
+                                   c_void_p, c_void_p, c_int64, c_int32, c_int32, c_void_p, c_void_p, c_float, c_void_p,
+                                   c_void_p],
+    'svae_ce_prob_bwd_prep_gs': [c_void_p, c_int64, c_void_p, c_void_p, c_void_p, c_void_p, c_void_p, c_float, c_void_p,
+                                 c_void_p, c_int32, c_int32, c_int32, c_int32, c_int32, c_int32, c_void_p, c_void_p,
+                                 c_void_p, c_void_p, c_void_p],
+    'svae_reparam_kl_bwd_bf': [c_void_p, c_void_p, c_void_p, c_void_p, c_void_p, c_void_p, c_void_p, c_int32, c_int32,
+                               c_void_p],
+    'svae_colsum_list': [c_void_p, c_int32, c_void_p],
     'svae_embedding_bwd_ce': [c_void_p, c_void_p, c_void_p, c_int32, c_int32, c_int32, c_void_p, c_void_p, c_void_p],
     'svae_ce_grad': [c_void_p, c_int64, c_void_p, c_void_p, c_void_p, c_void_p, c_void_p, c_int32, c_int32, c_int32,
                      c_int32, c_int32, c_void_p],
diff --git a/sparse-vae_amd/sparse_vae/engine.py b/sparse-vae_amd/sparse_vae/engine.py
--- a/sparse-vae_amd/sparse_vae/engine.py
+++ b/sparse-vae_amd/sparse_vae/engine.py
@@ -5,7 +5,7 @@
 import torch
 
 from . import kernels as K
-from ._native import COLSUM_MAX, GROUP_MAX, LN_MULTI_MAX, ZPROJ_MAX
+from ._native import COLSUM_LIST_MAX, COLSUM_MAX, GROUP_MAX, LN_MULTI_MAX, ZPROJ_MAX
 from ._native import EPI_BF16, EPI_F32, EPI_F32_ACC, EPI_GELU, EPI_GELU_BWD, EPI_DROPOUT_RESID, \
     EPI_ROTARY_BF16, EPI_CE_STATS, EPI_F32_ATOMIC, EPI_CE_PROB, EPI_ROWSCALE_GATHER
 
@@ -210,8 +210,8 @@
         self._dw_names = False
         self._dwg_states, self._dwg_sched = [], {}
         self._zp_pending, self._zp_ctx = [], None
-        self._cs_pending = []
-        self.ncu = (torch.cuda.get_device_properties(flat.device).multi_processor_count
+        self._cs_pending, self._cs_slots, self._cs_all = [], 0, False
+        self.ncu =(torch.cuda.get_device_properties(flat.device).multi_processor_count
                     if flat.device.type == 'cuda' else 256)
 
     def rot(self, L, window=0):
@@ -239,10 +239,7 @@
         x, mean, rstd = st
         D = self.d
         wg = self.P.grad[self.P.offsets[name + '.weight'][0]:][:2 * D]
-        if len(self._cs_pending) == COLSUM_MAX:
-            self.flush_colsum()
-        k, n1 = len(self._cs_pending), 1024 * 2 * D
-        part = self.ws.get('ln.parts', (COLSUM_MAX * n1,), f32)[k * n1:(k + 1) * n1]
+        part = self._cs_part(1, D)
         if gelu is not None:
             K.layernorm_bwd_gelu(dy, x, self.P.f(name + '.weight'), mean, rstd, gelu, dx_bf, wg, rows, D, part,
                                  defer=self._cs_pending)
@@ -256,10 +253,27 @@
             K.zproj_bwd_multi(self._zp_pending, z_bf, dz, B, d, Z)
             self._zp_pending = []
 
+    def _cs_part(self, n, D):
+        cap = COLSUM_LIST_MAX if self._cs_all else COLSUM_MAX
+        if len(self._cs_pending) + n > cap or self._cs_slots + n > cap:
+            self.flush_colsum()
+        k, n1 = self._cs_slots, 1024 * 2 * D
+        self._cs_slots += n
+        return self.ws.get('ln.parts_all' if self._cs_all else 'ln.parts', (cap * n1,), f32)[k * n1:(k + n) * n1]
+
+    def _cs_defer(self, inp, rows, cols, out):
+        if not self._cs_all or inp.dtype != f32 or (inp.data_ptr() | out.data_ptr()) % 16:
+            K.colsum(inp, rows, cols, cols, out)
+            return
+        if len(self._cs_pending) == COLSUM_LIST_MAX:
+            self.flush_colsum()
+        self._cs_pending.append((inp, rows, cols, cols, out))
+
     def flush_colsum(self):
         if self._cs_pending:
-            K.colsum_multi(self._cs_pending)
+            (K.colsum_list if self._cs_all else K.colsum_multi)(self._cs_pending)
             self._cs_pending = []
+        self._cs_slots = 0
 
     def _job(self, dY, X, wname, rows, n_out, n_in, ldy=None, ldx=None, bias=None):
         bg = None
@@ -309,7 +323,10 @@
 
     def _db(self, dY, bname, rows, cols, ld=None):
         off = self.P.offsets[bname][0]
-        K.colsum(dY, rows, cols, ld or cols, self.P.grad[off:off + cols])
+        if ld is None or ld == cols:
+            self._cs_defer(dY, rows, cols, self.P.grad[off:off + cols])
+        else:
+            K.colsum(dY, rows, cols, ld, self.P.grad[off:off + cols])
 
     def layer_fwd(self, pre, x, B, Sx, L, pad, *, learned=0, cross=False, causal=False, ctx=None, heads, hd,
                   drop_p=0.0, seed=0, tag, out=None, window=0, out_bf=None, zsplice=None, ctx_ln=None):
@@ -457,7 +474,7 @@
         K.gemm(gx1, P.wT(a + 'output_linear.weight', d, d), dO, rows_q, d, d, epi=EPI_BF16)
         if st['learned']:
             kv = st['kv']
-            dq32 = ws.get('b.dq32', (B * Lq, d), f32)
+            dq32 = ws.get(f'b.dq32.{st["tag"]}' if self._cs_all else 'b.dq32', (B * Lq, d), f32)
             dkv = ws.get(bn('b.dkv'), (rows_x, 2 * d))
             K.attention(P.w(a + 'learned_queries').view(Lq, d), kv, kv[:, d:], st['O'], st['lse'], B=B, H=heads,
                         Lq=Lq, Lk=Sx, hd=hd, sq=d, bq=0, sk=2 * d, sv=2 * d, bk=Sx * 2 * d, bv=Sx * 2 * d, so=d,
@@ -465,7 +482,7 @@
                         delta=delta, dq=dq32, bdq=Lq * d, dk=dkv, dv=dkv[:, d:], sdk=2 * d, sdv=2 * d,
                         bdk=Sx * 2 * d, bdv=Sx * 2 * d, rot=rot, rot_d=d, **st['Ox'],
                         dq_part=self._dq_part(B, heads, Lq, Sx, hd))
-            K.colsum(dq32, B, Lq * d, Lq * d, P.g(a + 'learned_queries').view(-1))
+            self._cs_defer(dq32, B, Lq * d, P.g(a + 'learned_queries').view(-1))
             self._dw_pair(wo_dw, self._job(dkv, st['h'], a + 'k_linear.weight', rows_x, 2 * d, d,
                                            bias=a + 'k_linear.bias'))
             dh = ws.get('b.dh', (rows_x, d))
@@ -564,17 +581,19 @@
             e1 = torch.cuda.Event(enable_timing=True)
             e1.record()
             probe.append((e0, e1))
+        loss = ws.get('loss', (1,), f32)
         if head == 'prob':
-            sat = ws.get('ce.sat', (T + 1,), torch.int32)
-            K.ce_prob_finalize(part, ntile, coff, labels, T, L, nchunks, chunk_len, lse, row_loss, chunk_w, nll,
-                               fix=(hh, W, bias, logits, sat))
+            sat = ws.bufs.get('ce.sat')
+            if sat is None or sat.numel() != T + 3:
+                sat = ws.get('ce.sat', (T + 3,), torch.int32, zero=True)
+            K.ce_prob_finalize_tail(part, ntile, coff, labels, T, L, nchunks, chunk_len, lse, row_loss, chunk_w, nll,
+                                    (hh, W, bias, logits, sat), kl, kl_weight, loss)
         else:
             K.ce_finalize(part, ntile, lab_logit, labels, T, L, nchunks, chunk_len, lse, row_loss, chunk_w, nll)
+            K.step_scalars(kl_weight, nll=nll, kl=kl, loss=loss)
         sv.update(xf=xf, gp0=gp0, h0=h0, hh=hh, ln_h=ln_h, logits=logits, lse=lse, chunk_w=chunk_w,
                   nchunks=nchunks, chunk_len=chunk_len, labels=labels, ids32=ids32, ntok=ntok64, x_emb=x_emb,
                   row_loss=row_loss, head=head, coff=coff)
-        loss = ws.get('loss', (1,), f32)
-        K.step_scalars(kl_weight, nll=nll, kl=kl, loss=loss)
         self.saved = sv
         return {'loss': loss[0], 'nll': nll[0], 'kl': kl[0], 'train_kl': kl[1], 'raw_kl': raw_kl,
                 'mu': stats[:, :Z], 'logvar': stats[:, Z:], 'stats': stats, 'kl_buf': kl, 'z': zf, 'eps': eps_buf,
@@ -634,11 +653,7 @@
             rows = x.shape[0]
             names = [g['pre'] + 'context_layer_norm' for g in grp]
             wgs = [P.grad[P.offsets[n + '.weight'][0]:][:2 * D] for n in names]
-            n1 = 1024 * 2 * D
-            if len(self._cs_pending) + len(grp) > COLSUM_MAX:
-                self.flush_colsum()
-            k = len(self._cs_pending)
-            part = self.ws.get('ln.parts', (COLSUM_MAX * n1,), f32)[k * n1:(k + len(grp)) * n1]
+            part = self._cs_part(len(grp), D)
             K.layernorm_bwd_multi([g['dcx'] for g in grp], x, [P.f(n + '.weight') for n in names], mean, rstd, dctx,
                                   dctx, wgs, rows, D, part, defer=self._cs_pending)
 
@@ -824,15 +839,21 @@
             raise RuntimeError('backward() without a saved forward')
         self._dwq, self._dw_jobs = None, []
         self._dw_names = self.dw_group and user_ready is None
+        self.flush_colsum()
+        self._cs_all = user_ready is None
         B, L = sv['B'], sv['L']
         T, V, Z, N = B * L, hp.vocab_size, hp.latent_depth, hp.num_latents
         gs = ws.get('gscale', (2,), f32)
+        dz = ws.get('b.dz', (B, Z), f32)
         gl = gloss.reshape(1)
-        if gl.is_cuda and gl.dtype == f32:
-            K.step_scalars(kl_weight, gloss=gl, gs=gs)
-        else:
-            gs[0:1].copy_(gl)
-            gs[1:2].copy_(gl * kl_weight)
+        gs_fused = sv['head'] == 'prob' and gl.is_cuda and gl.dtype == f32
+        if not gs_fused:
+            if gl.is_cuda and gl.dtype == f32:
+                K.step_scalars(kl_weight, gloss=gl, gs=gs)
+            else:
+                gs[0:1].copy_(gl)
+                gs[1:2].copy_(gl * kl_weight)
+            dz.zero_()
 
         logits = sv['logits']
         dhh = ws.get('b.dhh', (T, d))
@@ -843,8 +864,12 @@
             r_t = ws.get('b.ce_r', (T,), f32)
             q_t = ws.get('b.ce_q', (T,), f32)
             dbias = P.g('output_layer.3.bias')
-            K.ce_prob_bwd_prep(hh, sv['lse'], sv['coff'], sv['chunk_w'], sv['labels'], gs[0:1], T, L, nch, clen, d, hh_r,
-                               r_t, q_t, dbias)
+            if gs_fused:
+                K.ce_prob_bwd_prep_gs(hh, sv['lse'], sv['coff'], sv['chunk_w'], sv['labels'], gl, kl_weight, gs, T, L,
+                                      nch, clen, d, hh_r, r_t, q_t, dbias, zero=dz)
+            else:
+                K.ce_prob_bwd_prep(hh, sv['lse'], sv['coff'], sv['chunk_w'], sv['labels'], gs[0:1], T, L, nch, clen, d,
+                                   hh_r, r_t, q_t, dbias)
             s = self._head_dw_splits(V, d)
             if s == 1:
                 K.gemm(logits, hh_r, P.g('input_layer.0.weight'), V, d, T, a_t=True, b_t=True, lda=V, ldb=d, ldc=d,
@@ -872,7 +897,6 @@
                drop_p=top['drop_p'] if g2_pre else 0.0, seed=top['seed'] if g2_pre else 0)
         ready(P.end('output_layer.3.bias'))
 
-        dz = ws.get('b.dz', (B, Z), f32, zero=True)
         dzh = ws.get('b.dzh', (B, d), f32)
         dzh_bf = ws.get('b.dzh_bf', (B, d))
         dx_prev = ws.get('b.dx_prev', (T, d), f32)
@@ -906,9 +930,8 @@
         dx_emb = dx
 
         dstats = ws.get('b.dstats', (B, 2 * Z), f32)
-        K.reparam_bwd(sv['stats'], sv['eps'], dz, sv['ntok'], gs[1:2], dstats, B, Z)
         dstats_bf = ws.get('b.dstats_bf', (B, 2 * Z))
-        K.cast_bf16(dstats, dstats_bf)
+        K.reparam_bwd(sv['stats'], sv['eps'], dz, sv['ntok'], gs[1:2], dstats, B, Z, dstats_bf=dstats_bf)
         self._dw(self._job(dstats_bf, sv['enc_bf'], 'q_of_z_given_x.linear.weight', B, 2 * Z, d))
         self._db(dstats, 'q_of_z_given_x.linear.bias', B, 2 * Z)
         denc = ws.get('b.denc', (B, d), f32)
diff --git a/sparse-vae_amd/sparse_vae/kernels.py b/sparse-vae_amd/sparse_vae/kernels.py
--- a/sparse-vae_amd/sparse_vae/kernels.py
+++ b/sparse-vae_amd/sparse_vae/kernels.py
@@ -343,6 +343,19 @@
         _colsum_segs[i].inp, _colsum_segs[i].out = inp.data_ptr(), out.data_ptr()
         _colsum_segs[i].ld, _colsum_segs[i].rows, _colsum_segs[i].cols = ld, rows, cols
     check(lib.svae_colsum_multi(ctypes.addressof(_colsum_segs), len(segs), stream()), 'svae_colsum_multi')
+
+
+_colsum_list = (N.ColsumSeg * N.COLSUM_LIST_MAX)()
+
+
+def colsum_list(segs):
+    assert 0 < len(segs) <= N.COLSUM_LIST_MAX
+    for i, (inp, rows, cols, ld, out) in enumerate(segs):
+        _dev(inp, out)
+        assert inp.dtype == f32 and out.dtype == f32
+        _colsum_list[i].inp, _colsum_list[i].out = inp.data_ptr(), out.data_ptr()
+        _colsum_list[i].ld, _colsum_list[i].rows, _colsum_list[i].cols = ld, rows, cols
+    check(lib.svae_colsum_list(ctypes.addressof(_colsum_list), len(segs), stream()), 'svae_colsum_list')
 
 
 def colsum(inp, rows, cols, ld, out, accumulate=True):
@@ -432,7 +445,13 @@
                                   stream()), 'svae_reparam_kl_fwd')
 
 
-def reparam_bwd(stats, eps, dz, ntok, gkl, dstats, B, Z):
+def reparam_bwd(stats, eps, dz, ntok, gkl, dstats, B, Z, dstats_bf=None):
+    if dstats_bf is not None:
+        assert dstats_bf.dtype == bf16 and dstats_bf.is_contiguous() and dstats_bf.numel() == 2 * B * Z
+        check(lib.svae_reparam_kl_bwd_bf(stats.data_ptr(), eps.data_ptr(), ptr(dz), ntok.data_ptr(), gkl.data_ptr(),
+                                         dstats.data_ptr(), dstats_bf.data_ptr(), B, Z, stream()),
+              'svae_reparam_kl_bwd_bf')
+        return
     check(lib.svae_reparam_kl_bwd(stats.data_ptr(), eps.data_ptr(), ptr(dz), ntok.data_ptr(), gkl.data_ptr(),
                                   dstats.data_ptr(), B, Z, stream()), 'svae_reparam_kl_bwd')
 
@@ -502,6 +521,34 @@
                                     chunk_w.data_ptr(), labels.data_ptr(), gscale.data_ptr(), rows, seq, nchunks,
                                     chunk_len, D, hh_out.data_ptr(), r_out.data_ptr(), q_out.data_ptr(), ptr(dbias),
                                     stream()), 'svae_ce_prob_bwd_prep')
+
+
+def ce_prob_finalize_tail(part, ntile, row_off, labels, rows, seq, nchunks, chunk_len, lse, row_loss, chunk_w, nll,
+                          fix, kl, kl_weight, loss):
+    assert chunk_w.numel() >= nchunks and chunk_w.dtype == f32
+    red = ce_red_ws(part.device, nchunks)
+    hh, W, bias, P, sat = fix
+    _dev(hh, W, P, sat, kl, loss)
+    assert sat.dtype == torch.int32 and sat.numel() >= rows + 3 and P.shape[0] >= rows
+    assert kl.dtype == f32 and loss.dtype == f32
+    check(lib.svae_ce_prob_finalize_tail(part.data_ptr(), ntile, row_off.data_ptr(), labels.data_ptr(), rows, seq,
+                                         nchunks, chunk_len, lse.data_ptr(), row_loss.data_ptr(), chunk_w.data_ptr(),
+                                         nll.data_ptr(), red.data_ptr(), hh.data_ptr(), hh.stride(0), W.data_ptr(),
+                                         W.stride(0), ptr(bias), P.data_ptr(), P.stride(0), W.shape[0], hh.shape[1],
+                                         sat.data_ptr(), kl.data_ptr(), float(kl_weight), loss.data_ptr(), stream()),
+          'svae_ce_prob_finalize_tail')
+
+
+def ce_prob_bwd_prep_gs(hh, lse, row_off, chunk_w, labels, gloss, kl_weight, gs, rows, seq, nchunks, chunk_len, D,
+                        hh_out, r_out, q_out, dbias=None, zero=None):
+    _dev(hh, lse, row_off, chunk_w, labels, gloss, gs, hh_out, r_out, q_out)
+    assert gloss.dtype == f32 and gs.dtype == f32 and gs.numel() >= 2 and gs.data_ptr() != gloss.data_ptr()
+    assert zero is None or (zero.is_cuda and zero.dtype == f32 and zero.is_contiguous())
+    check(lib.svae_ce_prob_bwd_prep_gs(hh.data_ptr(), hh.stride(0), lse.data_ptr(), row_off.data_ptr(),
+                                       chunk_w.data_ptr(), labels.data_ptr(), gloss.data_ptr(), float(kl_weight),
+                                       gs.data_ptr(), ptr(zero), zero.numel() if zero is not None else 0, rows, seq,
+                                       nchunks, chunk_len, D, hh_out.data_ptr(), r_out.data_ptr(), q_out.data_ptr(),
+                                       ptr(dbias), stream()), 'svae_ce_prob_bwd_prep_gs')
 
 
 def embedding_bwd_ce(ids, dout, dtable, rows, D, seq, hh, q):
```
